# mj-will/aspire

Measured on AMD Instinct MI355X. Metric: particle-steps/sec (N x n_steps), 1M particles d=32; log-evidence err vs ref, higher is better.
Workload: dtype f64

## Files before the change

### aspire_amd/csrc/asmc_ctx.hip

```cpp
#include <dlfcn.h>
#include <stdarg.h>

#include <math.h>

#include "asmc_common.h"

static thread_local char g_err[512] = "";

void asmc_set_error(const char* fmt, ...) {
    va_list ap;
    va_start(ap, fmt);
    vsnprintf(g_err, sizeof(g_err), fmt, ap);
    va_end(ap);
}

__global__ __launch_bounds__(256) void k_poison_lds(int words) {
    extern __shared__ unsigned int s_poison[];
    for (int i = threadIdx.x; i < words; i += 256) s_poison[i] = 0xFFFFFFFFu;
    __syncthreads();
    if (s_poison[(threadIdx.x * 977) % words] != 0xFFFFFFFFu) __builtin_trap();
}
void asmc_poison_lds(asmc_ctx* ctx, hipStream_t st) {
    const int bytes = 160 * 1024 - 1024;
    static bool attr_set_dev[ASMC_MAX_DEVICES] = {false}; bool& attr_set = attr_set_dev[asmc_dev_slot(ctx)];
    if (!attr_set) {
        (void)hipFuncSetAttribute(reinterpret_cast<const void*>(k_poison_lds), hipFuncAttributeMaxDynamicSharedMemorySize, bytes);
        attr_set = true;
    }
    hipLaunchKernelGGL(k_poison_lds, dim3(4 * ctx->num_cu), dim3(256), bytes, st, bytes / 4);
}

void asmc_prof_begin(asmc_ctx* ctx, const char* label, const void* kernel, hipStream_t st) {
    if (!ctx || !ctx->prof_on) return;
    int v = 0;
    while (v < ctx->prof_nv && ctx->prof_vfn[v] != kernel) v++;
    if (v < ASMC_PROF_VARIANTS) {
        if (v == ctx->prof_nv) ctx->prof_vfn[v] = kernel, ctx->prof_vcnt[v] = 0, ctx->prof_nv++;
        ctx->prof_vcnt[v]++;
    }
    if (ctx->prof_n >= ASMC_PROF_MAX) return;
    ctx->prof_label[ctx->prof_n] = label;
    (void)hipEventRecord(ctx->prof_ev[2 * ctx->prof_n], st);
}

void asmc_prof_end(asmc_ctx* ctx, hipStream_t st) {
    if (!ctx || !ctx->prof_on || ctx->prof_n >= ASMC_PROF_MAX) return;
    (void)hipEventRecord(ctx->prof_ev[2 * ctx->prof_n + 1], st);
    ctx->prof_n++;
}

void asmc_bm_table_host(double* tab) {
    const long double two_pi = 6.283185307179586476925286766559005768L;
    for (int k = 0; k < BM_SC_N; k++) {
        const long double ang = two_pi * ((long double)k + 0.5L) / (long double)BM_SC_N;
        tab[2 * k] = (double)sinl(ang);
        tab[2 * k + 1] = (double)cosl(ang);
    }
    for (int i = 0; i < BM_LG_N; i++) {
        const long double c = 0.5L + ((long double)i + 0.5L) / (2.0L * BM_LG_N);
        const double rc = (double)(1.0L / c);
        tab[2 * (BM_SC_N + i)] = rc;
        tab[2 * (BM_SC_N + i) + 1] = (double)(2.0L * logl((long double)rc));
    }
}

extern "C" {

int asmc_profile_enable(asmc_ctx* ctx, int on) {
    ASMC_REQUIRE(ctx != nullptr, "null ctx");
    if (on && !ctx->prof_ev) {
        ctx->prof_ev = new (std::nothrow) hipEvent_t[2 * ASMC_PROF_MAX];
        ctx->prof_label = new (std::nothrow) const char*[ASMC_PROF_MAX];
        if (!ctx->prof_ev || !ctx->prof_label) {
            asmc_set_error("out of host memory");
            return ASMC_ERR_NOMEM;
        }
        for (int i = 0; i < 2 * ASMC_PROF_MAX; i++) ASMC_HIP(hipEventCreate(&ctx->prof_ev[i]));
    }
    ctx->prof_on = on ? 1 : 0;
    if (on) ctx->prof_n = 0, ctx->prof_nv = 0;
    return ASMC_OK;
}

int asmc_profile_variants(asmc_ctx* ctx, char* buf, int64_t buf_len) {
    ASMC_REQUIRE(ctx && buf && buf_len > 0, "bad arguments");
    buf[0] = 0;
    int64_t off = 0;
    for (int v = 0; v < ctx->prof_nv; v++) {
        Dl_info info;
        const char* sym = dladdr(ctx->prof_vfn[v], &info) && info.dli_sname && info.dli_saddr == ctx->prof_vfn[v] ? info.dli_sname : nullptr;
        char unknown[32];
        if (!sym) snprintf(unknown, sizeof(unknown), "%p", ctx->prof_vfn[v]), sym = unknown;
        const int w = snprintf(buf + off, (size_t)(buf_len - off), "%s %lld\n", sym, ctx->prof_vcnt[v]);
        if (w < 0 || off + w >= buf_len) {
            buf[off] = 0;
            asmc_set_error("asmc_profile_variants: buffer of %lld bytes too small", (long long)buf_len);
            return ASMC_ERR_ARG;
        }
        off += w;
    }
    ctx->prof_nv = 0;
    return ASMC_OK;
}

int asmc_profile_report(asmc_ctx* ctx, char* buf, int64_t buf_len) {
    ASMC_REQUIRE(ctx && buf && buf_len > 0, "bad arguments");
    buf[0] = 0;
    if (!ctx->prof_ev || ctx->prof_n == 0) return ASMC_OK;
    ASMC_HIP(hipEventSynchronize(ctx->prof_ev[2 * (ctx->prof_n - 1) + 1]));
    const int n = ctx->prof_n;
    int64_t off = 0;
    char* done = new (std::nothrow) char[n]();
    if (!done) return ASMC_ERR_NOMEM;
    for (int i = 0; i < n; i++) {
        if (done[i]) continue;
        double tot = 0.0;
        int cnt = 0;
        for (int j = i; j < n; j++) {
            if (done[j] || strcmp(ctx->prof_label[j], ctx->prof_label[i]) != 0) continue;
            float ms = 0.f;
            if (hipEventElapsedTime(&ms, ctx->prof_ev[2 * j], ctx->prof_ev[2 * j + 1]) == hipSuccess) {
                tot += ms;
                cnt++;
            }
            done[j] = 1;
        }
        const int w = snprintf(buf + off, (size_t)(buf_len - off), "%s %d %.6f\n", ctx->prof_label[i], cnt, cnt ? tot / cnt : 0.0);
        if (w < 0 || off + w >= buf_len) break;
        off += w;
    }
    delete[] done;
    ctx->prof_n = 0;
    return ASMC_OK;
}

int asmc_abi_version(void) { return ASMC_ABI_VERSION; }

const char* asmc_last_error(void) { return g_err; }

int asmc_device_count(int* n_out) {
    ASMC_REQUIRE(n_out != nullptr, "null output");
    int n = 0;
    hipError_t e = hipGetDeviceCount(&n);
    if (e != hipSuccess) {
        *n_out = 0;
        asmc_set_error("hipGetDeviceCount failed: %s", hipGetErrorString(e));
        return ASMC_ERR_HIP;
    }
    *n_out = n;
    return ASMC_OK;
}

int asmc_ctx_create(asmc_ctx** ctx_out, int device, int64_t n_max, int d_max) {
    ASMC_REQUIRE(ctx_out != nullptr, "null ctx_out");
    ASMC_REQUIRE(n_max > 0, "n_max must be positive");
    ASMC_REQUIRE(d_max > 0 && d_max <= ASMC_MAX_DIMS, "d_max out of range");
    *ctx_out = nullptr;
    ASMC_HIP(hipSetDevice(device));
    hipDeviceProp_t prop;
    ASMC_HIP(hipGetDeviceProperties(&prop, device));
    asmc_ctx* c = new (std::nothrow) asmc_ctx();
    if (!c) {
        asmc_set_error("out of host memory");
        return ASMC_ERR_NOMEM;
    }
    memset(c, 0, sizeof(*c));
    c->device = device;
    c->n_max = n_max;
    c->d_max = d_max;
    c->num_cu = prop.multiProcessorCount > 0 ? prop.multiProcessorCount : 256;
    c->n_tiles_max = scan_tiles(n_max) + 1;
    c->gram_blocks = (d_max <= 128 ? 4 : 2) * c->num_cu;
    if (c->gram_blocks > ASMC_MAX_BLOCKS) c->gram_blocks = ASMC_MAX_BLOCKS;
    hipError_t e = hipSuccess;
    auto dmalloc = [&](void** p, size_t bytes) {
        if (e == hipSuccess) e = hipMalloc(p, bytes);
    };
    dmalloc((void**)&c->d_partials, sizeof(double) * ASMC_MAX_BLOCKS * ASMC_MAX_BETAS * 2);
    dmalloc((void**)&c->d_small, sizeof(double) * DS_LEN);
    dmalloc((void**)&c->d_keys, sizeof(unsigned long long) * (ASMC_MAX_BETAS + 8));
    dmalloc((void**)&c->d_tiles, sizeof(double) * scratch_tiles_len(c->n_tiles_max));
    dmalloc((void**)&c->d_tiles_i, sizeof(long long) * scratch_tiles_i_len(c->n_tiles_max));
    c->gram_cap = (size_t)c->gram_blocks * d_max * d_max;
    if (c->gram_cap < (size_t)2048 * 1024) c->gram_cap = (size_t)2048 * 1024;
    dmalloc((void**)&c->d_gram, sizeof(double) * c->gram_cap);
    c->d_mmtab = nullptr;
    c->poison_lds = getenv("ASMC_POISON_LDS") != nullptr;
    c->d_max_pad = d_max <= 4 ? 4 : d_max <= 8 ? 8 : d_max <= 16 ? 16 : d_max <= 32 ? 32 : d_max <= 64 ? 64 : d_max <= 128 ? 128 : 0;
    dmalloc((void**)&c->d_mmtab, sizeof(double) * 2 * 144 * 64);
    dmalloc((void**)&c->d_guide, sizeof(unsigned int) * ((size_t)n_max + 8));
    dmalloc((void**)&c->d_tilectr, ASMC_TILECTR_BYTES + (size_t)n_max + 64);
    c->d_flags = c->d_tilectr ? reinterpret_cast<unsigned char*>(c->d_tilectr) + ASMC_TILECTR_BYTES : nullptr;
    dmalloc((void**)&c->d_gamma, sizeof(double) * ((size_t)ASMC_GAMMA_BATCH * (size_t)n_max + 64 * ASMC_GAMMA_BATCH));
    dmalloc((void**)&c->d_rec, sizeof(double) * 4 * (size_t)n_max);
    const size_t student = (size_t)d_max * (d_max + 1) + (size_t)(ASMC_STUDENT_MAX_ROWS / 64) * (d_max + 2);
    dmalloc((void**)&c->d_student, sizeof(double) * student);
    if (e == hipSuccess) e = hipHostMalloc((void**)&c->h_student, sizeof(double) * student, hipHostMallocDefault);
    dmalloc((void**)&c->d_counts, sizeof(long long) * (size_t)(ASMC_MAX_PCN_STEPS + ASMC_MAX_BLOCKS + n_max / 64 + 8));
    dmalloc((void**)&c->d_rho, sizeof(double) * (ASMC_MAX_PCN_STEPS + 8));
    dmalloc((void**)&c->d_stretch, sizeof(unsigned long long) * ASMC_MAX_PCN_STEPS);
    dmalloc((void**)&c->d_mh, sizeof(unsigned long long) * ASMC_MAX_PCN_STEPS);
    dmalloc((void**)&c->d_nuts, sizeof(unsigned long long) * (4 * ASMC_MAX_PCN_STEPS + 8));
    if (e == hipSuccess) e = hipMemset(c->d_tilectr, 0, ASMC_TILECTR_BYTES);
    dmalloc((void**)&c->d_bar, sizeof(unsigned int) * 1024 * 17);
    if (e == hipSuccess) e = hipMemset(c->d_bar, 0, sizeof(unsigned int) * 1024 * 17);
    dmalloc((void**)&c->d_pcgtab, sizeof(unsigned long long) * (64 * 4 + 8));
    dmalloc((void**)&c->d_select, sizeof(long long) * (2 * (ASMC_SELECT_THREADS / 64) + 8));
    dmalloc((void**)&c->d_ptab, sizeof(double) * (2 * 32 * 32 + 32 + 3 * ASMC_MAX_COMPONENTS * (1 + 2 * 32) + 64));
    dmalloc((void**)&c->d_bmtab, sizeof(double) * 2 * BM_TAB_N);
    dmalloc((void**)&c->d_fimg, ASMC_FUSED_IMAGE_BYTES);
    dmalloc((void**)&c->d_ref, sizeof(double) * (128 + 128 * 128));
    if (e == hipSuccess) {
        double tab[2 * BM_TAB_N];
        asmc_bm_table_host(tab);
        e = hipMemcpy(c->d_bmtab, tab, sizeof(tab), hipMemcpyHostToDevice);
    }
    if (e == hipSuccess) e = hipHostMalloc((void**)&c->h_pinned, sizeof(double) * HP_LEN, hipHostMallocDefault);
    if (e == hipSuccess) e = hipHostMalloc((void**)&c->h_gram, sizeof(double) * (128 + 128 * 128), hipHostMallocDefault);
    if (e != hipSuccess) {
        asmc_set_error("asmc_ctx_create: allocation failed: %s", hipGetErrorString(e));
        asmc_ctx_destroy(c);
        return ASMC_ERR_NOMEM;
    }
    *ctx_out = c;
    return ASMC_OK;
}

int asmc_ctx_destroy(asmc_ctx* c) {
    if (!c) return ASMC_OK;
    (void)hipSetDevice(c->device);
    (void)hipFree(c->d_partials);
    (void)hipFree(c->d_small);
    (void)hipFree(c->d_keys);
    (void)hipFree(c->d_tiles);
    (void)hipFree(c->d_tiles_i);
    (void)hipFree(c->d_gram);
    if (c->d_mmtab) (void)hipFree(c->d_mmtab);
    if (c->d_f16tab) (void)hipFree(c->d_f16tab);
    (void)hipFree(c->d_guide);
    (void)hipFree(c->d_gamma);
    (void)hipFree(c->d_student);
    if (c->h_student) (void)hipHostFree(c->h_student);
    if (c->d_ysoa) (void)hipFree(c->d_ysoa);
    if (c->d_xpad) (void)hipFree(c->d_xpad);
    if (c->d_chain_lq) (void)hipFree(c->d_chain_lq);
    if (c->d_chain_rows) (void)hipFree(c->d_chain_rows);
    (void)hipFree(c->d_counts);
    (void)hipFree(c->d_rho);
    (void)hipFree(c->d_stretch);
    (void)hipFree(c->d_mh);
    (void)hipFree(c->d_nuts);
    if (c->d_nuts_ws) (void)hipFree(c->d_nuts_ws);
    (void)hipFree(c->d_tilectr);
    (void)hipFree(c->d_rec);
    (void)hipFree(c->d_bar);
    (void)hipFree(c->d_pcgtab);
    (void)hipFree(c->d_select);
    (void)hipFree(c->d_ptab);
    (void)hipFree(c->d_bmtab);
    (void)hipFree(c->d_fimg);
    (void)hipFree(c->d_ref);
    if (c->prof_ev) {
        for (int i = 0; i < 2 * ASMC_PROF_MAX; i++) (void)hipEventDestroy(c->prof_ev[i]);
        delete[] c->prof_ev;
        delete[] c->prof_label;
    }
    if (c->h_pinned) (void)hipHostFree(c->h_pinned);
    if (c->h_gram) (void)hipHostFree(c->h_gram);
    if (c->ev_mutate) (void)hipEventDestroy(c->ev_mutate);
    if (c->ev_is) (void)hipEventDestroy(c->ev_is);
    delete c;
    return ASMC_OK;
}

}
```

### aspire_amd/csrc/asmc_pcn_dev.h

```cpp
#pragma once
#include "asmc_common.h"

bool asmc_flow_math_split();

struct PcnAdaptArgs {
    unsigned int* done;
    unsigned long long* nonfinite;
    long long* cell;
    const long long* prev_cell;
    long long* counts_out;
    double* rho;
    double* rho_hist;
    double target;
    int64_t n;
    int t, adapt;
    int last;
};

__device__ __forceinline__ double pcn_adapt_rho(double rho, long long c, int64_t n, double target, int t) {
    const double acc = (double)c / (double)n;
    double r = exp(log(rho) + (acc - target) / pow((double)(t + 1), 0.75));
    r = r < 1e-4 ? 1e-4 : r;
    r = r > 0.99 ? 0.99 : r;
    return r;
// ... 58 lines not shown
    const double dk = (double)k;
    return fma(dk, 6.93147180369123816490e-01, -((hfsq - fma(s, hfsq + R, dk * 1.90821492927058770002e-10)) - f));
}

__device__ __forceinline__ double bm_sqrt(double a) {
    const double y = __builtin_amdgcn_rsq(a);
    double g = a * y, h = 0.5 * y;
    const double r = fma(-h, g, 0.5);
    g = fma(g, r, g);
    h = fma(h, r, h);
    const double dres = fma(-g, g, a);
    return a > 0.0 ? fma(dres, h, g) : 0.0;
}

__device__ __forceinline__ void bm_sincos_turns(double u, double& sn, double& cs) {
    const double q = __builtin_rint(4.0 * u);
    const double f = fma(q, -0.25, u);
    const double x = f * 6.28318530717958647692;
    const double z = x * x;
    const double v = z * x;
    const double rs = fma(z, fma(z, fma(z, fma(z, 1.58969099521155010221e-10, -2.50507602534068634195e-08), 2.75573137070700676789e-06),
                                 -1.98412698298579493134e-04), 8.33333333332248946124e-03);
    const double sx = fma(v, fma(z, rs, -1.66666666666666324348e-01), x);
    const double rc = z * fma(z, fma(z, fma(z, fma(z, fma(z, -1.13596475577881948265e-11, 2.08757232129817482790e-09),
                                                -2.75573143513906633035e-07), 2.48015872894767294178e-05),
                                 -1.38888888888741095749e-03), 4.16666666666666019037e-02);
    const double hz = 0.5 * z;
    const double wv = 1.0 - hz;
    const double cx = wv + fma(z, rc, (1.0 - wv) - hz);
    const int qi = (int)q;
    const bool swap = qi & 1;
    const double s0 = swap ? cx : sx, c0 = swap ? sx : cx;
    sn = (qi & 2) ? -s0 : s0;
    cs = ((qi + 1) & 2) ? -c0 : c0;
}

__device__ __forceinline__ void box_muller(double u1, double u2, double& z0, double& z1) {
#ifdef ASMC_NOISE_LIBM
    const double r = sqrt(-2.0 * log(u1));
    double s, c;
    sincospi(2.0 * u2, &s, &c);
#else
    const double r = bm_sqrt(-2.0 * bm_log_unit(u1));
    double s, c;
    bm_sincos_turns(u2, s, c);
#endif
    z0 = r * c;
    z1 = r * s;
}

typedef double bm_d2 __attribute__((ext_vector_type(2)));
void asmc_bm_table_host(double* tab);

template <int THREADS>
__device__ __forceinline__ void bm_tab_stage(bm_d2* __restrict__ s, const double* __restrict__ g) {
    for (int e = threadIdx.x; e < BM_TAB_N; e += THREADS) s[e] = reinterpret_cast<const bm_d2*>(g)[e];
}
__device__ __forceinline__ void bm_tab_stage_rt(bm_d2* __restrict__ s, const double* __restrict__ g) {
    for (int e = threadIdx.x; e < BM_TAB_N; e += (int)blockDim.x) s[e] = reinterpret_cast<const bm_d2*>(g)[e];
}
__device__ __forceinline__ bm_d2* bm_lds() {
    __shared__ bm_d2 s_bm[BM_TAB_N];
    return s_bm;
}

struct BmPair {
    double m, sx, cm1;
    int e;
};
__device__ __forceinline__ void bm_pair_idx(uint32_t wr, uint32_t wa, BmPair& t, uint32_t& i_sc, uint32_t& i_lg) {
    i_sc = wa >> 24;
    const double X = (double)wr + 0.5;
    t.m = __builtin_amdgcn_frexp_mant(X);
    t.e = __builtin_amdgcn_frexp_exp(X);
    const uint32_t mh = (uint32_t)((unsigned long long)__double_as_longlong(t.m) >> 32);
    i_lg = BM_SC_N + ((mh >> 13) & (BM_LG_N - 1));
    const double x = fma((double)((int)(wa & 0xFFFFFFu) - (1 << 23)), 1.4629180792671596e-09, 7.314590396335798e-10);
    const double z = x * x;
    const double ps = fma(z, fma(z, -1.9841269841269841e-04, 8.3333333333333332e-03), -1.6666666666666666e-01);
    t.sx = fma(x * z, ps, x);
    t.cm1 = z * fma(z, fma(z, -1.3888888888888889e-03, 4.1666666666666664e-02), -0.5);
}
__device__ __forceinline__ void bm_pair_fin(const BmPair& t, const bm_d2 sc, const bm_d2 lg, double& z0, double& z1) {
    const double sn = sc.x + fma(sc.y, t.sx, sc.x * t.cm1);
    const double cs = sc.y + fma(-sc.x, t.sx, sc.y * t.cm1);
    const double r = fma(t.m, lg.x, -1.0);
    double p = fma(r, 3.3333333333333331e-01, -4.0000000000000002e-01);
    p = fma(r, p, 0.5);
    p = fma(r, p, -6.6666666666666663e-01);
    p = fma(r, p, 1.0);
    p = fma(r, p, -2.0);
    const double a = fma((double)(32 - t.e), 1.3862943611198906, lg.y) + r * p;
    const double y = __builtin_amdgcn_rsq(a);
    double g = a * y, h = 0.5 * y;
    const double rr = fma(-h, g, 0.5);
    g = fma(g, rr, g);
    h = fma(h, rr, h);
    const double rad = fma(fma(-g, g, a), h, g);
    z0 = rad * cs;
    z1 = rad * sn;
}
__device__ __forceinline__ void bm_pair32(uint32_t wr, uint32_t wa, const bm_d2* __restrict__ tab, double& z0, double& z1) {
    BmPair t;
    uint32_t i_sc, i_lg;
    bm_pair_idx(wr, wa, t, i_sc, i_lg);
    bm_pair_fin(t, tab[i_sc], tab[i_lg], z0, z1);
}

__device__ __forceinline__ void normal_quad(unsigned long long seed, unsigned long long gid, uint32_t step, uint32_t q,
                                            const bm_d2* __restrict__ tab, double& z0, double& z1, double& z2, double& z3) {
    uint32_t w[4];
    philox4x32_10((uint32_t)gid, (uint32_t)(gid >> 32), step, q | 0x20000000u, (uint32_t)seed, (uint32_t)(seed >> 32), w);
    BmPair ta, tb;
    uint32_t ia_sc, ia_lg, ib_sc, ib_lg;
    bm_pair_idx(w[0], w[1], ta, ia_sc, ia_lg);
    bm_pair_idx(w[2], w[3], tb, ib_sc, ib_lg);
    const bm_d2 sca = tab[ia_sc], lga = tab[ia_lg], scb = tab[ib_sc], lgb = tab[ib_lg];
    bm_pair_fin(ta, sca, lga, z0, z1);
    bm_pair_fin(tb, scb, lgb, z2, z3);
}
__device__ __forceinline__ void normal_pair(unsigned long long seed, unsigned long long gid, uint32_t step, uint32_t pr,
                                            const bm_d2* __restrict__ tab, double& z0, double& z1) {
    uint32_t w[4];
    philox4x32_10((uint32_t)gid, (uint32_t)(gid >> 32), step, (pr >> 1) | 0x20000000u, (uint32_t)seed, (uint32_t)(seed >> 32), w);
    const bool second = pr & 1u;
    bm_pair32(second ? w[2] : w[0], second ? w[3] : w[1], tab, z0, z1);
}

__device__ __forceinline__ void normal_quad_f32_raw(unsigned long long seed, unsigned long long gid, uint32_t step,
                                                    uint32_t slot, float& f0, float& f1, float& f2, float& f3) {
    uint32_t w[4];
    philox4x32_10((uint32_t)gid, (uint32_t)(gid >> 32), step, slot | 0x40000000u, (uint32_t)seed,
                  (uint32_t)(seed >> 32), w);
    const float k = 2.3283064365386963e-10f;
    const float u0 = fmaf((float)w[0], k, 1.1641532182693481e-10f);
    const float u1 = fmaf((float)w[2], k, 1.1641532182693481e-10f);
    const float t0 = (float)w[1] * k, t1 = (float)w[3] * k;
    const float r0 = __builtin_amdgcn_sqrtf(-1.3862943611198906f * __builtin_amdgcn_logf(u0));
    const float r1 = __builtin_amdgcn_sqrtf(-1.3862943611198906f * __builtin_amdgcn_logf(u1));
    f0 = r0 * __builtin_amdgcn_cosf(t0);
    f1 = r0 * __builtin_amdgcn_sinf(t0);
    f2 = r1 * __builtin_amdgcn_cosf(t1);
    f3 = r1 * __builtin_amdgcn_sinf(t1);
}

__device__ __forceinline__ void normal_quad_f32(unsigned long long seed, unsigned long long gid, uint32_t step,
                                                uint32_t slot, double& z0, double& z1, double& z2, double& z3) {
    float f0, f1, f2, f3;
    normal_quad_f32_raw(seed, gid, step, slot, f0, f1, f2, f3);
    z0 = (double)f0;
    z1 = (double)f1;
    z2 = (double)f2;
    z3 = (double)f3;
}

__device__ __forceinline__ double accept_uniform(unsigned long long seed, unsigned long long gid,
                                                 uint32_t step) {
    uint32_t w[4];
    philox4x32_10((uint32_t)gid, (uint32_t)(gid >> 32), step, 0xFFFFFFFFu, (uint32_t)seed,
                  (uint32_t)(seed >> 32), w);
    return u01_from_words(w[0], w[1]);
}

template <bool F32 = false>
__device__ __forceinline__ double gamma_unit(double shape, unsigned long long seed, unsigned long long gid,
                                             uint32_t step, const bm_d2* __restrict__ tab) {
    const double dd = shape - 1.0 / 3.0, c = 1.0 / sqrt(9.0 * dd);
#pragma unroll
    for (uint32_t a = 0; a < 8; a++) {
        double z0;
        uint32_t w[4];
        philox4x32_10((uint32_t)gid, (uint32_t)(gid >> 32), step, (F32 ? 0xC0000000u : 0x80000000u) | a, (uint32_t)seed, (uint32_t)(seed >> 32), w);
        if (F32) {
            const float k = 2.3283064365386963e-10f;
            const float u0 = fmaf((float)w[0], k, 1.1641532182693481e-10f);
            const float r0 = __builtin_amdgcn_sqrtf(-1.3862943611198906f * __builtin_amdgcn_logf(u0));
            z0 = (double)(r0 * __builtin_amdgcn_cosf((float)w[1] * k));
        } else {
            double z1;
            bm_pair32(w[0], w[1], tab, z0, z1);
        }
        const double u = u01_from_words(w[2], w[3]);
        double v = 1.0 + c * z0;
        if (v <= 0.0) continue;
        v = v * v * v;
        if (log(u) < 0.5 * z0 * z0 + dd - dd * v + dd * log(v)) return dd * v;
    }
    return dd;
}
template <bool TP = true>
__device__ __forceinline__ double tpcn_scale(double rho, double nu, double q0, const double* __restrict__ gam, int64_t i) {
    if (!TP || gam == nullptr) return rho;
    return rho * sqrt((nu + q0) / (2.0 * gam[i]));
}
template <bool TP>
__device__ __forceinline__ double tpcn_scale_ct(double rho, double nu, double q0, const double* __restrict__ gam, int64_t i) {
    if (!TP) return rho;
    return rho * sqrt((nu + q0) / (2.0 * gam[i]));
}
__device__ __forceinline__ double log1p_nonneg(double x) {
    const double u = 1.0 + x;
    const double r = bm_log_unit(u);
    return u < INFINITY ? r : u;
}
template <bool TP>
__device__ __forceinline__ double ref_corr_ct(double q, double nu, int d) {
    if (!TP) return 0.5 * q;
    return 0.5 * ((double)d + nu) * log1p_nonneg(q / nu);
}

template <bool TP = true>
__device__ __forceinline__ double ref_corr(double q, double nu, int d) {
    if (!TP) return 0.5 * q;
    return nu > 0.0 ? 0.5 * ((double)d + nu) * log1p_nonneg(q / nu) : 0.5 * q;
}

struct MixDev {
    int C;
    const double* logw;
    const double* mu;
    const double* prec;
};

static inline MixDev to_dev(const asmc_mixture& m) {
    MixDev r;
    r.C = m.n_components;
    r.logw = m.logw_dev;
    r.mu = m.mu_dev;
    r.prec = m.prec_dev;
    return r;
}


__device__ __forceinline__ double log_p_t_guard(double r) { return (r < INFINITY) ? r : -INFINITY; }
__device__ __forceinline__ double log_p_t(double ll, double lp, double lq, double beta) {
    return log_p_t_guard((1.0 - beta) * lq + beta * (ll + lp));
}


struct PcnDev {
    int d;
    double beta;
    const double* mu;
    const double* L;
    const double* Linv;
    MixDev ll, lp, lq;
    unsigned long long seed, gid0;
    int noise;
    double nu;
    const double* gam;
    void* ys;
    long long n_pad;
    const double* bmtab;
    unsigned char* tile_par;
    int d_noise;
    int dpad;
    int mode;
};


#define PTAB_TRI(D) ((D) * ((D) + 1) / 2)
#define PTAB_MIX(D) (ASMC_MAX_COMPONENTS * (1 + 2 * (D)))
#define PTAB_SIZE(D) (2 * PTAB_TRI(D) + (D) + 3 * PTAB_MIX(D))
#define PTAB_BLK(D) (((D) / 4) * ((D) / 4 + 1) / 2 * 16)
struct PcnScalars {
    double beta;
    double nu;
    const double* gam;
    void* ys;
    long long n_pad;
    int d_real;
    unsigned long long seed, gid0;
    int c_ll, c_lp, c_lq;
    const double* bmtab;
    unsigned char* tile_par;
    int d_noise;
};


template <typename T>
__device__ __forceinline__ double soa_load(__amdgpu_buffer_rsrc_t r, unsigned voff, unsigned soff) {
    if constexpr (sizeof(T) == 8) {
        const auto v = __builtin_amdgcn_raw_buffer_load_b64(r, (int)voff, (int)soff, 0);
        return __builtin_bit_cast(double, v);
    } else {
        const unsigned v = __builtin_amdgcn_raw_buffer_load_b32(r, (int)voff, (int)soff, 0);
        return (double)__uint_as_float(v);
    }
}
template <typename T>
__device__ __forceinline__ void soa_store(__amdgpu_buffer_rsrc_t r, unsigned voff, unsigned soff, double x) {
    if constexpr (sizeof(T) == 8) {
        using u2 = decltype(__builtin_amdgcn_raw_buffer_load_b64(r, 0, 0, 0));
        __builtin_amdgcn_raw_buffer_store_b64(__builtin_bit_cast(u2, x), r, (int)voff, (int)soff, 0);
    } else {
        __builtin_amdgcn_raw_buffer_store_b32(__float_as_uint((float)x), r, (int)voff, (int)soff, 0);
    }
}


bool asmc_pcn_flow_fused_ok(const asmc_pcn_params* prm, const asmc_coupling* f);
int asmc_pcn_flow_fused_launch(asmc_ctx* ctx, int64_t n, int x_dtype, double* ll, double* lp, double* lq, const PcnDev& pd,
                               const asmc_coupling* f, const double* rho_ptr, uint32_t step, unsigned int* tile_counter,
                               long long* block_counts, int* grid_out, const PcnAdaptArgs& adapt, int img_words, hipStream_t st);
int asmc_pcn_flow_fused_stage(asmc_ctx* ctx, const PcnDev& pd, const asmc_coupling* f, int* words_out, hipStream_t st);

#define MM_WHITEN 0
#define MM_STEP 1
#define MM_UNWHITEN 2
#define MM_STEP_T 3
#define MM_XPROPOSE 4
#define MM_XPROPOSE_T 5
#define MM_UNWHITEN_X 6
bool asmc_pcn_mm_supported(int d, const void* x);
int asmc_pcn_mm_pack(asmc_ctx* ctx, const PcnDev& pd, hipStream_t st);
int asmc_pcn_flow16_tables(asmc_ctx* ctx, const PcnDev& pd, const asmc_coupling* f, hipStream_t st);
int asmc_pcn_flow16_launch(asmc_ctx* ctx, int64_t n, int x_dtype, void* x, double* ll, double* lp, double* lq, const PcnDev& pd,
                           const asmc_coupling* f, const double* rho_ptr, uint32_t step, long long* block_counts, int* grid_out,
                           unsigned long long* nonfinite, hipStream_t st);
int asmc_pcn_mm_launch(asmc_ctx* ctx, int64_t n, int x_dtype, void* x, double* ll, double* lp, double* lq, const PcnDev& pd,
                       int mode, const double* rho_ptr, uint32_t step, long long* block_counts, int* grid_out,
                       hipStream_t st);
bool asmc_gram_mm_supported(int d, const void* x);
int asmc_gram_mm_launch(asmc_ctx* ctx, int64_t n, int d, int x_dtype, const void* x, const double* d_center, int* grid_out,
                        hipStream_t st, double* out2, double n_div);
```

### aspire_amd/csrc/asmc_pcn_drive.hip

```cpp
#include <stdlib.h>

#include <chrono>

#include "asmc_pcn_shared.h"

static PcnDev pcn_dev_from_params(const asmc_ctx* ctx, const asmc_pcn_params* prm, int d_noise) {
    PcnDev pd;
    memset(&pd, 0, sizeof(pd));
    pd.bmtab = ctx->d_bmtab;
    pd.d = prm->d;
    pd.d_noise = d_noise;
    pd.beta = prm->beta;
    pd.mu = prm->mu_dev;
    pd.L = prm->L_dev;
    pd.Linv = prm->Linv_dev;
    pd.seed = prm->seed;
    pd.gid0 = prm->gid0;
    pd.nu = prm->nu;
    return pd;
}

struct PcnNeeds {
    int n_mix;
    bool noise;
// ... 245 lines not shown
        rc = pack_pcn_tables(ctx, pd, st);
        if (rc) return rc;
        return pcn_step_launch(ctx, n, x_dtype, const_cast<void*>(x), qf_old, qf_new, nullptr, pd, rho_ptr, step, nullptr, &grid, st);
    }
    if (asmc_pcn_mm_supported(d, x) && ((uintptr_t)x_prop % 16) == 0 && ctx->d_mmtab && !pcn_env_generic()) {
        pd.noise = ASMC_NOISE_F64;
        rc = asmc_pcn_mm_pack(ctx, pd, st);
        if (rc) return rc;
        return asmc_pcn_mm_launch(ctx, n, x_dtype, const_cast<void*>(x), qf_old, qf_new, reinterpret_cast<double*>(x_prop), pd,
                                  pd.nu > 0.0 ? MM_XPROPOSE_T : MM_XPROPOSE, rho_ptr, step, nullptr, &grid, st);
    }
    const int D = pcn_pad_dim(d);
    if (D != d && D > 0 && D <= ctx->d_max_pad && !(D == 32 && d > 16) && !pcn_env_generic() && !pcn_env_nopad()) {
        PcnDev src = pd;
        src.ll.C = src.lp.C = src.lq.C = 0;
        PcnPadded pad;
        rc = pcn_pad_problem(ctx, n, d, D, x_dtype, x, src, 0, st, &pad);
        if (rc) return rc;
        PcnDev p2 = pd;
        p2.d = D;
        p2.d_noise = d;
        p2.mu = pad.mu;
        p2.L = pad.L;
        p2.Linv = pad.Linv;
        rc = pcn_propose_launch(ctx, n, D, x_dtype, pad.xp, pad.xq, qf_old, qf_new, p2, rho_ptr, step, st);
        if (rc) return rc;
        return launch_unpad_rows(ctx, n, d, D, x_dtype, pad.xq, x_prop, st);
    }
    return pcn_generic_propose_launch(ctx, n, x_dtype, x, x_prop, qf_old, qf_new, pd, rho_ptr, step, &grid, st);
}

static int ysplit_pd(asmc_ctx* ctx, int64_t n, const asmc_pcn_params* prm, PcnDev& pd) {
    ASMC_REQUIRE(ctx && prm, "null pointer");
    ASMC_REQUIRE(n > 0 && n <= ctx->n_max, "n out of range for this ctx");
    ASMC_REQUIRE(prm->x_dtype == ASMC_F64 || prm->x_dtype == ASMC_F32, "bad x_dtype");
    ASMC_REQUIRE(prm->mu_dev && prm->L_dev && prm->Linv_dev, "null reference pointer");
    ASMC_REQUIRE(!(prm->nu > 0.0) || prm->nu >= 1.0, "nu must be >= 1 (or <= 0 for the Gaussian reference)");
    pd = pcn_dev_from_params(ctx, prm, 0);
    ASMC_REQUIRE(prm->noise == ASMC_NOISE_F64 || prm->noise == ASMC_NOISE_F32, "bad noise mode");
    pd.noise = prm->noise;
    return ASMC_OK;
}

static int ysplit_propose_prepare(asmc_ctx* ctx, int64_t n, PcnDev& pd, uint32_t step, hipStream_t st) {
    pd.ys = ctx->d_ysoa;
    pd.n_pad = ((n + 63) / 64) * 64;
    if (ctx->ptab_tag == 0 || ctx->ptab_tag != ctx->ysplit_seq) {
        const int rc = pack_pcn_tables(ctx, pd, st);
        if (rc) return rc;
        ctx->ptab_tag = ctx->ysplit_seq;
    }
    return pcn_prepare_gamma(ctx, n, pd, step, st);
}

extern "C" {

int asmc_pcn_propose(asmc_ctx* ctx, int64_t n, int d, int x_dtype, const void* x, void* x_prop, double* qf_old,
                     double* qf_new, const double* mu, const double* L, const double* Linv, double rho, double nu,
                     uint64_t seed, uint64_t gid0, uint32_t step, asmc_stream stream) {
    ASMC_REQUIRE(ctx && x && x_prop && qf_old && qf_new && mu && L && Linv, "null pointer");
    ASMC_REQUIRE(!(nu > 0.0) || nu >= 1.0, "nu must be >= 1 (or <= 0 for the Gaussian reference)");
    ASMC_REQUIRE(n > 0 && n <= ctx->n_max && d > 0 && d <= ASMC_MAX_DIMS, "bad sizes");
    ASMC_REQUIRE(x_dtype == ASMC_F64 || x_dtype == ASMC_F32, "bad x_dtype");
    ASMC_REQUIRE(rho >= 0.0 && rho <= 1.0, "rho must be in (0, 1], or 0 for the device-resident step size");
    const int fits = pcn_generic_check(d, x_dtype);
    if (fits) return fits;
    hipStream_t st = as_stream(stream);
    PcnDev pd;
    memset(&pd, 0, sizeof(pd));
    pd.bmtab = ctx->d_bmtab;
    pd.d = d;
    pd.mu = mu;
    pd.L = L;
    pd.Linv = Linv;
    pd.seed = seed;
    pd.gid0 = gid0;
    pd.nu = nu;
    if (rho > 0.0) {
        const int rc = pcn_set_scalar_launch(ctx, ctx->d_rho, rho, st);
        if (rc) return rc;
    }
    return pcn_propose_launch(ctx, n, d, x_dtype, x, x_prop, qf_old, qf_new, pd, ctx->d_rho, step, st);
}

int asmc_pcn_split_begin(asmc_ctx* ctx, double rho0, asmc_stream stream) {
    ASMC_REQUIRE(ctx != nullptr, "null ctx");
    ASMC_REQUIRE(rho0 > 0.0 && rho0 <= 1.0, "rho must be in (0, 1]");
    return pcn_set_scalar_launch(ctx, ctx->d_rho, rho0, as_stream(stream));
}

int asmc_pcn_split_adapt(asmc_ctx* ctx, int64_t n_global, double target_accept, int t, int adapt, asmc_stream stream) {
    ASMC_REQUIRE(ctx != nullptr, "null ctx");
    ASMC_REQUIRE(n_global > 0 && t >= 0 && t < ASMC_MAX_PCN_STEPS, "bad n_global / step index");
    hipStream_t st = as_stream(stream);
    return pcn_close_step(ctx, st, 1, reinterpret_cast<const long long*>(ctx->d_keys), n_global, t, ctx->d_counts, ctx->d_rho,
                          ctx->d_rho + 8, target_accept, adapt);
}

int asmc_pcn_split_end(asmc_ctx* ctx, int n_steps, int64_t* n_accept_host, double* rho_hist_host, double* rho_host,
                       asmc_stream stream) {
    ASMC_REQUIRE(ctx && n_accept_host && rho_host, "null pointer");
    ASMC_REQUIRE(n_steps >= 1 && n_steps <= ASMC_MAX_PCN_STEPS, "n_steps out of range");
    hipStream_t st = as_stream(stream);
    ASMC_HIP(hipStreamSynchronize(st));
    return pcn_finish_call(ctx, 0, nullptr, n_steps, nullptr, false, rho_host, n_accept_host, rho_hist_host, st);
}

int asmc_pcn_ysplit_begin(asmc_ctx* ctx, int64_t n, const void* x, const asmc_pcn_params* prm, double rho0,
                          asmc_stream stream) {
    PcnDev pd;
    int rc = ysplit_pd(ctx, n, prm, pd);
    if (rc) return rc;
    ASMC_REQUIRE(x != nullptr, "null pointer");
    ASMC_REQUIRE(rho0 > 0.0 && rho0 <= 1.0, "rho must be in (0, 1]");
    hipStream_t st = as_stream(stream);
    if (!pcn_reg_supported(pd.d, prm->x_dtype == ASMC_F64 ? 8 : 4, x) || !pcn_ensure_ysoa(ctx, n, pd.d, prm->x_dtype, pd, st)) {
        asmc_set_error("whitened-state split session: d=%d is not a register-kernel dimension or no scratch", pd.d);
        return ASMC_ERR_UNSUPPORTED;
    }
    rc = pcn_set_scalar_launch(ctx, ctx->d_rho, rho0, st);
    if (rc) return rc;
    rc = pack_pcn_tables(ctx, pd, st);
    if (rc) return rc;
    ctx->ptab_tag = ++ctx->ysplit_seq;
    pd.mode = PCN_WHITEN_S;
    pd.noise = ASMC_NOISE_F64;
    int grid = 0;
    return pcn_step_launch(ctx, n, prm->x_dtype, const_cast<void*>(x), nullptr, nullptr, nullptr, pd, ctx->d_rho, 0, pcn_block_counts(ctx),
                           &grid, st);
}

int asmc_pcn_ysplit_propose(asmc_ctx* ctx, int64_t n, const asmc_pcn_params* prm, uint32_t step, void* x_prop,
                            asmc_stream stream) {
    PcnDev pd;
    int rc = ysplit_pd(ctx, n, prm, pd);
    if (rc) return rc;
    ASMC_REQUIRE(x_prop != nullptr && ((uintptr_t)x_prop % 16) == 0, "x_prop must be a 16-byte aligned device buffer");
    ASMC_REQUIRE(ctx->d_ysoa != nullptr, "no session (asmc_pcn_ysplit_begin)");
    hipStream_t st = as_stream(stream);
    rc = ysplit_propose_prepare(ctx, n, pd, step, st);
    if (rc) return rc;
    int grid = 0;
    return pcn_reg_flow_launch(ctx, n, prm->x_dtype, PCN_FLOW_PROPOSE_SX, nullptr, x_prop, nullptr, nullptr, nullptr, nullptr, nullptr,
                               nullptr, pd, ctx->d_rho, step, pcn_block_counts(ctx), &grid, st);
}

int asmc_pcn_ysplit_propose_tr(asmc_ctx* ctx, int64_t n, const asmc_pcn_params* prm, uint32_t step, const asmc_transform* t,
                               const double* premap_dev, const asmc_mixture* qmix, int minus_logj, void* x_prop,
                               double* logj_out, double* lq_out, asmc_stream stream) {
    PcnDev pd;
    int rc = ysplit_pd(ctx, n, prm, pd);
    if (rc) return rc;
    ASMC_REQUIRE(t && x_prop && logj_out && ((uintptr_t)x_prop % 16) == 0, "null / misaligned pointer");
    ASMC_REQUIRE(ctx->d_ysoa != nullptr, "no session (asmc_pcn_ysplit_begin)");
    ASMC_REQUIRE(t->d == pd.d && t->kind_dev && t->lower_dev && t->upper_dev, "transform tables missing or of another dimension");
    ASMC_REQUIRE((t->mean_dev == nullptr) == (t->std_dev == nullptr), "affine stage needs both mean and std");
    ASMC_REQUIRE((premap_dev == nullptr) == (qmix == nullptr) && (premap_dev == nullptr) == (lq_out == nullptr),
                 "premap, mixture and lq_out come together");
    ASMC_REQUIRE(!qmix || qmix->n_components == 1, "the proposal density must be a single Gaussian");
    const int logit = (t->hints & 7) == (ASMC_TR_NO_PERIODIC | ASMC_TR_NO_PROBIT);
    const int probit = (t->hints & 7) == (ASMC_TR_NO_PERIODIC | ASMC_TR_NO_LOGIT);
    if (!logit && !probit) {
        asmc_set_error("asmc_pcn_ysplit_propose_tr: the transform must be non-periodic with ONE bounded stage (hints %d)", t->hints);
        return ASMC_ERR_UNSUPPORTED;
    }
    hipStream_t st = as_stream(stream);
    rc = ysplit_propose_prepare(ctx, n, pd, step, st);
    if (rc) return rc;
    double* d_tab = ctx->d_small + DS_TRTAB;
    rc = pcn_trtab_pack_launch(ctx, pd.d, t, premap_dev, qmix, minus_logj, d_tab, st);
    if (rc) return rc;
    int grid = 0;
    return pcn_reg_flow_launch(ctx, n, prm->x_dtype, logit ? PCN_FLOW_PROPOSE_SXT_LOGIT : PCN_FLOW_PROPOSE_SXT_PROBIT, nullptr, x_prop,
                               nullptr, nullptr, nullptr, logj_out, lq_out, d_tab, pd, ctx->d_rho, step, pcn_block_counts(ctx), &grid, st);
}

int asmc_pcn_ysplit_accept(asmc_ctx* ctx, int64_t n, const asmc_pcn_params* prm, uint32_t step, double* ll, double* lp,
                           double* lq, const double* ll_new, const double* lp_new, const double* lq_new, double* lj,
                           const double* lj_new, int64_t n_global, int t, asmc_stream stream) {
    PcnDev pd;
    int rc = ysplit_pd(ctx, n, prm, pd);
    if (rc) return rc;
    ASMC_REQUIRE(ll && lp && lq && ll_new && lp_new && lq_new, "null pointer");
    ASMC_REQUIRE((lj == nullptr) == (lj_new == nullptr), "log-Jacobian arrays: both or neither");
    ASMC_REQUIRE(ctx->d_ysoa != nullptr, "no session (asmc_pcn_ysplit_begin)");
    ASMC_REQUIRE(n_global > 0 && t >= 0 && t < ASMC_MAX_PCN_STEPS, "bad n_global / step index");
    hipStream_t st = as_stream(stream);
    pd.ys = ctx->d_ysoa;
    pd.n_pad = ((n + 63) / 64) * 64;
    rc = pcn_prepare_gamma(ctx, n, pd, step, st);
    if (rc) return rc;
    int grid = 0;
    long long* d_block = pcn_block_counts(ctx);
    rc = pcn_reg_flow_launch(ctx, n, prm->x_dtype, lj ? PCN_FLOW_ACCEPT_SJ : PCN_FLOW_ACCEPT_S, lj, const_cast<double*>(lj_new), ll, lp, lq,
                             const_cast<double*>(ll_new), const_cast<double*>(lp_new), lq_new, pd, ctx->d_rho, step, d_block, &grid, st);
    if (rc) return rc;
    return pcn_close_step(ctx, st, grid, d_block, n_global, t, ctx->d_counts, ctx->d_rho, ctx->d_rho + 8, prm->target_accept,
                          prm->adapt);
}

}

int asmc_pcn_ysplit_unwhiten(asmc_ctx* ctx, int64_t n, void* x, const asmc_pcn_params* prm, bool repack, hipStream_t st) {
    PcnDev pd;
    int rc = ysplit_pd(ctx, n, prm, pd);
    if (rc) return rc;
    ASMC_REQUIRE(x != nullptr && ctx->d_ysoa != nullptr, "null pointer / no session");
    ASMC_REQUIRE(repack || pcn_reg_supported(pd.d, prm->x_dtype == ASMC_F64 ? 8 : 4, x), "x_out: a 16-byte aligned buffer of a session's d");
    pd.ys = ctx->d_ysoa;
    pd.n_pad = ((n + 63) / 64) * 64;
    pd.mode = PCN_UNWHITEN_XS;
    pd.noise = ASMC_NOISE_F64;
    if (repack || ctx->ptab_tag == 0 || ctx->ptab_tag != ctx->ysplit_seq) {
        rc = pack_pcn_tables(ctx, pd, st);
        if (rc) return rc;
        if (!repack) ctx->ptab_tag = ctx->ysplit_seq;
    }
    int grid = 0;
    return pcn_step_launch(ctx, n, prm->x_dtype, x, nullptr, nullptr, nullptr, pd, ctx->d_rho, 0, pcn_block_counts(ctx), &grid, st);
}

extern "C" {

int asmc_pcn_ysplit_end(asmc_ctx* ctx, int64_t n, void* x, const asmc_pcn_params* prm, asmc_stream stream) {
    return asmc_pcn_ysplit_unwhiten(ctx, n, x, prm, true, as_stream(stream));
}

int asmc_pcn_accept(asmc_ctx* ctx, int64_t n, int d, int x_dtype, void* x, const void* x_prop, double* ll, double* lp,
                    double* lq, const double* ll_new, const double* lp_new, const double* lq_new,
                    double* lj_old, const double* lj_new, const double* qf_old, const double* qf_new,
                    double beta, uint64_t seed, uint64_t gid0, uint32_t step, int64_t* n_accept_host,
                    asmc_stream stream) {
    ASMC_REQUIRE(ctx && x && x_prop && ll && lp && lq && ll_new && lp_new && lq_new && qf_old && qf_new, "null pointer");
    ASMC_REQUIRE(n > 0 && n <= ctx->n_max && d > 0, "bad sizes");
    ASMC_REQUIRE(x_dtype == ASMC_F64 || x_dtype == ASMC_F32, "bad x_dtype");
    hipStream_t st = as_stream(stream);
    int rc = pcn_accept_flags_launch(ctx, n, ll, lp, lq, ll_new, lp_new, lq_new, lj_old, lj_new, qf_old, qf_new, beta, seed, gid0, step, st);
    if (rc) return rc;
    rc = launch_copy_flagged(ctx, n, d, x_dtype, x, x_prop, ctx->d_flags, st);
    if (rc) return rc;
    if (n_accept_host) {
        unsigned long long* h = reinterpret_cast<unsigned long long*>(ctx->h_pinned);
        ASMC_HIP(hipMemcpyAsync(h, ctx->d_keys, sizeof(unsigned long long), hipMemcpyDeviceToHost, st));
        ASMC_HIP(hipStreamSynchronize(st));
        *n_accept_host = (int64_t)h[0];
    }
    return ASMC_OK;
}

int64_t asmc_pcn_flow_work_bytes(int64_t n, int d, int x_dtype) {
    const int64_t xb = ((n * d * (x_dtype == ASMC_F64 ? 8 : 4) + 255) / 256) * 256;
    return xb + 5 * (((n * 8 + 255) / 256) * 256);
}

}

static unsigned long long* pcn_flow_bad_cell(asmc_ctx* ctx) {
    return reinterpret_cast<unsigned long long*>(ctx->d_tilectr + 2 * ASMC_MAX_PCN_STEPS);
}

static int pcn_mutate_flow_impl(asmc_ctx* ctx, int64_t n, void* x, double* ll, double* lp, double* lq,
                                const asmc_pcn_params* prm, const asmc_coupling* flow, void* work_dev, int n_steps, uint32_t step0,
                                double* rho_inout_host, int64_t* n_accept_host, double* rho_hist_host, asmc_stream stream, int d_noise) {
    hipStream_t st = as_stream(stream);
    const int d = prm->d;
    const int64_t xb = ((n * d * (prm->x_dtype == ASMC_F64 ? 8 : 4) + 255) / 256) * 256;
    const int64_t vb = ((n * 8 + 255) / 256) * 256;
    char* w = reinterpret_cast<char*>(work_dev);
    void* x_prop = w;
    double* q0 = reinterpret_cast<double*>(w + xb);
    double* q1 = reinterpret_cast<double*>(w + xb + vb);
    double* ll_new = reinterpret_cast<double*>(w + xb + 2 * vb);
    double* lp_new = reinterpret_cast<double*>(w + xb + 3 * vb);
    double* lq_new = reinterpret_cast<double*>(w + xb + 4 * vb);
    PcnDev pd = pcn_dev_from_params(ctx, prm, d_noise);
    double* d_rho = ctx->d_rho;
    long long* d_block = pcn_block_counts(ctx);
    const PcnLoop loop = {ctx, n, prm, n_steps, step0, st};
    int rc;
    const bool reg_ok = pcn_reg_supported(d, prm->x_dtype == ASMC_F64 ? 8 : 4, x) && !pcn_env_xstate();
    if (reg_ok) {
        pd.ll = to_dev(prm->log_likelihood);
        pd.lp = to_dev(prm->log_prior);
        pd.lq = pd.lp;
        pd.noise = prm->noise;
        rc = pack_pcn_tables(ctx, pd, st, d_rho, *rho_inout_host);
        if (rc) return rc;
        int grid = 0;
        const bool soa = pcn_ensure_ysoa(ctx, n, d, prm->x_dtype, pd, st, asmc_pcn_flow_fused_ok(prm, flow));
        auto convert = [&](int mode) -> int {
            PcnDev pc = pd;
            pc.mode = !soa ? mode : mode == PCN_WHITEN ? PCN_WHITEN_S : PCN_UNWHITEN_XS;
            pc.noise = ASMC_NOISE_F64;
            return pcn_step_launch(ctx, n, prm->x_dtype, x, ll, lp, lq, pc, d_rho, 0, d_block, &grid, st);
        };
        rc = convert(PCN_WHITEN);
        if (rc) return rc;
        const bool fused = soa && asmc_pcn_flow_fused_ok(prm, flow);
        if (d_noise > 0 && !fused) {
            asmc_set_error("asmc_pcn_mutate_flow: the zero-padded form needs the one-kernel step");
            return ASMC_ERR_UNSUPPORTED;
        }
        if (fused) {
            ASMC_HIP(hipMemsetAsync(ctx->d_tilectr, 0, ASMC_TILECTR_BYTES + ((size_t)((n + 63) / 64) + 15) / 16 * 16, st));
            pd.tile_par = ctx->d_flags;
            int img_words = 0;
            rc = asmc_pcn_flow_fused_stage(ctx, pd, flow, &img_words, st);
            if (rc) return rc;
            const int lag = prm->adapt >= 2 ? prm->adapt : 1;
            rc = pcn_steps(
                loop, pd,
                [&](int t, uint32_t step, int* g) -> int {
                    PcnAdaptArgs ad = {ctx->d_tilectr + ASMC_MAX_PCN_STEPS + t,
                                       reinterpret_cast<unsigned long long*>(ctx->d_tilectr + 2 * ASMC_MAX_PCN_STEPS),
                                       ctx->count_hook ? ctx->count_cell : nullptr,
                                       ctx->count_hook && t > 0 ? ctx->count_cell : nullptr, ctx->d_counts, d_rho, d_rho + 8,
                                       prm->target_accept, ctx->count_hook ? ctx->count_n_global : n, t, prm->adapt, t == n_steps - 1};
                    if (ctx->count_hook && lag > ctx->count_cells) {
                        asmc_set_error("adapt_lag %d needs %d exchange cells, the installed hook has %d (asmc_pcn_set_count_cells)", lag, lag, ctx->count_cells);
                        return ASMC_ERR_ARG;
                    }
                    return asmc_pcn_flow_fused_launch(ctx, n, prm->x_dtype == ASMC_F64 ? ASMC_F64 : ASMC_F32, ll, lp, lq, pd, flow, d_rho, step,
                                                      ctx->d_tilectr + t, d_block, g, ad, img_words, st);
                },
                [&](int t, int) -> int {
                    if (!(ctx->count_hook && ((t + 1) % lag == 0 || t == n_steps - 1))) return ASMC_OK;
                    const int hrc = ctx->count_hook(ctx->count_hook_user, reinterpret_cast<asmc_stream>(st));
                    if (hrc != 0) {
                        asmc_set_error("accept-count exchange hook failed (%d)", hrc);
                        return ASMC_ERR_ARG;
                    }
                    return t == n_steps - 1 ? pcn_adapt_exchanged_launch(ctx, t, prm->target_accept, prm->adapt, lag, st) : ASMC_OK;
                });
        } else {
            rc = pcn_steps(
                loop, pd,
                [&](int, uint32_t step, int* g) -> int {
                    int r = pcn_reg_flow_launch(ctx, n, prm->x_dtype, soa ? PCN_FLOW_PROPOSE_S : PCN_FLOW_PROPOSE, x, x_prop, ll, lp, lq, ll_new,
                                                lp_new, lq_new, pd, d_rho, step, d_block, g, st);
                    if (r) return r;
                    r = asmc_coupling_logprob(ctx, n, prm->x_dtype, x_prop, flow, lq_new, stream);
                    if (r) return r;
                    return pcn_reg_flow_launch(ctx, n, prm->x_dtype, soa ? PCN_FLOW_ACCEPT_S : PCN_FLOW_ACCEPT, x, x_prop, ll, lp, lq, ll_new,
                                               lp_new, lq_new, pd, d_rho, step, d_block, g, st);
                },
                pcn_close(loop, d_block));
        }
        if (rc) return rc;
        rc = convert(PCN_UNWHITEN_X);
        if (rc) return rc;
    } else {
        rc = pcn_set_scalar_launch(ctx, d_rho, *rho_inout_host, st);
        if (rc) return rc;
        if (d_noise > 0) {
            asmc_set_error("asmc_pcn_mutate_flow: the zero-padded form needs the one-kernel step");
            return ASMC_ERR_UNSUPPORTED;
        }
        rc = pcn_steps(
            loop, pd,
            [&](int, uint32_t step, int* g) -> int {
                int r = pcn_propose_launch(ctx, n, d, prm->x_dtype, x, x_prop, q0, q1, pd, d_rho, step, st);
                if (r) return r;
                r = asmc_coupling_logprob(ctx, n, prm->x_dtype, x_prop, flow, lq_new, stream);
                if (r) return r;
                r = asmc_mixture_logpdf(ctx, n, d, prm->x_dtype, x_prop, &prm->log_prior, lp_new, stream);
                if (r) return r;
                r = asmc_mixture_logpdf(ctx, n, d, prm->x_dtype, x_prop, &prm->log_likelihood, ll_new, stream);
                if (r) return r;
                r = pcn_accept_flags_launch(ctx, n, ll, lp, lq, ll_new, lp_new, lq_new, nullptr, nullptr, q0, q1, prm->beta, prm->seed, prm->gid0,
                                            step, st);
                if (r) return r;
                *g = 1;
                return launch_copy_flagged(ctx, n, d, prm->x_dtype, x, x_prop, ctx->d_flags, st);
            },
            pcn_close(loop, reinterpret_cast<const long long*>(ctx->d_keys)));
        if (rc) return rc;
    }
    return pcn_finish_call(ctx, n, lq, n_steps, pcn_flow_bad_cell(ctx), ctx->mutate_defer, rho_inout_host, n_accept_host, rho_hist_host, st);
}

static int pcn_mutate_flow16_impl(asmc_ctx* ctx, int64_t n, void* x, double* ll, double* lp, double* lq, const asmc_pcn_params* prm,
                                  const asmc_coupling* flow, int n_steps, uint32_t step0, double* rho_inout_host,
                                  int64_t* n_accept_host, double* rho_hist_host, asmc_stream stream, int d_noise) {
    ASMC_REQUIRE(ctx->d_mmtab != nullptr && ((uintptr_t)x % 16) == 0, "flow16: ctx was created with d_max <= 32, or a misaligned state");
    hipStream_t st = as_stream(stream);
    PcnDev pd = pcn_dev_from_params(ctx, prm, d_noise);
    pd.ll = to_dev(prm->log_likelihood);
    pd.lp = to_dev(prm->log_prior);
    pd.lq = pd.lp;
    pd.noise = prm->noise;
    double* d_rho = ctx->d_rho;
    long long* d_block = pcn_block_counts(ctx);
    unsigned long long* d_bad = pcn_flow_bad_cell(ctx);
    const PcnLoop loop = {ctx, n, prm, n_steps, step0, st};
    int rc = pcn_set_scalar_launch(ctx, d_rho, *rho_inout_host, st);
    if (rc) return rc;
    ASMC_HIP(hipMemsetAsync(d_bad, 0, sizeof(unsigned long long), st));
    rc = asmc_pcn_mm_pack(ctx, pd, st);
    if (rc) return rc;
    rc = asmc_pcn_flow16_tables(ctx, pd, flow, st);
    if (rc) return rc;
    int grid = 0;
    rc = asmc_pcn_mm_launch(ctx, n, prm->x_dtype, x, ll, lp, lq, pd, MM_WHITEN, d_rho, 0, d_block, &grid, st);
    if (rc) return rc;
    rc = pcn_steps(
        loop, pd,
        [&](int, uint32_t step, int* g) { return asmc_pcn_flow16_launch(ctx, n, prm->x_dtype, x, ll, lp, lq, pd, flow, d_rho, step, d_block, g, d_bad, st); },
        pcn_close(loop, d_block));
    if (rc) return rc;
    rc = asmc_pcn_mm_launch(ctx, n, prm->x_dtype, x, ll, lp, lq, pd, MM_UNWHITEN_X, d_rho, 0, d_block, &grid, st);
    if (rc) return rc;
    return pcn_finish_call(ctx, n, lq, n_steps, d_bad, ctx->mutate_defer, rho_inout_host, n_accept_host, rho_hist_host, st);
}

template <typename Impl>
static int pcn_flow_padded_tail(asmc_ctx* ctx, int64_t n, int d, int D, int x_dtype, const void* xp, void* x, int n_steps,
                                double* rho_inout_host, int64_t* n_accept_host, double* rho_hist_host, hipStream_t st, Impl impl) {
    const int caller_defers = ctx->mutate_defer;
    ctx->mutate_defer = 1;
    int rc = impl();
    ctx->mutate_defer = caller_defers;
    if (rc) return rc;
    rc = launch_unpad_rows(ctx, n, d, D, x_dtype, xp, x, st);
    if (rc) return rc;
    if (caller_defers) return ASMC_OK;
    ctx->mutate_pending_steps = 0;
    return pcn_collect(ctx, n_steps, true, true, rho_inout_host, n_accept_host, rho_hist_host, st);
}

extern "C" {

int asmc_pcn_mutate_flow(asmc_ctx* ctx, int64_t n, void* x, double* ll, double* lp, double* lq,
                         const asmc_pcn_params* prm, const asmc_coupling* flow, void* work_dev, int64_t work_bytes,
                         int n_steps, uint32_t step0, double* rho_inout_host, int64_t* n_accept_host,
                         double* rho_hist_host, asmc_stream stream) {
    ASMC_REQUIRE(ctx && x && prm && flow, "null pointer");
    if (ctx->chain_on) {
        asmc_set_error("asmc_pcn_mutate_flow: the chain recorder is honoured by asmc_pcn_mutate only (asmc_chain_clear first)");
        return ASMC_ERR_UNSUPPORTED;
    }
    ASMC_REQUIRE(flow->affine == ASMC_AFFINE_TANH || (flow->affine == ASMC_AFFINE_SOFTCLIP && flow->kind == ASMC_FLOW_MAF),
                 "bad affine form (the soft-clipped form is for autoregressive flows)");
    const int d = prm->d;
    const bool lay16 = asmc_flow_layout(flow->kind, flow->dims, flow->hidden) == 1;
    int D16 = 0;
    asmc_pcn_params p16 = *prm;
    if ((d > 32 || lay16) && d <= 128 && d == flow->dims && ctx->d_mmtab && !pcn_env_generic() && !pcn_env_nopad() && !pcn_env_xstate()) {
        const int D = d <= 64 ? 64 : 128;
        p16.d = D;
        if ((D <= ctx->d_max_pad || d <= 32) && asmc_pcn_flow16_ok(&p16, flow)) D16 = D;
    }
    asmc_pcn_params p2 = *prm;
    p2.d = 32;
    const bool pad32 = !D16 && d >= 2 && d < 32 && d == flow->dims && 32 <= ctx->d_max_pad && !pcn_env_generic() && !pcn_env_nopad() &&
                       asmc_pcn_flow_fused_ok(&p2, flow) && !pcn_env_aos() && !pcn_env_xstate();
    const bool reads_noise = D16 || pad32 || (pcn_reg_supported(d, prm->x_dtype == ASMC_F64 ? 8 : 4, x) && !pcn_env_xstate());
    int rc = pcn_check_call(__func__, ctx, n, x, ll, lp, lq, prm, n_steps, rho_inout_host, n_accept_host,
                            {2, reads_noise, flow, !D16, work_dev, work_bytes});
    if (rc) return rc;
    hipStream_t st = as_stream(stream);
    if (D16) {
        if (d == D16 && ((uintptr_t)x % 16) == 0)
            return pcn_mutate_flow16_impl(ctx, n, x, ll, lp, lq, prm, flow, n_steps, step0, rho_inout_host, n_accept_host, rho_hist_host,
                                          stream, 0);
        void* xp = nullptr;
        rc = pcn_pad_params(ctx, n, x, prm, D16, 2, st, &p16, &xp);
        if (rc) return rc;
        return pcn_flow_padded_tail(ctx, n, d, D16, prm->x_dtype, xp, x, n_steps, rho_inout_host, n_accept_host, rho_hist_host, st, [&]() {
            return pcn_mutate_flow16_impl(ctx, n, xp, ll, lp, lq, &p16, flow, n_steps, step0, rho_inout_host, n_accept_host,
                                          rho_hist_host, stream, d);
        });
    }
    if (pad32) {
        void* xp = nullptr;
        rc = pcn_pad_params(ctx, n, x, prm, 32, 2, st, &p2, &xp);
        if (rc) return rc;
        rc = pcn_flow_padded_tail(ctx, n, d, 32, prm->x_dtype, xp, x, n_steps, rho_inout_host, n_accept_host, rho_hist_host, st, [&]() {
            return pcn_mutate_flow_impl(ctx, n, xp, ll, lp, lq, &p2, flow, work_dev, n_steps, step0, rho_inout_host, n_accept_host,
                                        rho_hist_host, stream, d);
        });
        if (rc != ASMC_ERR_UNSUPPORTED) return rc;
        ctx->mutate_pending_steps = 0;
    }
    return pcn_mutate_flow_impl(ctx, n, x, ll, lp, lq, prm, flow, work_dev, n_steps, step0, rho_inout_host, n_accept_host, rho_hist_host,
                                stream, 0);
}

int asmc_pcn_mutate_flow_enqueue(asmc_ctx* ctx, int64_t n, void* x, double* ll, double* lp, double* lq,
                                 const asmc_pcn_params* prm, const asmc_coupling* flow, void* work_dev, int64_t work_bytes,
                                 int n_steps, uint32_t step0, double rho, asmc_stream stream) {
    ASMC_REQUIRE(ctx != nullptr, "null ctx");
    ASMC_REQUIRE(ctx->mutate_pending_steps == 0, "a deferred mutation is still pending (asmc_pcn_mutate_flow_result)");
    int64_t dummy_acc = 0;
    ctx->mutate_defer = 1;
    const int rc = asmc_pcn_mutate_flow(ctx, n, x, ll, lp, lq, prm, flow, work_dev, work_bytes, n_steps, step0, &rho, &dummy_acc,
                                        nullptr, stream);
    ctx->mutate_defer = 0;
    return rc;
}

int asmc_pcn_mutate_flow_result(asmc_ctx* ctx, int n_steps, double* rho_out_host, int64_t* n_accept_host, double* rho_hist_host,
                                asmc_stream stream) {
    ASMC_REQUIRE(ctx && rho_out_host && n_accept_host, "null pointer");
    ASMC_REQUIRE(ctx->mutate_pending_steps == n_steps && n_steps > 0, "no deferred mutation of this length is pending");
    ctx->mutate_pending_steps = 0;
    return pcn_collect(ctx, n_steps, true, true, rho_out_host, n_accept_host, rho_hist_host, as_stream(stream), ctx->ev_mutate);
}

int64_t asmc_pcn_flow_nonfinite(asmc_ctx* ctx) { return ctx ? (int64_t)ctx->flow_nonfinite : -1; }

int64_t asmc_pcn_lq_nan(asmc_ctx* ctx) { return ctx ? (int64_t)ctx->lq_nan : -1; }

int asmc_pcn_set_count_hook(asmc_ctx* ctx, asmc_count_hook hook, void* user, int64_t* cell_dev, int64_t n_global) {
    ASMC_REQUIRE(ctx != nullptr, "null ctx");
    ASMC_REQUIRE(hook == nullptr || (cell_dev != nullptr && n_global > 0), "hook needs a device cell and n_global > 0");
    ctx->count_hook = hook;
    ctx->count_hook_user = user;
    ctx->count_cell = reinterpret_cast<long long*>(cell_dev);
    ctx->count_n_global = n_global;
    ctx->count_cells = 1;
    return ASMC_OK;
}

int asmc_pcn_set_count_cells(asmc_ctx* ctx, int n_cells) {
    ASMC_REQUIRE(ctx != nullptr && n_cells >= 1 && n_cells <= ASMC_MAX_COUNT_CELLS, "n_cells out of range");
    ctx->count_cells = n_cells;
    return ASMC_OK;
}

typedef int (*rccl_allreduce_fn)(const void*, void*, size_t, int, int, void*, hipStream_t);
static int rccl_count_hook(void* user, asmc_stream stream) {
    asmc_ctx* ctx = static_cast<asmc_ctx*>(user);
    const int nccl_int64 = 4, nccl_sum = 0;
    return reinterpret_cast<rccl_allreduce_fn>(ctx->rccl_allreduce)(ctx->count_cell, ctx->count_cell, (size_t)ctx->count_cells, nccl_int64, nccl_sum,
                                                                    ctx->rccl_comm, reinterpret_cast<hipStream_t>(stream));
}

int asmc_set_rccl(asmc_ctx* ctx, void* allreduce_fn, void* nccl_comm) {
    ASMC_REQUIRE(ctx != nullptr, "null ctx");
    ASMC_REQUIRE((allreduce_fn == nullptr) == (nccl_comm == nullptr), "function and communicator come together");
    ctx->rccl_allreduce = allreduce_fn;
    ctx->rccl_comm = nccl_comm;
    return ASMC_OK;
}

int asmc_set_rccl_allgather(asmc_ctx* ctx, void* allgather_fn) {
    ASMC_REQUIRE(ctx != nullptr, "null ctx");
    ctx->rccl_allgather = allgather_fn;
    return ASMC_OK;
}

int asmc_rccl_all_gather(asmc_ctx* ctx, const void* send_dev, void* recv_dev, int64_t count, int is_int64, asmc_stream stream) {
    ASMC_REQUIRE(ctx && send_dev && recv_dev && count > 0, "bad arguments");
    ASMC_REQUIRE(ctx->rccl_allgather && ctx->rccl_comm, "asmc_set_rccl / asmc_set_rccl_allgather first");
    typedef int (*allgather_fn)(const void*, void*, size_t, int, void*, hipStream_t);
    const int dt = is_int64 ? 4 : 8;
    if (reinterpret_cast<allgather_fn>(ctx->rccl_allgather)(send_dev, recv_dev, (size_t)count, dt, ctx->rccl_comm,
                                                            reinterpret_cast<hipStream_t>(stream)) != 0) {
        asmc_set_error("asmc_rccl_all_gather: ncclAllGather failed");
        return ASMC_ERR_ARG;
    }
    return ASMC_OK;
}

int asmc_pcn_set_count_rccl(asmc_ctx* ctx, int64_t* cell_dev, int64_t n_global) {
    ASMC_REQUIRE(ctx != nullptr, "null ctx");
    if (cell_dev == nullptr) return asmc_pcn_set_count_hook(ctx, nullptr, nullptr, nullptr, 0);
    ASMC_REQUIRE(ctx->rccl_allreduce && ctx->rccl_comm, "asmc_set_rccl first");
    return asmc_pcn_set_count_hook(ctx, rccl_count_hook, ctx, cell_dev, n_global);
}

}
```

### aspire_amd/csrc/asmc_pcn_fused.hip

```cpp
#include <stdlib.h>

#include "asmc_common.h"
#include <type_traits>
#include "asmc_pcn_dev.h"
#include "asmc_flow_dev.h"

#ifndef FUSED_THREADS
#define FUSED_THREADS 512
#endif

#define FUSED_TL_DOUBLES 1368
#define FUSED_MAX_COMPONENTS 4
#ifndef MV_DEPTH
#define MV_DEPTH 4
#endif
typedef double double2v __attribute__((ext_vector_type(2)));
__host__ __device__ constexpr int mv_group(int bi) {
    int g = 0;
    while ((g + 1) * (g + 2) <= bi) g++;
    return g;
}
template <int I, int N, typename F>
__device__ __forceinline__ void mv_for_each(F& f) {
    if constexpr (I < N) {
        f(std::integral_constant<int, I>{});
        mv_for_each<I + 1, N>(f);
    }
}
#ifndef FUSED_INPLACE
#define FUSED_INPLACE 1
#endif
#ifndef FUSED_MVMFMA
#define FUSED_MVMFMA FUSED_INPLACE
#endif
typedef double fused_d4 __attribute__((ext_vector_type(4)));
typedef unsigned fused_u4 __attribute__((ext_vector_type(4)));
__device__ __forceinline__ void fused_swap32(double& x, double& y) {
    const unsigned long long xb = __builtin_bit_cast(unsigned long long, x), yb = __builtin_bit_cast(unsigned long long, y);
    const auto lo = __builtin_amdgcn_permlane32_swap((unsigned)xb, (unsigned)yb, false, false);
    const auto hi = __builtin_amdgcn_permlane32_swap((unsigned)(xb >> 32), (unsigned)(yb >> 32), false, false);
    x = __builtin_bit_cast(double, ((unsigned long long)hi[0] << 32) | lo[0]);
    y = __builtin_bit_cast(double, ((unsigned long long)hi[1] << 32) | lo[1]);
}
__device__ __forceinline__ void fused_swap16(double& x, double& y) {
    const unsigned long long xb = __builtin_bit_cast(unsigned long long, x), yb = __builtin_bit_cast(unsigned long long, y);
    const auto lo = __builtin_amdgcn_permlane16_swap((unsigned)xb, (unsigned)yb, false, false);
    const auto hi = __builtin_amdgcn_permlane16_swap((unsigned)(xb >> 32), (unsigned)(yb >> 32), false, false);
    x = __builtin_bit_cast(double, ((unsigned long long)hi[0] << 32) | lo[0]);
    y = __builtin_bit_cast(double, ((unsigned long long)hi[1] << 32) | lo[1]);
}
__device__ __forceinline__ void fused_transpose4(double& q0, double& q1, double& q2, double& q3) {
    fused_swap32(q0, q2);
    fused_swap32(q1, q3);
    fused_swap16(q0, q1);
    fused_swap16(q2, q3);
}
#ifndef HS1P_PREFETCH
#define HS1P_PREFETCH false
#endif
#ifndef FUSED_PRIO_A
#define FUSED_PRIO_A 2
#define FUSED_PRIO_B 1
#endif
#ifndef MV_CHUNK
#define MV_CHUNK 8
#endif
constexpr int FUSED_D = 32;
constexpr int T_MU = FUSED_D * FUSED_D, T_LLMU = T_MU + FUSED_D, T_LLPR = T_LLMU + FUSED_D, T_LPMU = T_LLPR + FUSED_D, T_LPPR = T_LPMU + FUSED_D,
              T_LOGW = T_LPPR + FUSED_D, T_LOC = T_LOGW + 2;
static_assert(T_LOC + 3 * FUSED_D / 2 <= FUSED_TL_DOUBLES, "pCN tables");
constexpr int M_MU = 12 * 64, M_MIX = M_MU + FUSED_D, M_LOGW = M_MIX + 2 * FUSED_MAX_COMPONENTS * 2 * FUSED_D, M_LOC = M_LOGW + 2 * FUSED_MAX_COMPONENTS;
static_assert(M_LOC + 3 * FUSED_D / 2 <= FUSED_TL_DOUBLES, "pCN tables (matrix-core variant)");
constexpr bool MVM = FUSED_MVMFMA && FUSED_INPLACE;

template <int W, int NOISE, bool HS, int KIND>
__device__ __forceinline__ void fused_stage_tables(float* __restrict__ sp, const double* __restrict__ ptab, const PcnScalars& p,
                                                   const float* __restrict__ packed, int n_layers, const float* __restrict__ loc,
                                                   const float* __restrict__ scale) {
    constexpr int D = FUSED_D, THREADS = FUSED_THREADS, HF = KIND == ASMC_FLOW_MAF ? 32 : 16;
    using FD = FlowDims<HF, W>;
    if (HS) {
        flow_stage_hs<HF, W, THREADS>(sp, packed, n_layers);
    } else {
        const int total4 = n_layers * FD::LAYER / 4;
        for (int base = 0; base < total4; base += THREADS * 8) {
            float4 tmp[8];
#pragma unroll
            for (int q = 0; q < 8; q++) {
                const int i4 = base + q * THREADS + threadIdx.x;
                tmp[q] = i4 < total4 ? reinterpret_cast<const float4*>(packed)[i4] : make_float4(0.f, 0.f, 0.f, 0.f);
            }
#pragma unroll
            for (int q = 0; q < 8; q++) {
                const int i4 = base + q * THREADS + threadIdx.x;
                if (i4 < total4) reinterpret_cast<float4*>(sp)[i4] = tmp[q];
            }
        }
    }
    double* tl = reinterpret_cast<double*>(sp + (size_t)n_layers * FD::LAYER);
    {
        const double* m0g = ptab + 2 * PTAB_TRI(D) + D;
        const int dr = (p.d_noise > 0 && p.d_noise < D) ? p.d_noise : D;
        const int dhalf = KIND == ASMC_FLOW_MAF ? 16 : dr / 2;
        auto nat = [&](int r) -> int {
            const int c = r < 16 ? (r < dhalf ? r : -1) : (r - 16 + dhalf);
            return (c >= 0 && c < dr) ? c : -1;
        };
        if (MVM) {
            for (int e = threadIdx.x; e < 12 * 64; e += THREADS) {
                const int slot = e >> 6, l = e & 63, mb = slot < 4 ? 0 : 1, sidx = slot < 4 ? slot : slot - 4;
                const int i = l & 15, j = nat(16 * mb + 4 * (i & 3) + (i >> 2)), k = 4 * sidx + (l >> 4);
                tl[e] = (j >= 0 && k <= j) ? ptab[j * (j + 1) / 2 + k] : 0.0;
            }
            for (int e = threadIdx.x; e < D; e += THREADS) {
                const int j = nat(16 * ((e >> 2) & 1) + 4 * (e >> 3) + (e & 3));
                tl[M_MU + e] = j >= 0 ? ptab[2 * PTAB_TRI(D) + j] : 0.0;
                reinterpret_cast<float*>(tl + M_LOC)[e] = j >= 0 ? loc[j] : 0.0f;
                reinterpret_cast<float*>(tl + M_LOC)[D + e] = j >= 0 ? scale[j] : 1.0f;
                reinterpret_cast<float*>(tl + M_LOC)[2 * D + e] = j >= 0 ? 1.0f / scale[j] : 1.0f;
            }
            for (int e = threadIdx.x; e < 2 * FUSED_MAX_COMPONENTS * D; e += THREADS) {
                const int tc = e / D, er = e % D, tt = tc / FUSED_MAX_COMPONENTS, c = tc % FUSED_MAX_COMPONENTS;
                const int j = nat(16 * ((er >> 2) & 1) + 4 * (er >> 3) + (er & 3));
                const bool live = j >= 0 && c < (tt == 0 ? p.c_ll : p.c_lp);
                const double* mg = m0g + (size_t)tt * PTAB_MIX(D);
                tl[M_MIX + tc * 2 * D + er] = live ? mg[ASMC_MAX_COMPONENTS + c * D + j] : 0.0;
                tl[M_MIX + tc * 2 * D + D + er] = live ? mg[ASMC_MAX_COMPONENTS * (1 + D) + c * D + j] : 0.0;
            }
            if (threadIdx.x < 2 * FUSED_MAX_COMPONENTS) {
                const int tt = threadIdx.x / FUSED_MAX_COMPONENTS, c = threadIdx.x % FUSED_MAX_COMPONENTS;
                tl[M_LOGW + threadIdx.x] = c < (tt == 0 ? p.c_ll : p.c_lp) ? m0g[(size_t)tt * PTAB_MIX(D) + c] : -INFINITY;
            }
        } else {
            for (int e = threadIdx.x; e < D * D; e += THREADS) {
                const int j = e / D, k = e - j * D;
                tl[e] = k <= j ? ptab[j * (j + 1) / 2 + k] : 0.0;
            }
            for (int e = threadIdx.x; e < D; e += THREADS) {
                tl[T_MU + e] = ptab[2 * PTAB_TRI(D) + e];
                tl[T_LLMU + e] = m0g[ASMC_MAX_COMPONENTS + e];
                tl[T_LLPR + e] = m0g[ASMC_MAX_COMPONENTS * (1 + D) + e];
                tl[T_LPMU + e] = m0g[PTAB_MIX(D) + ASMC_MAX_COMPONENTS + e];
                tl[T_LPPR + e] = m0g[PTAB_MIX(D) + ASMC_MAX_COMPONENTS * (1 + D) + e];
                reinterpret_cast<float*>(tl + T_LOC)[e] = loc[e];
                reinterpret_cast<float*>(tl + T_LOC)[D + e] = scale[e];
                reinterpret_cast<float*>(tl + T_LOC)[2 * D + e] = 1.0f / scale[e];
            }
        }
        if (!MVM && threadIdx.x == 0) tl[T_LOGW] = m0g[0], tl[T_LOGW + 1] = m0g[PTAB_MIX(D)];
    }
    if (NOISE == ASMC_NOISE_F64) bm_tab_stage<THREADS>(reinterpret_cast<bm_d2*>(tl + FUSED_TL_DOUBLES), p.bmtab);
}
template <int W, int NOISE, int KIND>
__host__ __device__ constexpr int fused_image_words(int n_layers) {
    return (int)(((size_t)n_layers * FlowDims<(KIND == ASMC_FLOW_MAF ? 32 : 16), W>::LAYER * sizeof(float) + FUSED_TL_DOUBLES * sizeof(double) +
                  (NOISE == ASMC_NOISE_F64 ? BM_TAB_N * sizeof(bm_d2) : 0)) / 16);
}
template <int W, int NOISE, bool HS, int KIND>
__global__ __launch_bounds__(FUSED_THREADS) void k_fused_stage_image(const double* __restrict__ ptab, PcnScalars p, const float* __restrict__ packed,
                                                                     int n_layers, const float* __restrict__ loc, const float* __restrict__ scale,
                                                                     fused_u4* __restrict__ img, int img_words) {
    extern __shared__ __align__(16) float sp[];
    fused_stage_tables<W, NOISE, HS, KIND>(sp, ptab, p, packed, n_layers, loc, scale);
    __syncthreads();
    for (int i = threadIdx.x; i < img_words; i += FUSED_THREADS) img[i] = reinterpret_cast<const fused_u4*>(sp)[i];
}

template <typename T, int W, int NOISE, bool HS, int KIND = ASMC_FLOW_COUPLING, bool MIX = false>
__global__ __launch_bounds__(FUSED_THREADS) void k_pcn_flow_fused(
    int64_t n, double* __restrict__ ll, double* __restrict__ lp, double* __restrict__ lq, const double* __restrict__ ptab,
    PcnScalars p, const double* rho_ptr, uint32_t step, const float* __restrict__ packed, int n_layers,
    const float* __restrict__ loc, const float* __restrict__ scale, float ladj0, float base_const,
    unsigned int* __restrict__ tile_counter, long long* __restrict__ block_counts, PcnAdaptArgs ad, int par_words, int affine,
    const fused_u4* __restrict__ img, int img_words) {
    constexpr int D = FUSED_D, H = 16, THREADS = FUSED_THREADS;
    constexpr int HF = KIND == ASMC_FLOW_MAF ? 32 : H;
    static_assert(KIND == ASMC_FLOW_COUPLING || HS, "the autoregressive variant runs the split-fp16 layers only");
    using FD = FlowDims<HF, W>;
    extern __shared__ __align__(16) float sp[];
    constexpr int IMG_Q = ASMC_FUSED_IMAGE_BYTES / 16 / THREADS;
    fused_u4 iw[IMG_Q];
    if (img != nullptr) {
#pragma unroll
        for (int q = 0; q < IMG_Q; q++) {
            const int i4 = q * THREADS + (int)threadIdx.x;
            iw[q] = img[i4 < img_words ? i4 : img_words - 1];
        }
    } else {
        fused_stage_tables<W, NOISE, HS, KIND>(sp, ptab, p, packed, n_layers, loc, scale);
    }
    double* tl = reinterpret_cast<double*>(sp + (size_t)n_layers * FD::LAYER);
    bm_d2* bmt = reinterpret_cast<bm_d2*>(tl + FUSED_TL_DOUBLES);
    unsigned* const par_bits = reinterpret_cast<unsigned*>(bmt + BM_TAB_N);
    for (int wd = threadIdx.x; wd < par_words; wd += THREADS) {
        const uint4 b0 = reinterpret_cast<const uint4*>(p.tile_par)[2 * wd], b1 = reinterpret_cast<const uint4*>(p.tile_par)[2 * wd + 1];
        const unsigned q[8] = {b0.x, b0.y, b0.z, b0.w, b1.x, b1.y, b1.z, b1.w};
        unsigned bits = 0;
#pragma unroll
        for (int k = 0; k < 8; k++) {
            const unsigned nib = (((q[k] & 0x01010101u) * 0x01020408u) >> 24) & 0xFu;
            bits |= nib << (4 * k);
        }
        par_bits[wd] = bits;
    }
    if (img != nullptr) {
        __builtin_amdgcn_sched_barrier(0);
#pragma unroll
        for (int q = 0; q < IMG_Q; q++) {
            const int i4 = q * THREADS + (int)threadIdx.x;
            if (i4 < img_words) reinterpret_cast<fused_u4*>(sp)[i4] = iw[q];
        }
    }
    __syncthreads();
    const int lane = threadIdx.x & 63, wave = threadIdx.x >> 6, hh = lane >> 5;
    const bool first_on_simd = __builtin_amdgcn_readfirstlane(wave) < 4;
#ifdef FUSED_STAGGER
    if (!first_on_simd) {
#pragma unroll 1
        for (int i = 0; i < FUSED_STAGGER; i++) __builtin_amdgcn_s_sleep(127);
    }
#endif
    double rho;
    if (ad.prev_cell) {
        const double rp = ad.rho_hist[ad.t - 1];
        if (ad.adapt <= 1) {
            const long long cp = *ad.prev_cell;
            rho = ad.adapt ? pcn_adapt_rho(rp, cp, ad.n, ad.target, ad.t - 1) : rp;
            if (blockIdx.x == 0 && threadIdx.x == 0) ad.counts_out[ad.t - 1] = cp;
        } else if (ad.t % ad.adapt == 0) {
            double r = rp;
            for (int tp = ad.t - ad.adapt; tp < ad.t; tp++) {
                const long long ct = ad.prev_cell[tp % ad.adapt];
                r = pcn_adapt_rho(r, ct, ad.n, ad.target, tp);
                if (blockIdx.x == 0 && threadIdx.x == 0) ad.counts_out[tp] = ct;
            }
            rho = r;
        } else {
            rho = rp;
        }
    } else {
        rho = *rho_ptr;
    }
    if (ad.cell && blockIdx.x == 0 && threadIdx.x == 0) ad.rho_hist[ad.t] = rho;
    const double a = sqrt(1.0 - rho * rho);
    const int dn = __builtin_amdgcn_readfirstlane((p.d_noise > 0 && p.d_noise < 32) ? p.d_noise : 32);
    const int64_t n_tiles = (n + 63) / 64;
    long long n_acc = 0, n_bad = 0;
#ifdef FUSED_STAMP
    unsigned long long tsum[8] = {0, 0, 0, 0, 0, 0, 0, 0}, tprev = 0;
    int ntile = 0;
#define STAMP(k)                                                  \
    do {                                                          \
        __builtin_amdgcn_sched_barrier(0);                        \
        unsigned long long tn_;                                   \
        asm volatile("s_memtime %0\n\ts_waitcnt lgkmcnt(0)" : "=s"(tn_)::"memory"); \
        tsum[k] += tn_ - tprev;                                   \
        tprev = tn_;                                              \
        __builtin_amdgcn_sched_barrier(0);                        \
    } while (0)
#else
#define STAMP(k)
#endif
    const unsigned long long ysa = (unsigned long long)(uintptr_t)p.ys;
    T* ysu = reinterpret_cast<T*>(((unsigned long long)(unsigned)__builtin_amdgcn_readfirstlane((int)(ysa >> 32)) << 32) |
                                  (unsigned)__builtin_amdgcn_readfirstlane((int)(unsigned)ysa));
    const int half_records = (int)__builtin_amdgcn_readfirstlane((int)(unsigned)((unsigned long long)p.n_pad * D * sizeof(T)));
    T* const ysu1 = ysu + (size_t)__builtin_amdgcn_readfirstlane((int)(unsigned)p.n_pad) * D;
    const unsigned ys_row = (unsigned)__builtin_amdgcn_readfirstlane((int)(unsigned)p.n_pad) * (unsigned)sizeof(T);
    const unsigned ys_lane = (unsigned)lane * (unsigned)sizeof(T);
    unsigned char* __restrict__ const tile_par = p.tile_par;
#ifdef FUSED_STAMP
    asm volatile("s_memtime %0\n\ts_waitcnt lgkmcnt(0)" : "=s"(tprev)::"memory");
#endif
#ifdef FUSED_HALF
    const bool idle_wave = wave >= 4;
#else
    const bool idle_wave = false;
#endif
#ifdef FUSED_STATIC_TILES
    unsigned static_next = blockIdx.x * (THREADS / 64) + (threadIdx.x >> 6);
    auto tile_fetch = [&]() -> unsigned {
        const unsigned t_l = static_next;
        static_next += gridDim.x * (THREADS / 64);
        return t_l;
    };
#else
    const unsigned deal_stride = gridDim.x * (unsigned)(THREADS / 64);
    const unsigned n_dealt = (unsigned)(((n + 63) / 64) / deal_stride) * deal_stride;
    unsigned deal_next = blockIdx.x * (unsigned)(THREADS / 64) + (threadIdx.x >> 6);
    auto tile_fetch = [&]() -> unsigned {
        if (deal_next < n_dealt) {
            const unsigned t_d = deal_next;
            deal_next += deal_stride;
            return t_d;
        }
        unsigned t_l = 0;
        if (lane == 0) t_l = n_dealt + atomicAdd(tile_counter, 1u);
        return t_l;
    };
#endif
    auto tile_parity = [&](unsigned t) -> unsigned {
        if (FUSED_INPLACE) return 0u;
        if (par_words > 0) return (unsigned)__builtin_amdgcn_readfirstlane((int)((par_bits[t >> 5] >> (t & 31u)) & 1u));
        return (unsigned)__builtin_amdgcn_readfirstlane((int)tile_par[t]);
    };
    auto tile_load = [&](unsigned t, unsigned par, double(&v)[D], double& oll, double& olp, double& olq) __attribute__((always_inline)) {
        const int64_t i = (int64_t)t * 64 + lane;
        const bool valid = i < n;
        const unsigned ys_tile = t * 64u * (unsigned)sizeof(T);
        const __amdgpu_buffer_rsrc_t ysr = __builtin_amdgcn_make_buffer_rsrc(par ? ysu1 : ysu, 0, half_records, 0x00020000);
        (void)valid;
#pragma unroll
        for (int j = 0; j < D; j++) v[j] = soa_load<T>(ysr, ys_lane, ys_tile + (unsigned)j * ys_row);
        oll = olp = olq = 0.0;
        if (valid) oll = ll[i], olp = lp[i], olq = lq[i];
    };
    double v[D];
    double oll = 0.0, olp = 0.0, olq = 0.0;
    unsigned t = idle_wave ? 0xFFFFFFFFu : (unsigned)__builtin_amdgcn_readfirstlane((int)tile_fetch());
    unsigned par = 0;
    bool have = (int64_t)t < n_tiles;
    if (have) {
        par = tile_parity(t);
        tile_load(t, par, v, oll, olp, olq);
    }
    while (have) {
        STAMP(0);
        int zoff;
        asm volatile("v_mov_b32 %0, 0" : "=v"(zoff));
        const double* __restrict__ Lt = tl + zoff;
        const float* __restrict__ locs = reinterpret_cast<const float*>(tl + (MVM ? M_LOC : T_LOC)) + zoff;
        const int64_t i = (int64_t)t * 64 + lane;
        const bool valid = i < n;
        const unsigned ys_tile = t * 64u * (unsigned)sizeof(T);
#if !FUSED_INPLACE
        const __amdgpu_buffer_rsrc_t ypr = __builtin_amdgcn_make_buffer_rsrc(par ? ysu : ysu1, 0, half_records, 0x00020000);
#endif
        const unsigned long long gid = p.gid0 + (unsigned long long)i;
        double q0 = 0.0, q1 = 0.0, q0t = 0.0;
        if (p.gam != nullptr) {
#pragma unroll
            for (int j = 0; j < D; j++) q0t = fma(v[j], v[j], q0t);
        }
        STAMP(1);
        const double rs = tpcn_scale(rho, p.nu, q0t, p.gam, valid ? i : 0);
        auto noise_phase = [&](auto full_c) {
            constexpr bool FULL = decltype(full_c)::value;
#pragma unroll
            for (int qd = 0; qd < D / 4; qd++) {
                if (!FULL && 4 * qd >= dn) continue;
                double z[4];
                if constexpr (NOISE == ASMC_NOISE_F64) normal_quad(p.seed, gid, step, (uint32_t)qd, bmt, z[0], z[1], z[2], z[3]);
                else normal_quad_f32(p.seed, gid, step, (uint32_t)qd, z[0], z[1], z[2], z[3]);
                if (FULL || 4 * qd + 4 <= dn) {
#pragma unroll
                    for (int e = 0; e < 4; e++) {
                        q0 = fma(v[4 * qd + e], v[4 * qd + e], q0);
                        v[4 * qd + e] = (double)(T)fma(rs, z[e], a * v[4 * qd + e]);
                        q1 = fma(v[4 * qd + e], v[4 * qd + e], q1);
                    }
                } else {
#pragma unroll
                    for (int e = 0; e < 4; e++) {
                        if (4 * qd + e >= dn) continue;
                        q0 = fma(v[4 * qd + e], v[4 * qd + e], q0);
                        v[4 * qd + e] = (double)(T)fma(rs, z[e], a * v[4 * qd + e]);
                        q1 = fma(v[4 * qd + e], v[4 * qd + e], q1);
                    }
                }
#ifndef FUSED_NOISE_SB
#define FUSED_NOISE_SB 1
#endif
                if constexpr (NOISE == ASMC_NOISE_F64) {
                    if (qd % FUSED_NOISE_SB == FUSED_NOISE_SB - 1) __builtin_amdgcn_sched_barrier(0);
                } else {
                    if (qd & 1) __builtin_amdgcn_sched_barrier(0);
                }
            }
        };
        if (dn == D) noise_phase(std::true_type{});
        else noise_phase(std::false_type{});
        STAMP(2);
        float xf[D];
        double qa = 0.0, qb = 0.0, mix_ll = 0.0, mix_lp = 0.0;
        if constexpr (MVM) {
#pragma unroll
            for (int sI = 0; sI < D / 4; sI++) fused_transpose4(v[4 * sI], v[4 * sI + 1], v[4 * sI + 2], v[4 * sI + 3]);
            const double* __restrict__ rowt = Lt + (lane >> 4) * 8;
            const double* __restrict__ Aimg = Lt + lane;
            fused_d4 acc[2][4];
            typedef double row_d2 __attribute__((ext_vector_type(2)));
            typedef float row_f2 __attribute__((ext_vector_type(2)));
            static_assert(M_MU % 2 == 0 && M_MIX % 2 == 0 && D % 4 == 0, "16-byte aligned row tables");
            const row_d2* __restrict__ row2 = reinterpret_cast<const row_d2*>(rowt);
            auto row4 = [&](int off, int mb, double (&out)[4]) {
                const row_d2 lo = row2[(off + 4 * mb) / 2], hi = row2[(off + 4 * mb) / 2 + 1];
                out[0] = lo.x, out[1] = lo.y, out[2] = hi.x, out[3] = hi.y;
            };
#pragma unroll
            for (int mb = 0; mb < 2; mb++) {
                double mu4[4];
                row4(M_MU, mb, mu4);
                const fused_d4 m = {mu4[0], mu4[1], mu4[2], mu4[3]};
#pragma unroll
                for (int nb = 0; nb < 4; nb++) acc[mb][nb] = m;
            }
#pragma unroll
            for (int sI = 0; sI < D / 4; sI++) {
                const double a1 = Aimg[(4 + sI) * 64];
                const double a0 = sI < 4 ? Aimg[sI * 64] : 0.0;
#pragma unroll
                for (int nb = 0; nb < 4; nb++) {
                    if (sI < 4) acc[0][nb] = __builtin_amdgcn_mfma_f64_16x16x4f64(a0, v[4 * sI + nb], acc[0][nb], 0, 0, 0);
                    acc[1][nb] = __builtin_amdgcn_mfma_f64_16x16x4f64(a1, v[4 * sI + nb], acc[1][nb], 0, 0, 0);
                }
                if (sI & 1) __builtin_amdgcn_sched_barrier(0);
            }
            double qpa[4] = {0.0, 0.0, 0.0, 0.0}, qpb[4] = {0.0, 0.0, 0.0, 0.0};
            const float* __restrict__ locr = locs + (lane >> 4) * 8;
#pragma unroll
            for (int mb = 0; mb < 2; mb++)
#pragma unroll
                for (int rp = 0; rp < 2; rp++) {
                    const int e2 = (4 * mb + 2 * rp) / 2;
                    const row_d2 ma2 = row2[M_MIX / 2 + e2], pa2 = row2[(M_MIX + D) / 2 + e2];
                    const row_d2 mb2 = row2[(M_MIX + FUSED_MAX_COMPONENTS * 2 * D) / 2 + e2], pb2 = row2[(M_MIX + FUSED_MAX_COMPONENTS * 2 * D + D) / 2 + e2];
                    const row_f2 lc2 = reinterpret_cast<const row_f2*>(locr)[e2], sc2 = reinterpret_cast<const row_f2*>(locr + D)[e2],
                                 rc2 = reinterpret_cast<const row_f2*>(locr + 2 * D)[e2];
#pragma unroll
                    for (int nb = 0; nb < 4; nb++) {
                        double xj[2];
#pragma unroll
                        for (int rr = 0; rr < 2; rr++) {
                            const int r = 2 * rp + rr;
                            xj[rr] = (double)(T)acc[mb][nb][r];
                            const double ta = xj[rr] - ma2[rr], tb = xj[rr] - mb2[rr];
                            qpa[nb] = fma(ta * ta, pa2[rr], qpa[nb]);
                            qpb[nb] = fma(tb * tb, pb2[rr], qpb[nb]);
                        }
                        const flow_std2 z2 = flow_standardise2(flow_std2{(float)xj[0], (float)xj[1]}, lc2, sc2, rc2);
                        xf[(4 * mb + nb) * 4 + 2 * rp] = z2.x;
                        xf[(4 * mb + nb) * 4 + 2 * rp + 1] = z2.y;
                    }
                }
            fused_transpose4(qpa[0], qpa[1], qpa[2], qpa[3]);
            fused_transpose4(qpb[0], qpb[1], qpb[2], qpb[3]);
            qa = (qpa[0] + qpa[1]) + (qpa[2] + qpa[3]);
            qb = (qpb[0] + qpb[1]) + (qpb[2] + qpb[3]);
            auto more_components = [&](int tt, int C, double q0c) -> double {
                double best = Lt[M_LOGW + tt * FUSED_MAX_COMPONENTS] - 0.5 * q0c;
                if (!MIX || C == 1) return best;
                double ssum = 1.0;
#pragma unroll 1
                for (int c = 1; c < C; c++) {
                    const double* __restrict__ tb = rowt + M_MIX + (tt * FUSED_MAX_COMPONENTS + c) * 2 * D;
                    double qp[4] = {0.0, 0.0, 0.0, 0.0};
#pragma unroll
                    for (int mb = 0; mb < 2; mb++)
#pragma unroll
                        for (int r = 0; r < 4; r++) {
                            const double mc = tb[4 * mb + r], pc = tb[D + 4 * mb + r];
#pragma unroll
                            for (int nb = 0; nb < 4; nb++) {
                                const double tv = (double)(T)acc[mb][nb][r] - mc;
                                qp[nb] = fma(tv * tv, pc, qp[nb]);
                            }
                        }
                    fused_transpose4(qp[0], qp[1], qp[2], qp[3]);
                    const double tc = Lt[M_LOGW + tt * FUSED_MAX_COMPONENTS + c] - 0.5 * ((qp[0] + qp[1]) + (qp[2] + qp[3]));
                    if (tc > best) {
                        ssum = fma(ssum, exp(best - tc), 1.0);
                        best = tc;
                    } else if (tc > -INFINITY) {
                        ssum += exp(tc - best);
                    }
                }
                return best == -INFINITY ? -INFINITY : best + log(ssum);
            };
            mix_ll = more_components(0, p.c_ll, qa);
            mix_lp = more_components(1, p.c_lp, qb);
        } else {
#ifdef MV_COMPILER
#pragma unroll
        for (int g = 0; g < D / 4; g++) {
            const int j0 = 4 * g;
            double sr[4] = {0.0, 0.0, 0.0, 0.0};
#pragma unroll
            for (int k = 0; k < j0 + 4; k++) {
#pragma unroll
                for (int r = 0; r < 4; r++)
                    if (k <= j0 + r) sr[r] = fma(Lt[(j0 + r) * D + k], v[k], sr[r]);
                if ((k & (MV_CHUNK - 1)) == MV_CHUNK - 1 || k == j0 + 3) asm volatile("" : "+v"(sr[0]), "+v"(sr[1]), "+v"(sr[2]), "+v"(sr[3])::"memory");
            }
#pragma unroll
            for (int r = 0; r < 4; r++) {
                const int j = j0 + r;
                const double xj = (double)(T)(Lt[T_MU + j] + sr[r]);
                const double ta = xj - Lt[T_LLMU + j], tb = xj - Lt[T_LPMU + j];
                qa = fma(ta * ta, Lt[T_LLPR + j], qa);
                qb = fma(tb * tb, Lt[T_LPPR + j], qb);
                xf[j] = flow_standardise((float)xj, locs[j], locs[D + j], locs[2 * D + j]);
            }
            asm volatile("" : "+v"(qa), "+v"(qb), "+v"(xf[j0]), "+v"(xf[j0 + 1]), "+v"(xf[j0 + 2]), "+v"(xf[j0 + 3])::"memory");
        }
#else
        {
            constexpr int NB = (D / 4) * (D / 4 + 1), P = MV_DEPTH;
            const unsigned lbase = (unsigned)(size_t)tl + (unsigned)zoff;
            double2v ring[P][4];
            double sr[4] = {0.0, 0.0, 0.0, 0.0};
            auto issue = [&](auto bc) {
                constexpr int bi = decltype(bc)::value, g = mv_group(bi), b = bi - g * (g + 1), slot = bi % P;
                constexpr int o0 = ((4 * g + 0) * D + 2 * b) * 8, o1 = o0 + D * 8, o2 = o1 + D * 8, o3 = o2 + D * 8;
                auto& rg = ring[slot];
                const unsigned lb = lbase;
                asm volatile("ds_read_b128 %0, %4 offset:%5\n\tds_read_b128 %1, %4 offset:%6\n\t"
                             "ds_read_b128 %2, %4 offset:%7\n\tds_read_b128 %3, %4 offset:%8"
                             : "=&v"(rg[0]), "=&v"(rg[1]), "=&v"(rg[2]), "=&v"(rg[3])
                             : "v"(lb), "n"(o0), "n"(o1), "n"(o2), "n"(o3));
            };
            auto consume = [&](auto bc) {
                constexpr int bi = decltype(bc)::value, g = mv_group(bi), b = bi - g * (g + 1), slot = bi % P, j0 = 4 * g;
                constexpr int ahead = (NB - 1 - bi) < (P - 1) ? (NB - 1 - bi) : (P - 1);
                if constexpr (bi + P - 1 < NB) issue(std::integral_constant<int, (bi + P - 1 < NB ? bi + P - 1 : 0)>{});
                auto& rg = ring[slot];
                static_assert(ahead <= 3, "lgkmcnt holds 15");
                if constexpr (ahead == 0)
                    asm volatile("s_waitcnt lgkmcnt(0)" : "+v"(rg[0]), "+v"(rg[1]), "+v"(rg[2]), "+v"(rg[3]));
                else if constexpr (ahead == 1)
                    asm volatile("s_waitcnt lgkmcnt(4)" : "+v"(rg[0]), "+v"(rg[1]), "+v"(rg[2]), "+v"(rg[3]));
                else if constexpr (ahead == 2)
                    asm volatile("s_waitcnt lgkmcnt(8)" : "+v"(rg[0]), "+v"(rg[1]), "+v"(rg[2]), "+v"(rg[3]));
                else
                    asm volatile("s_waitcnt lgkmcnt(12)" : "+v"(rg[0]), "+v"(rg[1]), "+v"(rg[2]), "+v"(rg[3]));
#pragma unroll
                for (int e = 0; e < 2; e++)
#pragma unroll
                    for (int r = 0; r < 4; r++)
                        if (2 * b + e <= j0 + r) sr[r] = fma(rg[r][e], v[2 * b + e], sr[r]);
                if constexpr (b == 2 * g + 1) {
#pragma unroll
                    for (int r = 0; r < 4; r++) {
                        const int j = j0 + r;
                        const double xj = (double)(T)(Lt[T_MU + j] + sr[r]);
                        const double ta = xj - Lt[T_LLMU + j], tb = xj - Lt[T_LPMU + j];
                        qa = fma(ta * ta, Lt[T_LLPR + j], qa);
                        qb = fma(tb * tb, Lt[T_LPPR + j], qb);
                        xf[j] = flow_standardise((float)xj, locs[j], locs[D + j], locs[2 * D + j]);
                        sr[r] = 0.0;
                    }
                    auto &a0 = qa, &a1 = qb;
                    auto &f0 = xf[j0], &f1 = xf[j0 + 1], &f2 = xf[j0 + 2], &f3 = xf[j0 + 3];
                    asm volatile("" : "+v"(a0), "+v"(a1), "+v"(f0), "+v"(f1), "+v"(f2), "+v"(f3)::"memory");
                }
            };
            mv_for_each<0, (P - 1 < NB ? P - 1 : NB)>(issue);
            mv_for_each<0, NB>(consume);
        }
#endif
        }
        const double nll = MVM ? mix_ll : Lt[T_LOGW] - 0.5 * qa;
        const double nlp = MVM ? mix_lp : Lt[T_LOGW + 1] - 0.5 * qb;
        STAMP(3);
#if !FUSED_INPLACE
        if (valid) {
#pragma unroll
            for (int j = 0; j < D; j++) soa_store<T>(ypr, ys_lane, ys_tile + (unsigned)j * ys_row, v[j]);
        }
#endif
        double t2 = p.beta * (nll + nlp);
        t2 = (t2 < INFINITY) ? t2 : __builtin_nan("");
        double c1 = ref_corr(q1, p.nu, dn);
        double rhs = log_p_t(oll, olp, olq, p.beta) + ref_corr(q0, p.nu, dn);
        double logu = bm_log_unit(accept_uniform(p.seed, gid, step));
        double kll = nll, klp = nlp;
        double kacc = ((t2 + c1) - rhs) - logu;
        asm volatile("" : "+v"(kacc), "+v"(kll), "+v"(klp));
#ifndef FUSED_NOSB
        __builtin_amdgcn_sched_barrier(0);
#endif
        float lqt[2];
        unsigned tn_l = 0;
        float xaA[1][H / 2], xbA[1][H / 2], xaB[1][H / 2], xbB[1][H / 2];
        if constexpr (MVM) {
#pragma unroll
            for (int mb = 0; mb < 2; mb++)
#pragma unroll
                for (int r = 0; r < 4; r++) {
                    const auto sA = __builtin_amdgcn_permlane16_swap(__float_as_uint(xf[(4 * mb + 0) * 4 + r]), __float_as_uint(xf[(4 * mb + 1) * 4 + r]), false, false);
                    const auto sB = __builtin_amdgcn_permlane16_swap(__float_as_uint(xf[(4 * mb + 2) * 4 + r]), __float_as_uint(xf[(4 * mb + 3) * 4 + r]), false, false);
                    if (mb == 0) {
                        xaA[0][r] = __uint_as_float(sA[0]), xaA[0][4 + r] = __uint_as_float(sA[1]);
                        xaB[0][r] = __uint_as_float(sB[0]), xaB[0][4 + r] = __uint_as_float(sB[1]);
                    } else {
                        xbA[0][r] = __uint_as_float(sA[0]), xbA[0][4 + r] = __uint_as_float(sA[1]);
                        xbB[0][r] = __uint_as_float(sB[0]), xbB[0][4 + r] = __uint_as_float(sB[1]);
                    }
                }
        } else {
#pragma unroll
        for (int r = 0; r < H / 2; r++) {
            const auto s1 = __builtin_amdgcn_permlane32_swap(__float_as_uint(xf[r]), __float_as_uint(xf[H / 2 + r]), false, false);
            xaA[0][r] = __uint_as_float(s1[0]);
            xaB[0][r] = __uint_as_float(s1[1]);
            const auto s2 = __builtin_amdgcn_permlane32_swap(__float_as_uint(xf[H + r]), __float_as_uint(xf[H + H / 2 + r]), false, false);
            xbA[0][r] = __uint_as_float(s2[0]);
            xbB[0][r] = __uint_as_float(s2[1]);
        }
        }
        if constexpr (KIND == ASMC_FLOW_MAF) {
            float xA[16], xB[16];
#pragma unroll
            for (int r = 0; r < 8; r++) xA[r] = xaA[0][r], xA[8 + r] = xbA[0][r], xB[r] = xaB[0][r], xB[8 + r] = xbB[0][r];
#ifndef FUSED_NOPRIO
            if (first_on_simd)
                __builtin_amdgcn_s_setprio(FUSED_PRIO_A);
            else
                __builtin_amdgcn_s_setprio(FUSED_PRIO_B);
#endif
            STAMP(4);
            tn_l = tile_fetch();
            auto maf_tile = [&](float(&xv)[16], auto form_c) __attribute__((always_inline)) -> float {
                constexpr int FORM = decltype(form_c)::value;
                float ladj = 0.0f;
                unsigned amax_pk = 0u;
                for (int c = 0; c < n_layers; c++) {
                    float cond[16];
#pragma unroll
                    for (int r = 0; r < 16; r++) cond[r] = xv[r];
                    coupling_layer_hs1p<HF, W, false, FORM, true>(cond, xv, sp + (size_t)c * FD::LAYER, lane, hh, ladj, amax_pk, FORM);
                    __builtin_amdgcn_sched_barrier(0);
                }
                float amax = range_pk_max(amax_pk);
                float q = 0.0f;
#pragma unroll
                for (int r = 0; r < 16; r++) q += xv[r] * xv[r];
                q += __shfl_xor(q, 32);
                const float lj = ladj + __shfl_xor(ladj, 32);
                amax = fmaxf(amax, __shfl_xor(amax, 32));
                return !(amax < FLOW_HS_MAX) ? __builtin_nanf("") : (-0.5f * q + base_const) + (ladj0 + lj);
            };
            if (affine == 0) {
                lqt[0] = maf_tile(xA, std::integral_constant<int, 0>{});
                __builtin_amdgcn_sched_barrier(0);
                STAMP(5);
                lqt[1] = maf_tile(xB, std::integral_constant<int, 0>{});
            } else {
                lqt[0] = maf_tile(xA, std::integral_constant<int, 1>{});
                __builtin_amdgcn_sched_barrier(0);
                STAMP(5);
                lqt[1] = maf_tile(xB, std::integral_constant<int, 1>{});
            }
        } else {
        auto flow_tile = [&](float(&xa)[1][H / 2], float(&xb)[1][H / 2]) __attribute__((always_inline)) -> float {
            float ladj[1] = {0.0f};
            float amax = 0.0f;
#ifndef FUSED_NOFLOW
            for (int c = 0; c < n_layers; c++) {
                const float* lpk = sp + (size_t)c * FD::LAYER;
                if (HS) {
                    if ((c & 1) == 0)
                        coupling_layer_hs<H, W, false, -1, false>(xa[0], xb[0], lpk, lane, hh, ladj[0], amax);
                    else
                        coupling_layer_hs<H, W, false, -1, false>(xb[0], xa[0], lpk, lane, hh, ladj[0], amax);
                } else if ((c & 1) == 0)
                    coupling_layer<H, W, 1>(xa, xb, lpk, lane, hh, ladj);
                else
                    coupling_layer<H, W, 1>(xb, xa, lpk, lane, hh, ladj);
            }
#endif
            float q = 0.0f;
#pragma unroll
            for (int r = 0; r < H / 2; r++) q += xa[0][r] * xa[0][r] + xb[0][r] * xb[0][r];
            q += __shfl_xor(q, 32);
            const float lj = ladj[0] + __shfl_xor(ladj[0], 32);
            amax = fmaxf(amax, __shfl_xor(amax, 32));
            return !(amax < FLOW_HS_MAX) ? __builtin_nanf("") : (-0.5f * q + base_const) + (ladj0 + lj);
        };
#ifndef FUSED_NOPRIO
        if (first_on_simd)
            __builtin_amdgcn_s_setprio(FUSED_PRIO_A);
        else
            __builtin_amdgcn_s_setprio(FUSED_PRIO_B);
#endif
        STAMP(4);
        tn_l = tile_fetch();
#ifndef FUSED_FLOW2
#define FUSED_FLOW2 1
#endif
        if (HS && FUSED_INPLACE) {
            auto one_tile = [&](float(&xa)[1][H / 2], float(&xb)[1][H / 2]) __attribute__((always_inline)) -> float {
                float ladj = 0.0f;
                unsigned amax_pk = 0u;
                for (int c = 0; c < n_layers; c++) {
                    const float* lpk = sp + (size_t)c * FD::LAYER;
                    if ((c & 1) == 0)
                        coupling_layer_hs1p<H, W, HS1P_PREFETCH, 0, true>(xa[0], xb[0], lpk, lane, hh, ladj, amax_pk);
                    else
                        coupling_layer_hs1p<H, W, HS1P_PREFETCH, 0, true>(xb[0], xa[0], lpk, lane, hh, ladj, amax_pk);
                    __builtin_amdgcn_sched_barrier(0);
                }
                float amax = range_pk_max(amax_pk);
                float q = 0.0f;
#pragma unroll
                for (int r = 0; r < H / 2; r++) q += xa[0][r] * xa[0][r] + xb[0][r] * xb[0][r];
                q += __shfl_xor(q, 32);
                const float lj = ladj + __shfl_xor(ladj, 32);
                amax = fmaxf(amax, __shfl_xor(amax, 32));
                return !(amax < FLOW_HS_MAX) ? __builtin_nanf("") : (-0.5f * q + base_const) + (ladj0 + lj);
            };
            lqt[0] = one_tile(xaA, xbA);
            __builtin_amdgcn_sched_barrier(0);
            STAMP(5);
            lqt[1] = one_tile(xaB, xbB);
        } else if (HS && FUSED_FLOW2 && W < 128) {
            float ladjA = 0.0f, ladjB = 0.0f;
            unsigned amaxA = 0u, amaxB = 0u;
            for (int c = 0; c < n_layers; c++) {
                const float* lpk = sp + (size_t)c * FD::LAYER;
                if ((c & 1) == 0)
                    coupling_layer_hs2<H, W>(xaA[0], xbA[0], xaB[0], xbB[0], lpk, lane, hh, ladjA, ladjB, amaxA, amaxB);
                else
                    coupling_layer_hs2<H, W>(xbA[0], xaA[0], xbB[0], xaB[0], lpk, lane, hh, ladjA, ladjB, amaxA, amaxB);
                __builtin_amdgcn_sched_barrier(0);
            }
            auto finish = [&](const float(&xa)[1][H / 2], const float(&xb)[1][H / 2], float ladj, unsigned amax_pk) -> float {
                float amax = range_pk_max(amax_pk);
                float q = 0.0f;
#pragma unroll
                for (int r = 0; r < H / 2; r++) q += xa[0][r] * xa[0][r] + xb[0][r] * xb[0][r];
                q += __shfl_xor(q, 32);
                const float lj = ladj + __shfl_xor(ladj, 32);
                amax = fmaxf(amax, __shfl_xor(amax, 32));
                return !(amax < FLOW_HS_MAX) ? __builtin_nanf("") : (-0.5f * q + base_const) + (ladj0 + lj);
            };
            lqt[0] = finish(xaA, xbA, ladjA, amaxA);
            lqt[1] = finish(xaB, xbB, ladjB, amaxB);
        } else {
            lqt[0] = flow_tile(xaA, xbA);
            __builtin_amdgcn_sched_barrier(0);
            STAMP(5);
            lqt[1] = flow_tile(xaB, xbB);
        }
        }
        __builtin_amdgcn_sched_barrier(0);
        __builtin_amdgcn_s_setprio(0);
        STAMP(6);
        const double nlq = (double)(hh == 0 ? lqt[0] : lqt[1]);
        const bool lq_finite = fabs(nlq) < INFINITY;
        if (valid && !lq_finite) n_bad++;
        const bool accepted = valid && lq_finite && fma(1.0 - p.beta, nlq, kacc) > 0.0;
#if FUSED_INPLACE
        if (accepted) {
            ll[i] = kll;
            lp[i] = klp;
            lq[i] = nlq;
            n_acc++;
        }
        if constexpr (MVM) {
            const unsigned long long accmask = __ballot(accepted);
            const unsigned ys_lane_t = (unsigned)(lane >> 4) * ys_row + (unsigned)(lane & 15) * (unsigned)sizeof(T);
            const __amdgpu_buffer_rsrc_t ysw = __builtin_amdgcn_make_buffer_rsrc(ysu, 0, half_records, 0x00020000);
#pragma unroll
            for (int r = 0; r < 4; r++) {
                if ((accmask >> (16 * r + (lane & 15))) & 1ull) {
#pragma unroll
                    for (int sI = 0; sI < D / 4; sI++)
                        soa_store<T>(ysw, ys_lane_t, ys_tile + (unsigned)(4 * sI) * ys_row + (unsigned)(16 * r) * (unsigned)sizeof(T), v[4 * sI + r]);
                }
            }
        } else if (accepted) {
            const __amdgpu_buffer_rsrc_t ysw = __builtin_amdgcn_make_buffer_rsrc(ysu, 0, half_records, 0x00020000);
#pragma unroll
            for (int j = 0; j < D; j++) soa_store<T>(ysw, ys_lane, ys_tile + (unsigned)j * ys_row, v[j]);
        }
        const unsigned tn = (unsigned)__builtin_amdgcn_readfirstlane((int)tn_l);
        const bool have_n = (int64_t)tn < n_tiles;
        unsigned par_n = 0;
        double vn[D];
#pragma unroll
        for (int j = 0; j < D; j++) vn[j] = 0.0;
        double olln = 0.0, olpn = 0.0, olqn = 0.0;
        if (have_n) {
            par_n = tile_parity(tn);
            tile_load(tn, par_n, vn, olln, olpn, olqn);
        }
#else
        const unsigned tn = (unsigned)__builtin_amdgcn_readfirstlane((int)tn_l);
        const bool have_n = (int64_t)tn < n_tiles;
        unsigned par_n = 0;
        double vn[D];
#pragma unroll
        for (int j = 0; j < D; j++) vn[j] = 0.0;
        double olln = 0.0, olpn = 0.0, olqn = 0.0;
        if (have_n) {
            par_n = tile_parity(tn);
            tile_load(tn, par_n, vn, olln, olpn, olqn);
        }
        if (accepted) {
            ll[i] = kll;
            lp[i] = klp;
            lq[i] = nlq;
            n_acc++;
        }
        {
            const int n_a = __builtin_popcountll(__ballot(accepted)), n_r = __builtin_popcountll(__ballot(valid && !accepted));
            const bool flip = n_a > 0 && n_r <= n_a;
            if (flip ? n_r > 0 : n_a > 0) {
                const __amdgpu_buffer_rsrc_t src = __builtin_amdgcn_make_buffer_rsrc(flip == (par != 0) ? ysu1 : ysu, 0, half_records, 0x00020000);
                const __amdgpu_buffer_rsrc_t dst = __builtin_amdgcn_make_buffer_rsrc(flip == (par != 0) ? ysu : ysu1, 0, half_records, 0x00020000);
                if (valid && accepted != flip) {
                    double w[D];
#pragma unroll
                    for (int j = 0; j < D; j++) w[j] = soa_load<T>(src, ys_lane, ys_tile + (unsigned)j * ys_row);
#pragma unroll
                    for (int j = 0; j < D; j++) soa_store<T>(dst, ys_lane, ys_tile + (unsigned)j * ys_row, w[j]);
                }
            }
            if (flip && lane == 0) tile_par[t] = (unsigned char)(par ^ 1u);
        }
#endif
        STAMP(7);
#ifdef FUSED_STAMP
        ntile++;
#endif
#ifndef FUSED_NOSB
        __builtin_amdgcn_sched_barrier(0);
#endif
        t = tn, par = par_n, have = have_n;
        oll = olln, olp = olpn, olq = olqn;
#pragma unroll
        for (int j = 0; j < D; j++) v[j] = vn[j];
    }
#ifdef FUSED_STAMP
    if (lane == 0 && blockIdx.x == 7 && (wave == 0 || wave == 4) && ntile > 0)
        printf("wave %d tiles %d | fetch %llu yload %llu noise %llu matvec %llu park+swap %llu flowA %llu flowB %llu accept %llu (cycles per tile)\n", wave, ntile,
               tsum[0] / ntile, tsum[1] / ntile, tsum[2] / ntile, tsum[3] / ntile, tsum[4] / ntile, tsum[5] / ntile, tsum[6] / ntile, tsum[7] / ntile);
#endif
    __shared__ long long s_cnt[THREADS / 64];
    n_acc = wave_sum_ll(n_acc);
    n_bad = wave_sum_ll(n_bad);
    if (lane == 0 && n_bad != 0 && ad.nonfinite) atomicAdd(ad.nonfinite, (unsigned long long)n_bad);
    if (lane == 0) s_cnt[wave] = n_acc;
    __syncthreads();
    if (threadIdx.x == 0) {
        long long tsum = 0;
        for (int w = 0; w < THREADS / 64; w++) tsum += s_cnt[w];
        block_counts[blockIdx.x] = tsum;
    }
    if (ad.done == nullptr) return;
    __shared__ int s_last;
    if (threadIdx.x == 0) {
        __builtin_amdgcn_fence(__ATOMIC_RELEASE, "agent");
        const unsigned int tk = __hip_atomic_fetch_add(ad.done, 1u, __ATOMIC_RELAXED, __HIP_MEMORY_SCOPE_AGENT);
        s_last = (tk == gridDim.x - 1u);
        if (s_last) __builtin_amdgcn_fence(__ATOMIC_ACQUIRE, "agent");
    }
    __syncthreads();
    if (!s_last) return;
    long long c = 0;
    for (int b = threadIdx.x; b < (int)gridDim.x; b += THREADS)
        c += __hip_atomic_load(&block_counts[b], __ATOMIC_RELAXED, __HIP_MEMORY_SCOPE_AGENT);
    c = wave_sum_ll(c);
    __syncthreads();
    if (lane == 0) s_cnt[wave] = c;
    __syncthreads();
    if (threadIdx.x == 0) {
        c = 0;
        for (int w = 0; w < THREADS / 64; w++) c += s_cnt[w];
        if (ad.cell) {
            ad.cell[ad.adapt >= 2 ? ad.t % ad.adapt : 0] = c;
            return;
        }
        ad.counts_out[ad.t] = c;
        ad.rho_hist[ad.t] = rho;
        if (ad.adapt == 1) {
            *ad.rho = pcn_adapt_rho(rho, c, ad.n, ad.target, ad.t);
        } else if (ad.adapt >= 2 && ((ad.t + 1) % ad.adapt == 0 || ad.last)) {
            double r = rho;
            for (int tp = ad.t - (ad.t % ad.adapt); tp <= ad.t; tp++)
                r = pcn_adapt_rho(r, tp == ad.t ? c : ad.counts_out[tp], ad.n, ad.target, tp);
            *ad.rho = r;
        }
    }
}

static PcnScalars fused_scalars(const PcnDev& pd) {
    PcnScalars ps;
    ps.beta = pd.beta;
    ps.nu = pd.nu;
    ps.gam = pd.gam;
    ps.ys = pd.ys;
    ps.n_pad = pd.n_pad;
    ps.d_real = pd.d;
    ps.d_noise = pd.d_noise;
    ps.seed = pd.seed;
    ps.gid0 = pd.gid0;
    ps.c_ll = pd.ll.C;
    ps.c_lp = pd.lp.C;
    ps.c_lq = 0;
    ps.bmtab = pd.bmtab;
    ps.tile_par = pd.tile_par;
    return ps;
}

template <typename T>
static int launch_pcn_flow_fused(asmc_ctx* ctx, int64_t n, double* ll, double* lp, double* lq, const PcnDev& pd,
                                 const asmc_coupling* f, const double* rho_ptr, uint32_t step, unsigned int* tile_counter,
                                 long long* block_counts, int* grid_out, const PcnAdaptArgs& adapt, int img_words, hipStream_t st) {
    const PcnScalars ps = fused_scalars(pd);
    const fused_u4* img = img_words > 0 ? reinterpret_cast<const fused_u4*>(ctx->d_fimg) : nullptr;
    const float ladj0 = (float)(-f->log_scale_sum);
    const float base_const = (float)(-0.5 * f->dims * 1.8378770664093453);
    const int64_t n_tiles = (n + 63) / 64;
    const int grid = (int)(n_tiles < (int64_t)ctx->num_cu * (FUSED_THREADS / 64) ? (n_tiles + FUSED_THREADS / 64 - 1) / (FUSED_THREADS / 64) : ctx->num_cu);
    *grid_out = grid;
    const bool hs = asmc_flow_math_split();
    const bool mix = pd.ll.C > 1 || pd.lp.C > 1;
#define ASMC_FUSED_CASE_K(WW, NZ, HSV, KD) ASMC_FUSED_CASE_KM(WW, NZ, HSV, KD, false)
#define ASMC_FUSED_CASE_KM(WW, NZ, HSV, KD, MX)                                                                           \
    if (f->hidden == WW && pd.noise == NZ && hs == HSV && f->kind == KD && mix == MX) {                                   \
        auto kern = k_pcn_flow_fused<T, WW, NZ, HSV, KD, MX>;                                                                 \
        const size_t lds0 = (size_t)f->n_layers * FlowDims<(KD == ASMC_FLOW_MAF ? 32 : 16), WW>::LAYER * sizeof(float) + FUSED_TL_DOUBLES * sizeof(double) + BM_TAB_N * sizeof(bm_d2); \
        const size_t par_bytes = (size_t)((n_tiles + 31) / 32) * 4;    \
        const int par_words = (!FUSED_INPLACE && lds0 + par_bytes <= 160 * 1024) ? (int)(par_bytes / 4) : 0;                     \
        const size_t lds = lds0 + (size_t)par_words * 4;                                                                     \
        static size_t attr_lds_dev[ASMC_MAX_DEVICES] = {0}; size_t& attr_lds = attr_lds_dev[asmc_dev_slot(ctx)];                                                                                      \
        if (lds > 64 * 1024 && lds > attr_lds) {                                                                         \
            ASMC_HIP(hipFuncSetAttribute(reinterpret_cast<const void*>(kern), hipFuncAttributeMaxDynamicSharedMemorySize, (int)lds)); \
            attr_lds = lds;                                                                                              \
        }                                                                                                                \
        ASMC_LAUNCH(ctx, st, "k_pcn_flow_fused", kern, dim3(grid), dim3(FUSED_THREADS), lds, st, n, ll, lp, lq,                     \
                    (const double*)ctx->d_ptab, ps, rho_ptr, step, f->packed_dev, (int)f->n_layers, f->loc_dev, f->scale_dev, \
                    ladj0, base_const, tile_counter, block_counts, adapt, par_words, KD == ASMC_FLOW_MAF ? (int)f->affine : 0, img, img_words);  \
        ASMC_LAUNCH_CHECK();                                                                                             \
        return ASMC_OK;                                                                                                  \
    }
#define ASMC_FUSED_CASE(WW, NZ, HSV) ASMC_FUSED_CASE_K(WW, NZ, HSV, ASMC_FLOW_COUPLING)
    ASMC_FUSED_CASE(64, ASMC_NOISE_F64, true)
#ifndef FUSED_ONLY_HEADLINE
    ASMC_FUSED_CASE_KM(64, ASMC_NOISE_F64, true, ASMC_FLOW_COUPLING, true)
    ASMC_FUSED_CASE_KM(64, ASMC_NOISE_F32, true, ASMC_FLOW_COUPLING, true)
    ASMC_FUSED_CASE(64, ASMC_NOISE_F64, false)
    ASMC_FUSED_CASE(64, ASMC_NOISE_F32, true)
    ASMC_FUSED_CASE(64, ASMC_NOISE_F32, false)
    ASMC_FUSED_CASE(32, ASMC_NOISE_F64, true)
    ASMC_FUSED_CASE(32, ASMC_NOISE_F64, false)
    ASMC_FUSED_CASE(32, ASMC_NOISE_F32, true)
    ASMC_FUSED_CASE(32, ASMC_NOISE_F32, false)
    ASMC_FUSED_CASE(128, ASMC_NOISE_F64, true)
    ASMC_FUSED_CASE(128, ASMC_NOISE_F64, false)
    ASMC_FUSED_CASE(128, ASMC_NOISE_F32, true)
    ASMC_FUSED_CASE(128, ASMC_NOISE_F32, false)
    ASMC_FUSED_CASE_K(64, ASMC_NOISE_F64, true, ASMC_FLOW_MAF)
    ASMC_FUSED_CASE_K(64, ASMC_NOISE_F32, true, ASMC_FLOW_MAF)
    ASMC_FUSED_CASE_K(32, ASMC_NOISE_F64, true, ASMC_FLOW_MAF)
    ASMC_FUSED_CASE_K(32, ASMC_NOISE_F32, true, ASMC_FLOW_MAF)
#endif
#undef ASMC_FUSED_CASE
#undef ASMC_FUSED_CASE_K
#undef ASMC_FUSED_CASE_KM
    asmc_set_error("fused flow step: unsupported flow (kind %d, hidden width %d)", (int)f->kind, (int)f->hidden);
    return ASMC_ERR_UNSUPPORTED;
}

bool asmc_pcn_flow_fused_ok(const asmc_pcn_params* prm, const asmc_coupling* f) {
    if (getenv("ASMC_FLOW_SPLIT")) return false;
    if (prm->d != 32 || f->dims > 32 || f->dims < 2) return false;
    if (f->dims != 32 && !(FUSED_MVMFMA && FUSED_INPLACE)) return false;
    if (f->kind == ASMC_FLOW_COUPLING && (f->dims % 2)) return false;
    const bool mvm = FUSED_MVMFMA && FUSED_INPLACE && f->kind == ASMC_FLOW_COUPLING && f->hidden == 64 && asmc_flow_math_split();
    const int cmax = mvm ? FUSED_MAX_COMPONENTS : 1;
    if (prm->log_likelihood.n_components < 1 || prm->log_likelihood.n_components > cmax) return false;
    if (prm->log_prior.n_components < 1 || prm->log_prior.n_components > cmax) return false;
    if (!(f->hidden == 32 || f->hidden == 64 || f->hidden == 128)) return false;
    if (f->kind == ASMC_FLOW_MAF) {
        if (!asmc_flow_math_split() || f->hidden == 128) return false;
        const size_t per_tr = (size_t)((2 * (f->hidden / 32) + 2) * 32 + f->hidden * 32 + f->hidden * f->hidden + 2 * 32 * f->hidden) * sizeof(float);
        return per_tr * (size_t)f->n_layers + FUSED_TL_DOUBLES * sizeof(double) + BM_TAB_N * sizeof(bm_d2) <= 160 * 1024;
    }
    const size_t per_layer = (size_t)((2 * (f->hidden / 32) + 1) * 32 + f->hidden * 16 + f->hidden * f->hidden + 2 * 16 * f->hidden) * sizeof(float);
    return per_layer * (size_t)f->n_layers + FUSED_TL_DOUBLES * sizeof(double) + BM_TAB_N * sizeof(bm_d2) <= 160 * 1024;
}


int asmc_pcn_flow_fused_stage(asmc_ctx* ctx, const PcnDev& pd, const asmc_coupling* f, int* words_out, hipStream_t st) {
    *words_out = 0;
    const char* mode = getenv("ASMC_FUSED_STAGE");
    if (mode && !strcmp(mode, "inline")) return ASMC_OK;
    const PcnScalars ps = fused_scalars(pd);
    const bool hs = asmc_flow_math_split();
#define ASMC_STAGE_CASE(WW, NZ, HSV, KD)                                                                                 \
    if (f->hidden == WW && pd.noise == NZ && hs == HSV && f->kind == KD) {                                               \
        auto kern = k_fused_stage_image<WW, NZ, HSV, KD>;                                                                \
        const int words = fused_image_words<WW, NZ, KD>((int)f->n_layers);                                               \
        const size_t lds = (size_t)words * 16;                                                                           \
        if (lds > ASMC_FUSED_IMAGE_BYTES) {                                                                              \
            asmc_set_error("fused flow step: LDS image of %zu bytes", lds);                                              \
            return ASMC_ERR_UNSUPPORTED;                                                                                 \
        }                                                                                                                \
        static size_t attr_lds_dev[ASMC_MAX_DEVICES] = {0}; size_t& attr_lds = attr_lds_dev[asmc_dev_slot(ctx)];         \
        if (lds > 64 * 1024 && lds > attr_lds) {                                                                         \
            ASMC_HIP(hipFuncSetAttribute(reinterpret_cast<const void*>(kern), hipFuncAttributeMaxDynamicSharedMemorySize, (int)lds)); \
            attr_lds = lds;                                                                                              \
        }                                                                                                                \
        ASMC_LAUNCH(ctx, st, "k_fused_stage_image", kern, dim3(1), dim3(FUSED_THREADS), lds, st, (const double*)ctx->d_ptab, ps, \
                    f->packed_dev, (int)f->n_layers, f->loc_dev, f->scale_dev, reinterpret_cast<fused_u4*>(ctx->d_fimg), words); \
        ASMC_LAUNCH_CHECK();                                                                                             \
        *words_out = words;                                                                                              \
        return ASMC_OK;                                                                                                  \
    }
#define ASMC_STAGE_CASES(WW)                                   \
    ASMC_STAGE_CASE(WW, ASMC_NOISE_F64, true, ASMC_FLOW_COUPLING)  \
    ASMC_STAGE_CASE(WW, ASMC_NOISE_F32, true, ASMC_FLOW_COUPLING)  \
    ASMC_STAGE_CASE(WW, ASMC_NOISE_F64, false, ASMC_FLOW_COUPLING) \
    ASMC_STAGE_CASE(WW, ASMC_NOISE_F32, false, ASMC_FLOW_COUPLING)
    ASMC_STAGE_CASES(64)
#ifndef FUSED_ONLY_HEADLINE
    ASMC_STAGE_CASES(32)
    ASMC_STAGE_CASES(128)
    ASMC_STAGE_CASE(64, ASMC_NOISE_F64, true, ASMC_FLOW_MAF)
    ASMC_STAGE_CASE(64, ASMC_NOISE_F32, true, ASMC_FLOW_MAF)
    ASMC_STAGE_CASE(32, ASMC_NOISE_F64, true, ASMC_FLOW_MAF)
    ASMC_STAGE_CASE(32, ASMC_NOISE_F32, true, ASMC_FLOW_MAF)
#endif
#undef ASMC_STAGE_CASES
#undef ASMC_STAGE_CASE
    asmc_set_error("fused flow step: unsupported flow (kind %d, hidden width %d)", (int)f->kind, (int)f->hidden);
    return ASMC_ERR_UNSUPPORTED;
}

int asmc_pcn_flow_fused_launch(asmc_ctx* ctx, int64_t n, int x_dtype, double* ll, double* lp, double* lq, const PcnDev& pd,
                               const asmc_coupling* f, const double* rho_ptr, uint32_t step, unsigned int* tile_counter,
                               long long* block_counts, int* grid_out, const PcnAdaptArgs& adapt, int img_words, hipStream_t st) {
    if (x_dtype == ASMC_F64)
        return launch_pcn_flow_fused<double>(ctx, n, ll, lp, lq, pd, f, rho_ptr, step, tile_counter, block_counts, grid_out, adapt, img_words, st);
    return launch_pcn_flow_fused<float>(ctx, n, ll, lp, lq, pd, f, rho_ptr, step, tile_counter, block_counts, grid_out, adapt, img_words, st);
}
```

### aspire_amd/csrc/asmc_scratch.h

```cpp
#pragma once

constexpr int DS_LEN = 4096;
constexpr int DS_REDUCE = 0;
constexpr int DS_REDUCE_LEN = 1024;
constexpr int DS_CDF_TOTAL = 1024;
constexpr int DS_CDF_APPROX_TOTAL = 1025;
constexpr int DS_GRAM_CENTER = 2048;
constexpr int DS_GRAM_CENTER_LEN = 128;
constexpr int DS_REF_STATUS = 2300;
constexpr int DS_STUDENT_EM = 2320;
constexpr int DS_STUDENT_EM_LEN = 8;
constexpr int DS_BISECT = 2560;
constexpr int DS_BISECT_REC = 64;
constexpr int DS_BISECT_LEN = 2 * DS_BISECT_REC;
constexpr int DS_TRTAB = 3072;
#define TRTAB_ROWS 14
#define TRTAB_SCALARS 8
constexpr int DS_TRTAB_LEN = TRTAB_ROWS * 32 + TRTAB_SCALARS;

constexpr int HP_LEN = 8192;
constexpr int HP_FRONT = 0;
constexpr int HP_FRONT_LEN = 128;
constexpr int HP_PCN_COUNTS = 0;
constexpr int HP_PCN_COUNTS_LEN = ASMC_MAX_PCN_STEPS;
constexpr int HP_PCN_RHO_HEAD = ASMC_MAX_PCN_STEPS;
constexpr int HP_PCN_RHO_HEAD_LEN = 8;
constexpr int HP_PCN_RHO_HIST = HP_PCN_RHO_HEAD + HP_PCN_RHO_HEAD_LEN;
constexpr int HP_PCN_RHO_HIST_LEN = ASMC_MAX_PCN_STEPS;
constexpr int HP_PCN_RHO = 8000;
constexpr int HP_PCN_NONFINITE = 8001;
constexpr int HP_PCN_LQ_COUNTS = 8002;
constexpr int HP_PCN_LQ_COUNTS_LEN = 2;
constexpr int HP_GRAM_CENTER = 2048;
constexpr int HP_GRAM_CENTER_LEN = 128;
constexpr int HP_PCG_TAB = 4096;
constexpr int HP_PCG_TAB_LEN = 256;
constexpr int HP_STEP_RESULT = 4096 + 512;
constexpr int HP_STEP_RESULT_LEN = 40 + 4 * 64;
constexpr int REF_STATUS_CELL0 = 8010;
constexpr int REF_STATUS_CELLS = 16;

constexpr size_t scratch_tiles_len(int64_t n_tiles_max) { return (size_t)(n_tiles_max * 4 + 64); }
constexpr size_t scratch_tiles_i_len(int64_t n_tiles_max) { return (size_t)(n_tiles_max * 8 + 64); }
static inline double* scratch_tile_s(const asmc_ctx* ctx) { return ctx->d_tiles + ctx->n_tiles_max * 2; }
static inline double* scratch_tile_s2(const asmc_ctx* ctx) { return ctx->d_tiles + ctx->n_tiles_max * 3; }
static inline long long* scratch_tile_split(const asmc_ctx* ctx) { return ctx->d_tiles_i + ctx->n_tiles_max * 4; }
static inline long long* scratch_count_total(const asmc_ctx* ctx) { return ctx->d_tiles_i + ctx->n_tiles_max * 8; }
constexpr bool scratch_tiles_fit(int64_t t) { return 4 * t <= (int64_t)scratch_tiles_len(t) && 8 * t + 1 <= (int64_t)scratch_tiles_i_len(t); }
static_assert(scratch_tiles_fit(1) && scratch_tiles_fit(1 << 20), "four / eight entries per tile and the total lie inside the tile arrays");

struct ScratchRegion {
    int buf, off, len, held;
};
enum {
    R_DS_REDUCE, R_DS_CDF_TOTAL, R_DS_CDF_APPROX_TOTAL, R_DS_GRAM_CENTER, R_DS_REF_STATUS, R_DS_STUDENT_EM, R_DS_BISECT, R_DS_TRTAB,
    R_HP_FRONT, R_HP_PCN_COUNTS, R_HP_PCN_RHO_HEAD, R_HP_PCN_RHO_HIST, R_HP_PCN_RHO, R_HP_PCN_NONFINITE, R_HP_PCN_LQ_COUNTS,
    R_HP_GRAM_CENTER, R_HP_PCG_TAB, R_HP_STEP_RESULT, R_HP_REF_STATUS, R_COUNT
};
constexpr ScratchRegion SCRATCH_MAP[R_COUNT] = {
    {0, DS_REDUCE, DS_REDUCE_LEN, 0},
    {0, DS_CDF_TOTAL, 1, 1},
    {0, DS_CDF_APPROX_TOTAL, 1, 0},
    {0, DS_GRAM_CENTER, DS_GRAM_CENTER_LEN, 0},
    {0, DS_REF_STATUS, 1, 0},
    {0, DS_STUDENT_EM, DS_STUDENT_EM_LEN, 0},
    {0, DS_BISECT, DS_BISECT_LEN, 1},
    {0, DS_TRTAB, DS_TRTAB_LEN, 0},
    {1, HP_FRONT, HP_FRONT_LEN, 0},
    {1, HP_PCN_COUNTS, HP_PCN_COUNTS_LEN, 1},
    {1, HP_PCN_RHO_HEAD, HP_PCN_RHO_HEAD_LEN, 1},
    {1, HP_PCN_RHO_HIST, HP_PCN_RHO_HIST_LEN, 1},
    {1, HP_PCN_RHO, 1, 1},
    {1, HP_PCN_NONFINITE, 1, 1},
    {1, HP_PCN_LQ_COUNTS, HP_PCN_LQ_COUNTS_LEN, 1},
    {1, HP_GRAM_CENTER, HP_GRAM_CENTER_LEN, 0},
    {1, HP_PCG_TAB, HP_PCG_TAB_LEN, 0},
    {1, HP_STEP_RESULT, HP_STEP_RESULT_LEN, 1},
    {1, REF_STATUS_CELL0, REF_STATUS_CELLS, 1},
};
constexpr int SCRATCH_KNOWN_OVERLAPS[][2] = {
    {R_HP_PCN_COUNTS, R_HP_FRONT},
    {R_HP_PCN_RHO_HEAD, R_HP_GRAM_CENTER},
    {R_HP_PCN_RHO_HIST, R_HP_GRAM_CENTER},
    {R_HP_PCN_RHO_HIST, R_HP_PCG_TAB},
};
constexpr int SCRATCH_HIST_SAFE_STEPS = HP_PCG_TAB - HP_PCN_RHO_HIST;

constexpr bool scratch_overlap(const ScratchRegion& a, const ScratchRegion& b) {
    return a.buf == b.buf && a.off < b.off + b.len && b.off < a.off + a.len;
}
constexpr bool scratch_known_overlap(int i, int j) {
    for (const auto& k : SCRATCH_KNOWN_OVERLAPS)
        if ((k[0] == i && k[1] == j) || (k[0] == j && k[1] == i)) return true;
    return false;
}
constexpr int scratch_first_outside() {
    for (int i = 0; i < R_COUNT; i++)
        if (SCRATCH_MAP[i].off < 0 || SCRATCH_MAP[i].len < 1 || SCRATCH_MAP[i].off + SCRATCH_MAP[i].len > (SCRATCH_MAP[i].buf ? HP_LEN : DS_LEN))
            return i;
    return -1;
}
constexpr int scratch_first_clash() {
    for (int i = 0; i < R_COUNT; i++)
        for (int j = 0; j < R_COUNT; j++)
            if (i != j && SCRATCH_MAP[i].held && scratch_overlap(SCRATCH_MAP[i], SCRATCH_MAP[j]) && !scratch_known_overlap(i, j)) return i;
    return -1;
}
constexpr bool scratch_known_overlaps_real() {
    for (const auto& k : SCRATCH_KNOWN_OVERLAPS)
        if (!scratch_overlap(SCRATCH_MAP[k[0]], SCRATCH_MAP[k[1]]) || !SCRATCH_MAP[k[0]].held || SCRATCH_MAP[k[1]].held) return false;
    return true;
}
static_assert(scratch_first_outside() == -1, "a scratch region leaves its buffer");
static_assert(scratch_first_clash() == -1, "a held scratch region overlaps another region");
static_assert(scratch_known_overlaps_real(), "SCRATCH_KNOWN_OVERLAPS lists held x transient overlaps that exist, nothing else");
static_assert(SCRATCH_HIST_SAFE_STEPS == 2040 && HP_PCN_RHO_HIST + SCRATCH_HIST_SAFE_STEPS <= HP_PCG_TAB, "history x jump-table staging");
static_assert(HP_PCN_RHO_HIST + HP_PCN_RHO_HIST_LEN <= HP_STEP_RESULT, "the longest history stays in front of the result record");
```

### aspire_amd/samplers/smc.py

```python
from __future__ import annotations

import copy
import logging
import math
import os
from typing import Any, Callable

import numpy as np
import torch

from .. import smc_math
from .._xp import is_torch, to_numpy
from ..history import SMCHistory
from ..samples import SMCSamples, Samples
from ..targets import DiagGaussianMixture
from .base import IdentityTransform, MCMCSampler, track_calls

logger = logging.getLogger(__name__)

DEFAULT_BETA_TOLERANCE = 1e-8


class SMCSampler(MCMCSampler):

# ... 471 lines not shown
        rows = torch.as_tensor((np.arange(k, dtype=np.int64) * n_local) // k, device=x.device)
        sub = x[rows].to(torch.float64).contiguous()
        if comm.sharded:
            sub = comm.all_gather_tensor(sub)
        st = self._pcn_state
        iters = int(self.sampler_kwargs.get("tpcn_fit_iters", 12 if st.get("nu") is None else 4))
        fit = None
        if (hasattr(e, "student_fit") and self.dims <= int(os.environ.get("ASMC_DEVICE_EM_MAX_D", 128))
                and not os.environ.get("ASMC_HOST_REFERENCE_FIT")):
            fit = e.student_fit(sub, iters, 1e-3, st.get("nu") or 20.0)
        if fit is not None:
            (mu_d, L_d, Linv_d), nu, _, status, _, _ = fit
            if status < 0:
                raise RuntimeError("could not factor the scale matrix of the Student-t fit")
            st["nu"] = nu
            self.history.mcmc_nu.append(float(nu) if nu <= NU_GAUSSIAN else float("inf"))
            return mu_d, L_d, Linv_d, (nu if nu <= NU_GAUSSIAN else 0.0)
        with _single_threaded_blas():
            mean, cov, nu = fit_student_t_device(e, sub, max_iter=iters, nu0=st.get("nu") or 20.0)
            L = _chol(cov)
            Linv = np.linalg.inv(L)
        st["nu"] = nu
        self.history.mcmc_nu.append(float(nu) if nu <= NU_GAUSSIAN else float("inf"))
        return (*self._upload_reference(mean, L, Linv), (nu if nu <= NU_GAUSSIAN else 0.0))

    def _mutate_preconditioned(self, particles: SMCSamples, x: torch.Tensor, beta: float, n_steps: int, target: float):
        e, comm, T = self.engine, self.comm, self.preconditioning_transform
        if getattr(T, "engine", None) is None and hasattr(T, "engine"):
            T.engine = e
        ll, lp, lq = particles.log_likelihood, particles.log_prior, particles.log_q
        n_local = x.shape[0]
        n_global = self._n_global(particles)
        gid0 = self._gid0(particles)
        try:
            z = T.fit(x, comm=comm)
        except TypeError:
            z = T.fit(x)
        z = e.asarray(z, dtype=x.dtype)
        logj = e.asarray(T.inverse(z)[1])
        mu, L, Linv, nu = self._fit_reference(z, n_global, self.sampler_kwargs.get("step_fn", "tpcn"))
        st = self._pcn_state
        if st["rho"] is None:
            st["rho"] = min(2.38 / math.sqrt(self.dims), 0.99)
        seed = int(self.rng.integers(0, 2**63 - 1, dtype=np.int64))
        step0 = st["step"]
        acc_rates = []

        logq_z = None
        if self.sampler_kwargs.get("flow_from_preconditioned", True) and hasattr(self.prior_flow, "log_prob_from_preconditioned"):
            logq_z = self.prior_flow.log_prob_from_preconditioned(T)

        def flow_lq(z_prop, x_prop, logj_new):
            nonlocal logq_z
            if logq_z is not None and z_prop.dtype in (torch.float64, torch.float32) and z_prop.is_contiguous():
                try:
                    return logq_z(z_prop, logj_new)
                except Exception as exc:
                    logger.info("log q from the preconditioned coordinate is not available: %s", exc)
                    logq_z = None
            return self._flow_log_prob(x_prop)

        def step(t, rho):
            z_prop, q0, q1 = e.pcn_propose(z, mu, L, Linv, rho, seed, gid0, step0 + t, nu=nu)
            x_prop, logj_new = T.inverse(z_prop)
            x_prop, logj_new = e.asarray(x_prop, dtype=x.dtype), e.asarray(logj_new)
            lq_new = flow_lq(z_prop, x_prop, logj_new)
            lp_new, ll_new = self._eval_prior_likelihood(x_prop, lq_new)
            return z_prop, q0, q1, ll_new, lp_new, lq_new, logj_new

        if hasattr(e, "pcn_split_begin"):
            if comm.sharded:
                e.set_count_hook(comm, n_global)
            try:
                done = 0
                while done < n_steps and hasattr(e, "pcn_ysplit_begin"):
                    chunk = min(n_steps - done, 2048)
                    sess = e.pcn_ysplit_begin(z, beta, mu, L, Linv, seed, gid0, st["rho"], target, True, nu,
                                              self.sampler_kwargs.get("noise", "f64"))
                    if sess is None:
                        break
                    t_dev = None
                    if (self.sampler_kwargs.get("fuse_transform", True) and hasattr(e, "pcn_ysplit_propose_tr")
                            and hasattr(T, "_tables") and not np.any(getattr(T, "_periodic", [1]))):
                        td = T._tables()[1]
                        if td.hints & 7 in (5, 3):
                            t_dev = td
                    for t in range(done, done + chunk):
                        if t_dev is not None:
                            x_prop, logj_new, lq_new = e.pcn_ysplit_propose_tr(sess, step0 + t, t_dev,
                                                                               getattr(logq_z, "fused_args", None))
                            if lq_new is None:
                                lq_new = self._flow_log_prob(x_prop)
                        else:
                            z_prop = e.pcn_ysplit_propose(sess, step0 + t)
                            x_prop, logj_new = T.inverse(z_prop)
                            x_prop, logj_new = e.asarray(x_prop, dtype=x.dtype), e.asarray(logj_new)
                            lq_new = flow_lq(z_prop, x_prop, logj_new)
                        lp_new, ll_new = self._eval_prior_likelihood(x_prop, lq_new)
                        e.pcn_ysplit_accept(sess, step0 + t, ll, lp, lq, ll_new, lp_new, lq_new, n_global, t - done,
                                            logj=logj, logj_new=logj_new)
                    n_acc, _, st["rho"] = e.pcn_ysplit_end(sess, chunk)
                    acc_rates.extend((n_acc / n_global).tolist())
                    done += chunk
                while done < n_steps:
                    chunk = min(n_steps - done, 2048)
                    e.pcn_split_begin(st["rho"])
                    for t in range(done, done + chunk):
                        z_prop, q0, q1, ll_new, lp_new, lq_new, logj_new = step(t, 0.0)
                        e.pcn_accept(z, z_prop, ll, lp, lq, ll_new, lp_new, lq_new, q0, q1, beta, seed, gid0, step0 + t,
                                     logj_old=logj, logj_new=logj_new, want_count=False)
                        e.pcn_split_adapt(n_global, target, t - done, True)
                    n_acc, _, st["rho"] = e.pcn_split_end(chunk)
                    acc_rates.extend((n_acc / n_global).tolist())
                    done += chunk
            finally:
                if comm.sharded:
                    e.set_count_hook(None, None)
        else:
            for t in range(n_steps):
                z_prop, q0, q1, ll_new, lp_new, lq_new, logj_new = step(t, st["rho"])
                n_acc = e.pcn_accept(z, z_prop, ll, lp, lq, ll_new, lp_new, lq_new, q0, q1, beta, seed, gid0, step0 + t,
                                     logj_old=logj, logj_new=logj_new)
                tot = float(comm.all_gather_f64(np.array([float(n_acc)])).sum())
                acc_rates.append(tot / n_global)
                st["rho"] = pcn_adapt(st["rho"], acc_rates[-1], target, t)
        st["step"] = step0 + n_steps
        self.history.mcmc_acceptance.append(float(np.mean(acc_rates)))
        self.history.mcmc_step_size.append(float(st["rho"]))
        x_new = e.asarray(T.inverse(z)[0], dtype=x.dtype)
        if self._global_counts([e.count_nonfinite(lq)[0]])[0]:
            raise ValueError("Log proposal contains NaN values")
        return self._wrap(x_new, ll, lp, lq, beta, like=particles)

    def _adapt_mode(self) -> int:
        k = int(self.sampler_kwargs.get("adapt_lag", 1) or 1)
        if not 1 <= k <= 64:
            raise ValueError(f"adapt_lag must be in 1 .. 64, got {k}")
        return k

    def _device_flow(self):
        if not hasattr(self.prior_flow, "device_coupling"):
            return self._adapted_zuko_flow()
        if not hasattr(self.engine, "coupling_logprob"):
            return None
        try:
            return self.prior_flow.device_coupling(self.engine)
        except (ValueError, RuntimeError) as exc:
            logger.info("flow stays on its torch modules: %s", exc)
            return None

    def _adapted_zuko_flow(self):
        if not self.sampler_kwargs.get("zuko_adapter", True) or not hasattr(self.engine, "coupling_logprob"):
            return None
        pf = self.prior_flow
        inner = getattr(pf, "_flow", None)
        if inner is None or not hasattr(inner, "state_dict"):
            return None
        dt = getattr(pf, "data_transform", None)
        if dt is not None and type(dt).__name__ != "IdentityTransform":
            logger.info("zuko adapter: the flow lives behind a data transform; it stays on its own modules")
            return None
        cache = self.__dict__.get("_zuko_cache")
        try:
            key = (id(inner), tuple((p.data_ptr(), int(p._version)) for p in inner.parameters()),
                   tuple((b.data_ptr(), int(b._version)) for b in inner.buffers()))
        except Exception:
            key = object()
        if cache is None or cache[0] != key:
            from ..flows import MAFFlow

            try:
                adapted = MAFFlow.from_zuko_state_dict(inner.state_dict(), device=self.engine.device)
                dev = adapted.device_coupling(self.engine)
                probe = torch.randn((256, self.dims), device=self.engine.device, dtype=torch.float64)
                try:
                    own = pf.sample_and_log_prob(256)[0]
                    own = self._to_dev(own).reshape(256, self.dims).to(torch.float64)
                    probe = torch.cat([probe, own[torch.isfinite(own).all(dim=1)]])
                except Exception as exc:
                    logger.info("zuko adapter: no draws from the flow for the cross-check (%s); standard-normal probes only", exc)
                mine = self.engine.coupling_logprob(probe, dev)
                theirs = self._to_dev(pf.log_prob(probe.to(getattr(pf, "dtype", torch.float32))))
                err = float(((mine - theirs).abs() / theirs.abs().clamp_min(1.0)).max())
                if not err <= 1e-4:
                    raise ValueError(f"adapted flow disagrees with the flow's own log_prob (max relative difference {err:.3g})")
                logger.info("zuko adapter in use (unverified against zuko itself; agrees with this flow's log_prob to %.1e on %d points)", err, len(probe))
            except Exception as exc:
                logger.warning("zuko adapter declined: %s", exc)
                dev = None
            cache = self._zuko_cache = (key, dev)
        return cache[1]

    def _flow_fused_ok(self, dev_flow) -> bool:
        return (dev_flow is not None and isinstance(self._log_likelihood, DiagGaussianMixture)
                and isinstance(self._log_prior, DiagGaussianMixture)
                and isinstance(self.preconditioning_transform, IdentityTransform))

    def _fused_ok(self) -> bool:
        return (isinstance(self._log_likelihood, DiagGaussianMixture)
                and isinstance(self._log_prior, DiagGaussianMixture)
                and hasattr(self.prior_flow, "device_mixture")
                and not getattr(self.prior_flow, "_has_transform", lambda: False)()
                and isinstance(self.preconditioning_transform, IdentityTransform))

    def mutate(self, particles: SMCSamples, beta: float, n_steps: int | None = None) -> SMCSamples:
        e, comm = self.engine, self.comm
        kwargs = self.sampler_kwargs.copy()
        n_steps = n_steps or kwargs.pop("n_steps")
        target = float(kwargs.get("target_acceptance_rate", 0.234))
        noise = kwargs.get("noise", "f64")
        x = particles.x if particles.x.is_contiguous() else particles.x.contiguous()
        T = self.preconditioning_transform
        transformed = not (isinstance(T, IdentityTransform) or getattr(T, "is_identity", False))
        if transformed:
            self.last_mutation_path = "preconditioned chain (z = T(x)): split propose / accept around the transform"
            out = self._mutate_preconditioned(particles, x, beta, n_steps, target)
            self._check_reference_fit()
            return out
        self.fit_preconditioning_transform(particles.x)
        ll, lp, lq = particles.log_likelihood, particles.log_prior, particles.log_q
        n_local = x.shape[0]
        n_global = self._n_global(particles)
        gid0 = self._gid0(particles)
        mu, L, Linv, nu = self._fit_reference(x, n_global, kwargs.get("step_fn", "tpcn"), particles.__dict__.get("_moments"))
        st = self._pcn_state
        if st["rho"] is None:
            st["rho"] = min(2.38 / math.sqrt(self.dims), 0.99)
        seed = int(self.rng.integers(0, 2**63 - 1, dtype=np.int64))
        step0 = st["step"]
        acc_rates = []
        dev_flow = self._device_flow()
        on_device = not comm.sharded or hasattr(e, "set_count_hook")
        if comm.sharded and on_device:
            e.set_count_hook(comm, n_global)
        try:
            out = self._mutate_steps(particles, x, ll, lp, lq, beta, n_steps, target, noise, mu, L, Linv, st, seed, step0,
                                     acc_rates, dev_flow, on_device, n_local, n_global, gid0, nu)
        finally:
            if comm.sharded and on_device:
                e.set_count_hook(None, None)
        self._check_reference_fit()
        return out

    def _check_reference_fit(self):
        if not self.__dict__.pop("_ref_fit_pending", False):
            return
        gen = self.__dict__.pop("_ref_fit_generation", None)
        status = self.engine.reference_factor_status(gen) if gen else self.engine.reference_factor_status()
        if status == -2:
            torch.cuda.synchronize(self.engine.device)
            status = self.engine.reference_factor_status(gen) if gen else self.engine.reference_factor_status()
        if status < 0:
            raise RuntimeError("could not factor the particle covariance")
        if status > 0:
            logger.info("reference covariance factored with jitter (try %d)", status)

    def _mutate_steps(self, particles, x, ll, lp, lq, beta, n_steps, target, noise, mu, L, Linv, st, seed, step0, acc_rates,
                      dev_flow, on_device, n_local, n_global, gid0, nu=0.0):
        e = self.engine
        m = (particles, x, ll, lp, lq, beta, n_steps, target, noise, mu, L, Linv, st, seed, step0, acc_rates, dev_flow, on_device,
             n_local, n_global, gid0, nu)
        if self._flow_fused_ok(dev_flow):
            self._steps_flow_on_device(m)
        elif self._fused_ok():
            self._steps_builtin_on_device(m)
        elif hasattr(e, "pcn_split_begin") and on_device:
            self._steps_callables_split(m)
        else:
            self._steps_callables_round_trip(m)
        return self._finish_mutation(m)

    def _steps_flow_on_device(self, m):
        e, comm = self.engine, self.comm
        (particles, x, ll, lp, lq, beta, n_steps, target, noise, mu, L, Linv, st, seed, step0, acc_rates, dev_flow, on_device,
         n_local, n_global, gid0, nu) = m
        self.last_mutation_path = "flow: device-side step loop (asmc_pcn_mutate_flow; one fused kernel per step where its shape is covered)"
        t_ll = self._log_likelihood.device_mixture(e)
        t_lp = self._log_prior.device_mixture(e)
        if on_device:
            done = 0
            while done < n_steps:
                chunk = min(n_steps - done, 2048)
                ahead = chunk == n_steps and n_steps <= 1024 and self._importance_step_follows(beta)
                if ahead:
                    handle = e.pcn_mutate_flow_enqueue(x, ll, lp, lq, beta, mu, L, Linv, t_ll, t_lp, dev_flow, seed, gid0,
                                                       st["rho"], chunk, step0, target, self._adapt_mode(), noise, nu)
                    out = self._wrap(x, ll, lp, lq, beta, like=particles)
                    ok = out.speculate_importance_step(self.current_target_efficiency(beta), self._beta_tolerance, self.rng,
                                                       resample_mode=self.resample_mode, resample_method=self.resample_method,
                                                       moments_n=self._speculated_moments_n(out), defer=True,
                                                       shard_layout=self.shard_layout, factor_ahead=self._factor_ahead())
                    n_acc, rho_hist, rho = e.pcn_mutate_flow_result(handle)
                    if ok:
                        st["prewrapped"] = out
                else:
                    n_acc, rho_hist, rho = e.pcn_mutate_flow(x, ll, lp, lq, beta, mu, L, Linv, t_ll, t_lp, dev_flow, seed,
                                                             gid0, st["rho"], chunk, step0 + done, target, self._adapt_mode(), noise, nu)
                st["rho"] = rho
                st["lq_checked"] = hasattr(e, "pcn_lq_nan")
                acc_rates.extend((n_acc / n_global).tolist())
                done += chunk
                n_bad = e.pcn_flow_nonfinite() if hasattr(e, "pcn_flow_nonfinite") else 0
                if n_bad > 0:
                    logger.warning(f"{n_bad} proposals had a non-finite flow density and were rejected (a badly scaled flow "
                                   "overflows the fp16 operand pairs of the flow kernel; ASMC_FLOW_MATH=f32 uses fp32 MFMAs)")
        else:
            for t in range(n_steps):
                n_acc, _, _ = e.pcn_mutate_flow(x, ll, lp, lq, beta, mu, L, Linv, t_ll, t_lp, dev_flow, seed, gid0,
                                                st["rho"], 1, step0 + t, target, False, noise, nu)
                tot = float(comm.all_gather_f64(np.array([float(n_acc[0])])).sum())
                acc_rates.append(tot / n_global)
                st["rho"] = pcn_adapt(st["rho"], acc_rates[-1], target, t)
        self.n_likelihood_evaluations += n_steps * n_local

    def _steps_builtin_on_device(self, m):
        e, comm = self.engine, self.comm
        (particles, x, ll, lp, lq, beta, n_steps, target, noise, mu, L, Linv, st, seed, step0, acc_rates, dev_flow, on_device,
         n_local, n_global, gid0, nu) = m
        self.last_mutation_path = "built-in densities: device-side step loop (asmc_pcn_mutate)"
        t_ll = self._log_likelihood.device_mixture(e)
        t_lp = self._log_prior.device_mixture(e)
        t_lq = self.prior_flow.device_mixture(e)
        if on_device:
            done = 0
            while done < n_steps:
                chunk = min(n_steps - done, 2048)
                n_acc, rho_hist, rho = e.pcn_mutate(x, ll, lp, lq, beta, mu, L, Linv, t_ll, t_lp, t_lq, seed,
                                                    gid0, st["rho"], chunk, step0 + done, target, self._adapt_mode(), noise, nu)
                st["rho"] = rho
                st["lq_checked"] = hasattr(e, "pcn_lq_nan")
                acc_rates.extend((n_acc / n_global).tolist())
                done += chunk
        else:
            for t in range(n_steps):
                n_acc, _, _ = e.pcn_mutate(x, ll, lp, lq, beta, mu, L, Linv, t_ll, t_lp, t_lq, seed, gid0,
                                           st["rho"], 1, step0 + t, target, False, noise, nu)
                tot = float(comm.all_gather_f64(np.array([float(n_acc[0])])).sum())
                acc_rates.append(tot / n_global)
                st["rho"] = pcn_adapt(st["rho"], acc_rates[-1], target, t)
        self.n_likelihood_evaluations += n_steps * n_local

    def _steps_callables_split(self, m):
        e, comm = self.engine, self.comm
        (particles, x, ll, lp, lq, beta, n_steps, target, noise, mu, L, Linv, st, seed, step0, acc_rates, dev_flow, on_device,
         n_local, n_global, gid0, nu) = m
        done = 0
        self.last_mutation_path = "callables: split propose / accept with the step closed on the stream (asmc_pcn_split_*)"
        while done < n_steps and hasattr(e, "pcn_ysplit_begin"):
            chunk = min(n_steps - done, 2048)
            sess = e.pcn_ysplit_begin(x, beta, mu, L, Linv, seed, gid0, st["rho"], target, True, nu, noise)
            if sess is None:
                break
            self.last_mutation_path = "callables: whitened-state session (asmc_pcn_ysplit_*)"
            for t in range(done, done + chunk):
                x_prop = e.pcn_ysplit_propose(sess, step0 + t)
                lq_new = self._flow_log_prob(x_prop)
                lp_new, ll_new = self._eval_prior_likelihood(x_prop, lq_new)
                e.pcn_ysplit_accept(sess, step0 + t, ll, lp, lq, ll_new, lp_new, lq_new, n_global, t - done)
            n_acc, _, st["rho"] = e.pcn_ysplit_end(sess, chunk)
            acc_rates.extend((n_acc / n_global).tolist())
            done += chunk
        while done < n_steps:
            chunk = min(n_steps - done, 2048)
            e.pcn_split_begin(st["rho"])
            for t in range(done, done + chunk):
                x_prop, q0, q1 = e.pcn_propose(x, mu, L, Linv, 0.0, seed, gid0, step0 + t, nu=nu)
                lq_new = self._flow_log_prob(x_prop)
                lp_new, ll_new = self._eval_prior_likelihood(x_prop, lq_new)
                e.pcn_accept(x, x_prop, ll, lp, lq, ll_new, lp_new, lq_new, q0, q1, beta, seed, gid0, step0 + t,
                             want_count=False)
                e.pcn_split_adapt(n_global, target, t - done, True)
            n_acc, _, st["rho"] = e.pcn_split_end(chunk)
            acc_rates.extend((n_acc / n_global).tolist())
            done += chunk

    def _steps_callables_round_trip(self, m):
        e, comm = self.engine, self.comm
        (particles, x, ll, lp, lq, beta, n_steps, target, noise, mu, L, Linv, st, seed, step0, acc_rates, dev_flow, on_device,
         n_local, n_global, gid0, nu) = m
        self.last_mutation_path = "callables: split propose / accept, one host round trip per step"
        for t in range(n_steps):
            x_prop, q0, q1 = e.pcn_propose(x, mu, L, Linv, st["rho"], seed, gid0, step0 + t, nu=nu)
            lq_new = self._flow_log_prob(x_prop)
            lp_new, ll_new = self._eval_prior_likelihood(x_prop, lq_new)
            n_acc = e.pcn_accept(x, x_prop, ll, lp, lq, ll_new, lp_new, lq_new, q0, q1, beta, seed, gid0,
                                 step0 + t)
            tot = float(comm.all_gather_f64(np.array([float(n_acc)])).sum())
            acc_rates.append(tot / n_global)
            st["rho"] = pcn_adapt(st["rho"], acc_rates[-1], target, t)

    def _finish_mutation(self, m):
        e, comm = self.engine, self.comm
        (particles, x, ll, lp, lq, beta, n_steps, target, noise, mu, L, Linv, st, seed, step0, acc_rates, dev_flow, on_device,
         n_local, n_global, gid0, nu) = m
        st["step"] = step0 + n_steps
        self.history.mcmc_acceptance.append(float(np.mean(acc_rates)))
        self.history.mcmc_step_size.append(float(st["rho"]))
        n_nan = e.pcn_lq_nan() if st.pop("lq_checked", False) else e.count_nonfinite(lq)[0]
        deferred = comm.sharded and beta < 1.0 and self.adaptive and self.device_bisection
        pre = st.pop("prewrapped", None)
        if not deferred and self._global_counts([n_nan])[0]:
            raise ValueError("Log proposal contains NaN values")
        return pre if pre is not None else self._wrap(x, ll, lp, lq, beta, like=particles)


_BLAS_CONTROLLER = []


def _single_threaded_blas():
    try:
        if not _BLAS_CONTROLLER:
            from threadpoolctl import ThreadpoolController

            _BLAS_CONTROLLER.append(ThreadpoolController())
        return _BLAS_CONTROLLER[0].limit(limits=1)
    except Exception:
        import contextlib

        return contextlib.nullcontext()


def pcn_adapt(rho: float, acc: float, target: float, t: int) -> float:
    r = math.exp(math.log(rho) + (acc - target) / (t + 1) ** 0.75)
    return min(max(r, 1e-4), 0.99)
```

Before: 3.578 billion.

## Skip flow density during beta=1 steps and refresh lq once for moved particles

When beta equals one, the fused pCN step kernel runs in a mode that omits the normalizing-flow log q evaluation, because the acceptance ratio does not depend on it. Accepted particles are marked in a per-particle moved-flag array. After the step loop, a separate refresh kernel recomputes lq only for tiles containing moved particles. This removes the flow network cost from every step at the final temperature, at the price of an extra pass, extra flag memory, and lq values that stay stale until the refresh.

```diff
diff --git a/aspire_amd/csrc/asmc_ctx.hip b/aspire_amd/csrc/asmc_ctx.hip
--- a/aspire_amd/csrc/asmc_ctx.hip
+++ b/aspire_amd/csrc/asmc_ctx.hip
@@ -189,7 +189,7 @@
     c->d_max_pad = d_max <= 4 ? 4 : d_max <= 8 ? 8 : d_max <= 16 ? 16 : d_max <= 32 ? 32 : d_max <= 64 ? 64 : d_max <= 128 ? 128 : 0;
     dmalloc((void**)&c->d_mmtab, sizeof(double) * 2 * 144 * 64);
     dmalloc((void**)&c->d_guide, sizeof(unsigned int) * ((size_t)n_max + 8));
-    dmalloc((void**)&c->d_tilectr, ASMC_TILECTR_BYTES + (size_t)n_max + 64);
+    dmalloc((void**)&c->d_tilectr, ASMC_TILECTR_BYTES + scratch_flags_len(n_max));
     c->d_flags = c->d_tilectr ? reinterpret_cast<unsigned char*>(c->d_tilectr) + ASMC_TILECTR_BYTES : nullptr;
     dmalloc((void**)&c->d_gamma, sizeof(double) * ((size_t)ASMC_GAMMA_BATCH * (size_t)n_max + 64 * ASMC_GAMMA_BATCH));
     dmalloc((void**)&c->d_rec, sizeof(double) * 4 * (size_t)n_max);
diff --git a/aspire_amd/csrc/asmc_pcn_dev.h b/aspire_amd/csrc/asmc_pcn_dev.h
--- a/aspire_amd/csrc/asmc_pcn_dev.h
+++ b/aspire_amd/csrc/asmc_pcn_dev.h
@@ -384,8 +384,12 @@
 bool asmc_pcn_flow_fused_ok(const asmc_pcn_params* prm, const asmc_coupling* f);
 int asmc_pcn_flow_fused_launch(asmc_ctx* ctx, int64_t n, int x_dtype, double* ll, double* lp, double* lq, const PcnDev& pd,
                                const asmc_coupling* f, const double* rho_ptr, uint32_t step, unsigned int* tile_counter,
-                               long long* block_counts, int* grid_out, const PcnAdaptArgs& adapt, int img_words, hipStream_t st);
+                               long long* block_counts, int* grid_out, const PcnAdaptArgs& adapt, int img_words, bool no_density,
+                               hipStream_t st);
 int asmc_pcn_flow_fused_stage(asmc_ctx* ctx, const PcnDev& pd, const asmc_coupling* f, int* words_out, hipStream_t st);
+bool asmc_pcn_flow_fused_beta1_ok(const asmc_coupling* f, int img_words);
+int asmc_pcn_flow_fused_refresh(asmc_ctx* ctx, int64_t n, int x_dtype, double* lq, const PcnDev& pd, const asmc_coupling* f,
+                                const double* rho_ptr, unsigned long long* nonfinite, hipStream_t st);
 
 #define MM_WHITEN 0
 #define MM_STEP 1
diff --git a/aspire_amd/csrc/asmc_pcn_drive.hip b/aspire_amd/csrc/asmc_pcn_drive.hip
--- a/aspire_amd/csrc/asmc_pcn_drive.hip
+++ b/aspire_amd/csrc/asmc_pcn_drive.hip
@@ -571,11 +571,13 @@
             return ASMC_ERR_UNSUPPORTED;
         }
         if (fused) {
-            ASMC_HIP(hipMemsetAsync(ctx->d_tilectr, 0, ASMC_TILECTR_BYTES + ((size_t)((n + 63) / 64) + 15) / 16 * 16, st));
+            const bool at_one = prm->beta == 1.0;
+            ASMC_HIP(hipMemsetAsync(ctx->d_tilectr, 0, ASMC_TILECTR_BYTES + scratch_flags_moved_off(n) + (at_one ? scratch_flags_fill(n) : 0), st));
             pd.tile_par = ctx->d_flags;
             int img_words = 0;
             rc = asmc_pcn_flow_fused_stage(ctx, pd, flow, &img_words, st);
             if (rc) return rc;
+            const bool no_density = at_one && asmc_pcn_flow_fused_beta1_ok(flow, img_words);
             const int lag = prm->adapt >= 2 ? prm->adapt : 1;
             rc = pcn_steps(
                 loop, pd,
@@ -590,7 +592,7 @@
                         return ASMC_ERR_ARG;
                     }
                     return asmc_pcn_flow_fused_launch(ctx, n, prm->x_dtype == ASMC_F64 ? ASMC_F64 : ASMC_F32, ll, lp, lq, pd, flow, d_rho, step,
-                                                      ctx->d_tilectr + t, d_block, g, ad, img_words, st);
+                                                      ctx->d_tilectr + t, d_block, g, ad, img_words, no_density, st);
                 },
                 [&](int t, int) -> int {
                     if (!(ctx->count_hook && ((t + 1) % lag == 0 || t == n_steps - 1))) return ASMC_OK;
@@ -601,6 +603,8 @@
                     }
                     return t == n_steps - 1 ? pcn_adapt_exchanged_launch(ctx, t, prm->target_accept, prm->adapt, lag, st) : ASMC_OK;
                 });
+            if (!rc && no_density)
+                rc = asmc_pcn_flow_fused_refresh(ctx, n, prm->x_dtype == ASMC_F64 ? ASMC_F64 : ASMC_F32, lq, pd, flow, d_rho, pcn_flow_bad_cell(ctx), st);
         } else {
             rc = pcn_steps(
                 loop, pd,
diff --git a/aspire_amd/csrc/asmc_pcn_fused.hip b/aspire_amd/csrc/asmc_pcn_fused.hip
--- a/aspire_amd/csrc/asmc_pcn_fused.hip
+++ b/aspire_amd/csrc/asmc_pcn_fused.hip
@@ -166,30 +166,36 @@
     for (int i = threadIdx.x; i < img_words; i += FUSED_THREADS) img[i] = reinterpret_cast<const fused_u4*>(sp)[i];
 }
 
-template <typename T, int W, int NOISE, bool HS, int KIND = ASMC_FLOW_COUPLING, bool MIX = false>
-__global__ __launch_bounds__(FUSED_THREADS) void k_pcn_flow_fused(
+#define FUSED_MODE_STEP 0
+#define FUSED_MODE_NQ 1
+#define FUSED_MODE_LQ 2
+template <typename T, int W, int NOISE, bool HS, int KIND, bool MIX, int MODE>
+__device__ __forceinline__ void fused_step_body(
     int64_t n, double* __restrict__ ll, double* __restrict__ lp, double* __restrict__ lq, const double* __restrict__ ptab,
     PcnScalars p, const double* rho_ptr, uint32_t step, const float* __restrict__ packed, int n_layers,
     const float* __restrict__ loc, const float* __restrict__ scale, float ladj0, float base_const,
     unsigned int* __restrict__ tile_counter, long long* __restrict__ block_counts, PcnAdaptArgs ad, int par_words, int affine,
-    const fused_u4* __restrict__ img, int img_words) {
+    const fused_u4* __restrict__ img, int img_words, unsigned char* __restrict__ moved) {
     constexpr int D = FUSED_D, H = 16, THREADS = FUSED_THREADS;
     constexpr int HF = KIND == ASMC_FLOW_MAF ? 32 : H;
     static_assert(KIND == ASMC_FLOW_COUPLING || HS, "the autoregressive variant runs the split-fp16 layers only");
+    static_assert(MODE == FUSED_MODE_STEP || (FUSED_MVMFMA && FUSED_INPLACE), "the beta = 1 modes live in the matrix-core, in-place build");
+    static_assert(MODE != FUSED_MODE_LQ || HS, "the refresh runs the split-fp16 layers");
     using FD = FlowDims<HF, W>;
     extern __shared__ __align__(16) float sp[];
-    constexpr int IMG_Q = ASMC_FUSED_IMAGE_BYTES / 16 / THREADS;
+    constexpr int IMG_BYTES = MODE == FUSED_MODE_NQ ? (int)(FUSED_TL_DOUBLES * sizeof(double) + BM_TAB_N * sizeof(bm_d2)) : ASMC_FUSED_IMAGE_BYTES;
+    constexpr int IMG_Q = (IMG_BYTES / 16 + THREADS - 1) / THREADS;
     fused_u4 iw[IMG_Q];
-    if (img != nullptr) {
+    if (MODE != FUSED_MODE_STEP || img != nullptr) {
 #pragma unroll
         for (int q = 0; q < IMG_Q; q++) {
             const int i4 = q * THREADS + (int)threadIdx.x;
             iw[q] = img[i4 < img_words ? i4 : img_words - 1];
         }
-    } else {
+    } else if constexpr (MODE == FUSED_MODE_STEP) {
         fused_stage_tables<W, NOISE, HS, KIND>(sp, ptab, p, packed, n_layers, loc, scale);
     }
-    double* tl = reinterpret_cast<double*>(sp + (size_t)n_layers * FD::LAYER);
+    double* tl = reinterpret_cast<double*>(sp + (MODE == FUSED_MODE_NQ ? (size_t)0 : (size_t)n_layers * FD::LAYER));
     bm_d2* bmt = reinterpret_cast<bm_d2*>(tl + FUSED_TL_DOUBLES);
     unsigned* const par_bits = reinterpret_cast<unsigned*>(bmt + BM_TAB_N);
     for (int wd = threadIdx.x; wd < par_words; wd += THREADS) {
@@ -203,7 +209,7 @@
         }
         par_bits[wd] = bits;
     }
-    if (img != nullptr) {
+    if (MODE != FUSED_MODE_STEP || img != nullptr) {
         __builtin_amdgcn_sched_barrier(0);
 #pragma unroll
         for (int q = 0; q < IMG_Q; q++) {
@@ -289,7 +295,7 @@
     const unsigned n_dealt = (unsigned)(((n + 63) / 64) / deal_stride) * deal_stride;
     unsigned deal_next = blockIdx.x * (unsigned)(THREADS / 64) + (threadIdx.x >> 6);
     auto tile_fetch = [&]() -> unsigned {
-        if (deal_next < n_dealt) {
+        if (MODE == FUSED_MODE_LQ || deal_next < n_dealt) {
             const unsigned t_d = deal_next;
             deal_next += deal_stride;
             return t_d;
@@ -313,7 +319,9 @@
 #pragma unroll
         for (int j = 0; j < D; j++) v[j] = soa_load<T>(ysr, ys_lane, ys_tile + (unsigned)j * ys_row);
         oll = olp = olq = 0.0;
-        if (valid) oll = ll[i], olp = lp[i], olq = lq[i];
+        if constexpr (MODE != FUSED_MODE_LQ) {
+            if (valid) oll = ll[i], olp = lp[i], olq = lq[i];
+        }
     };
     double v[D];
     double oll = 0.0, olp = 0.0, olq = 0.0;
@@ -322,10 +330,21 @@
     bool have = (int64_t)t < n_tiles;
     if (have) {
         par = tile_parity(t);
-        tile_load(t, par, v, oll, olp, olq);
+        if constexpr (MODE != FUSED_MODE_LQ) tile_load(t, par, v, oll, olp, olq);
     }
     while (have) {
         STAMP(0);
+        bool lq_mine = false;
+        if constexpr (MODE == FUSED_MODE_LQ) {
+            const int64_t i_m = (int64_t)t * 64 + lane;
+            lq_mine = i_m < n && moved[i_m] != 0;
+            if (__ballot(lq_mine) == 0ull) {
+                t = (unsigned)__builtin_amdgcn_readfirstlane((int)tile_fetch());
+                have = (int64_t)t < n_tiles;
+                continue;
+            }
+            tile_load(t, par, v, oll, olp, olq);
+        }
         int zoff;
         asm volatile("v_mov_b32 %0, 0" : "=v"(zoff));
         const double* __restrict__ Lt = tl + zoff;
@@ -338,12 +357,13 @@
 #endif
         const unsigned long long gid = p.gid0 + (unsigned long long)i;
         double q0 = 0.0, q1 = 0.0, q0t = 0.0;
-        if (p.gam != nullptr) {
+        if (MODE != FUSED_MODE_LQ && p.gam != nullptr) {
 #pragma unroll
             for (int j = 0; j < D; j++) q0t = fma(v[j], v[j], q0t);
         }
         STAMP(1);
-        const double rs = tpcn_scale(rho, p.nu, q0t, p.gam, valid ? i : 0);
+        double rs = 0.0;
+        if constexpr (MODE != FUSED_MODE_LQ) rs = tpcn_scale(rho, p.nu, q0t, p.gam, valid ? i : 0);
         auto noise_phase = [&](auto full_c) {
             constexpr bool FULL = decltype(full_c)::value;
 #pragma unroll
@@ -378,8 +398,10 @@
                 }
             }
         };
-        if (dn == D) noise_phase(std::true_type{});
-        else noise_phase(std::false_type{});
+        if constexpr (MODE != FUSED_MODE_LQ) {
+            if (dn == D) noise_phase(std::true_type{});
+            else noise_phase(std::false_type{});
+        }
         STAMP(2);
         float xf[D];
         double qa = 0.0, qb = 0.0, mix_ll = 0.0, mix_lp = 0.0;
@@ -575,12 +597,14 @@
         double logu = bm_log_unit(accept_uniform(p.seed, gid, step));
         double kll = nll, klp = nlp;
         double kacc = ((t2 + c1) - rhs) - logu;
-        asm volatile("" : "+v"(kacc), "+v"(kll), "+v"(klp));
+        if constexpr (MODE != FUSED_MODE_LQ) asm volatile("" : "+v"(kacc), "+v"(kll), "+v"(klp));
 #ifndef FUSED_NOSB
         __builtin_amdgcn_sched_barrier(0);
 #endif
-        float lqt[2];
+        float lqt[2] = {0.0f, 0.0f};
         unsigned tn_l = 0;
+        if constexpr (MODE == FUSED_MODE_NQ) tn_l = tile_fetch();
+        if constexpr (MODE != FUSED_MODE_NQ) {
         float xaA[1][H / 2], xbA[1][H / 2], xaB[1][H / 2], xbB[1][H / 2];
         if constexpr (MVM) {
 #pragma unroll
@@ -745,16 +769,27 @@
         }
         __builtin_amdgcn_sched_barrier(0);
         __builtin_amdgcn_s_setprio(0);
+        }
         STAMP(6);
-        const double nlq = (double)(hh == 0 ? lqt[0] : lqt[1]);
+        const double nlq = MODE == FUSED_MODE_NQ ? 0.0 : (double)(hh == 0 ? lqt[0] : lqt[1]);
         const bool lq_finite = fabs(nlq) < INFINITY;
-        if (valid && !lq_finite) n_bad++;
-        const bool accepted = valid && lq_finite && fma(1.0 - p.beta, nlq, kacc) > 0.0;
+        if constexpr (MODE == FUSED_MODE_LQ) {
+            if (lq_mine) {
+                lq[i] = nlq;
+                if (!lq_finite) n_bad++;
+            }
+            t = (unsigned)__builtin_amdgcn_readfirstlane((int)tn_l);
+            have = (int64_t)t < n_tiles;
+        } else {
+        if (MODE == FUSED_MODE_STEP && valid && !lq_finite) n_bad++;
+        const bool accepted = MODE == FUSED_MODE_NQ ? (valid && kacc > 0.0)
+                                                    : (valid && lq_finite && fma(1.0 - p.beta, nlq, kacc) > 0.0);
 #if FUSED_INPLACE
         if (accepted) {
             ll[i] = kll;
             lp[i] = klp;
             lq[i] = nlq;
+            if constexpr (MODE == FUSED_MODE_NQ) moved[i] = 1;
             n_acc++;
         }
         if constexpr (MVM) {
@@ -831,6 +866,7 @@
         oll = olln, olp = olpn, olq = olqn;
 #pragma unroll
         for (int j = 0; j < D; j++) v[j] = vn[j];
+        }
     }
 #ifdef FUSED_STAMP
     if (lane == 0 && blockIdx.x == 7 && (wave == 0 || wave == 4) && ntile > 0)
@@ -841,6 +877,7 @@
     n_acc = wave_sum_ll(n_acc);
     n_bad = wave_sum_ll(n_bad);
     if (lane == 0 && n_bad != 0 && ad.nonfinite) atomicAdd(ad.nonfinite, (unsigned long long)n_bad);
+    if constexpr (MODE == FUSED_MODE_LQ) return;
     if (lane == 0) s_cnt[wave] = n_acc;
     __syncthreads();
     if (threadIdx.x == 0) {
@@ -883,6 +920,37 @@
             *ad.rho = r;
         }
     }
+}
+
+template <typename T, int W, int NOISE, bool HS, int KIND = ASMC_FLOW_COUPLING, bool MIX = false>
+__global__ __launch_bounds__(FUSED_THREADS) void k_pcn_flow_fused(
+    int64_t n, double* __restrict__ ll, double* __restrict__ lp, double* __restrict__ lq, const double* __restrict__ ptab,
+    PcnScalars p, const double* rho_ptr, uint32_t step, const float* __restrict__ packed, int n_layers,
+    const float* __restrict__ loc, const float* __restrict__ scale, float ladj0, float base_const,
+    unsigned int* __restrict__ tile_counter, long long* __restrict__ block_counts, PcnAdaptArgs ad, int par_words, int affine,
+    const fused_u4* __restrict__ img, int img_words) {
+    fused_step_body<T, W, NOISE, HS, KIND, MIX, FUSED_MODE_STEP>(n, ll, lp, lq, ptab, p, rho_ptr, step, packed, n_layers, loc, scale, ladj0, base_const,
+                                                                 tile_counter, block_counts, ad, par_words, affine, img, img_words, nullptr);
+}
+template <typename T, int NOISE, bool MIX>
+__global__ __launch_bounds__(FUSED_THREADS) void k_pcn_flow_fused_nq(
+    int64_t n, double* __restrict__ ll, double* __restrict__ lp, double* __restrict__ lq, PcnScalars p, const double* rho_ptr, uint32_t step,
+    unsigned int* __restrict__ tile_counter, long long* __restrict__ block_counts, PcnAdaptArgs ad, const fused_u4* __restrict__ img,
+    int img_words, unsigned char* __restrict__ moved) {
+    fused_step_body<T, 64, NOISE, true, ASMC_FLOW_COUPLING, MIX, FUSED_MODE_NQ>(n, ll, lp, lq, nullptr, p, rho_ptr, step, nullptr, 0, nullptr, nullptr, 0.0f,
+                                                                               0.0f, tile_counter, block_counts, ad, 0, 0, img, img_words, moved);
+}
+template <typename T, int W, int KIND>
+__global__ __launch_bounds__(FUSED_THREADS) void k_pcn_flow_fused_lq(
+    int64_t n, double* __restrict__ lq, PcnScalars p, const double* rho_ptr, int n_layers, float ladj0, float base_const,
+    unsigned long long* __restrict__ nonfinite, int affine, const fused_u4* __restrict__ img, int img_words,
+    unsigned char* __restrict__ moved) {
+    PcnAdaptArgs ad;
+    ad.done = nullptr, ad.nonfinite = nonfinite, ad.cell = nullptr, ad.prev_cell = nullptr, ad.counts_out = nullptr, ad.rho = nullptr;
+    ad.rho_hist = nullptr, ad.target = 0.0, ad.n = n, ad.t = 0, ad.adapt = 0, ad.last = 0;
+    fused_step_body<T, W, ASMC_NOISE_F32, true, KIND, false, FUSED_MODE_LQ>(n, nullptr, nullptr, lq, nullptr, p, rho_ptr, 0u, nullptr, n_layers, nullptr,
+                                                                            nullptr, ladj0, base_const, nullptr, nullptr, ad, 0, affine, img,
+                                                                            img_words, moved);
 }
 
 static PcnScalars fused_scalars(const PcnDev& pd) {
@@ -904,10 +972,19 @@
     return ps;
 }
 
+static int fused_table_word0(const asmc_coupling* f) {
+    const int H = f->kind == ASMC_FLOW_MAF ? 32 : 16, W = (int)f->hidden;
+    const int layer = (2 * (W / 32) + H / 16) * 32 + W * H + W * W + 2 * H * W;
+    static_assert(FlowDims<16, 64>::LAYER == (2 * 2 + 1) * 32 + 64 * 16 + 64 * 64 + 2 * 16 * 64 && FlowDims<32, 32>::LAYER == (2 + 2) * 32 + 3 * 32 * 32 + 32 * 32,
+                  "FlowDims::LAYER by hand");
+    return (int)((size_t)f->n_layers * layer / 4);
+}
+
 template <typename T>
 static int launch_pcn_flow_fused(asmc_ctx* ctx, int64_t n, double* ll, double* lp, double* lq, const PcnDev& pd,
                                  const asmc_coupling* f, const double* rho_ptr, uint32_t step, unsigned int* tile_counter,
-                                 long long* block_counts, int* grid_out, const PcnAdaptArgs& adapt, int img_words, hipStream_t st) {
+                                 long long* block_counts, int* grid_out, const PcnAdaptArgs& adapt, int img_words, bool no_density,
+                                 hipStream_t st) {
     const PcnScalars ps = fused_scalars(pd);
     const fused_u4* img = img_words > 0 ? reinterpret_cast<const fused_u4*>(ctx->d_fimg) : nullptr;
     const float ladj0 = (float)(-f->log_scale_sum);
@@ -915,6 +992,30 @@
     const int64_t n_tiles = (n + 63) / 64;
     const int grid = (int)(n_tiles < (int64_t)ctx->num_cu * (FUSED_THREADS / 64) ? (n_tiles + FUSED_THREADS / 64 - 1) / (FUSED_THREADS / 64) : ctx->num_cu);
     *grid_out = grid;
+#if FUSED_MVMFMA && FUSED_INPLACE
+    if (no_density) {
+        const int tab_word0 = fused_table_word0(f);
+        const size_t lds = FUSED_TL_DOUBLES * sizeof(double) + BM_TAB_N * sizeof(bm_d2);
+        const bool mix = pd.ll.C > 1 || pd.lp.C > 1;
+#define ASMC_FUSED_NQ_CASE(NZ, MX)                                                                                              \
+    if (pd.noise == NZ && mix == MX) {                                                                                          \
+        auto kern = k_pcn_flow_fused_nq<T, NZ, MX>;                                                                             \
+        ASMC_LAUNCH(ctx, st, "k_pcn_flow_fused", kern, dim3(grid), dim3(FUSED_THREADS), lds, st, n, ll, lp, lq, ps, rho_ptr,     \
+                    step, tile_counter, block_counts, adapt, img + tab_word0, img_words - tab_word0, ctx->d_flags + scratch_flags_moved_off(n)); \
+        ASMC_LAUNCH_CHECK();                                                                                                    \
+        return ASMC_OK;                                                                                                         \
+    }
+        ASMC_FUSED_NQ_CASE(ASMC_NOISE_F64, false)
+#ifndef FUSED_ONLY_HEADLINE
+        ASMC_FUSED_NQ_CASE(ASMC_NOISE_F32, false)
+        ASMC_FUSED_NQ_CASE(ASMC_NOISE_F64, true)
+        ASMC_FUSED_NQ_CASE(ASMC_NOISE_F32, true)
+#endif
+#undef ASMC_FUSED_NQ_CASE
+        asmc_set_error("fused flow step without the density: unsupported noise mode %d", (int)pd.noise);
+        return ASMC_ERR_UNSUPPORTED;
+    }
+#endif
     const bool hs = asmc_flow_math_split();
     const bool mix = pd.ll.C > 1 || pd.lp.C > 1;
 #define ASMC_FUSED_CASE_K(WW, NZ, HSV, KD) ASMC_FUSED_CASE_KM(WW, NZ, HSV, KD, false)
@@ -1032,8 +1133,77 @@
 
 int asmc_pcn_flow_fused_launch(asmc_ctx* ctx, int64_t n, int x_dtype, double* ll, double* lp, double* lq, const PcnDev& pd,
                                const asmc_coupling* f, const double* rho_ptr, uint32_t step, unsigned int* tile_counter,
-                               long long* block_counts, int* grid_out, const PcnAdaptArgs& adapt, int img_words, hipStream_t st) {
+                               long long* block_counts, int* grid_out, const PcnAdaptArgs& adapt, int img_words, bool no_density,
+                               hipStream_t st) {
     if (x_dtype == ASMC_F64)
-        return launch_pcn_flow_fused<double>(ctx, n, ll, lp, lq, pd, f, rho_ptr, step, tile_counter, block_counts, grid_out, adapt, img_words, st);
-    return launch_pcn_flow_fused<float>(ctx, n, ll, lp, lq, pd, f, rho_ptr, step, tile_counter, block_counts, grid_out, adapt, img_words, st);
-}
+        return launch_pcn_flow_fused<double>(ctx, n, ll, lp, lq, pd, f, rho_ptr, step, tile_counter, block_counts, grid_out, adapt, img_words,
+                                             no_density, st);
+    return launch_pcn_flow_fused<float>(ctx, n, ll, lp, lq, pd, f, rho_ptr, step, tile_counter, block_counts, grid_out, adapt, img_words,
+                                        no_density, st);
+}
+
+bool asmc_pcn_flow_fused_beta1_ok(const asmc_coupling* f, int img_words) {
+#if FUSED_MVMFMA && FUSED_INPLACE
+    const char* mode = getenv("ASMC_FLOW_BETA1");
+    if (mode && !strcmp(mode, "full")) return false;
+    if (img_words <= 0 || !asmc_flow_math_split()) return false;
+#ifdef FUSED_ONLY_HEADLINE
+    return f->kind == ASMC_FLOW_COUPLING && f->hidden == 64;
+#else
+    if (f->kind == ASMC_FLOW_MAF) return f->hidden == 32 || f->hidden == 64;
+    return f->kind == ASMC_FLOW_COUPLING && (f->hidden == 32 || f->hidden == 64 || f->hidden == 128);
+#endif
+#else
+    (void)f, (void)img_words;
+    return false;
+#endif
+}
+
+#if FUSED_MVMFMA && FUSED_INPLACE
+template <typename T>
+static int launch_fused_lq_refresh(asmc_ctx* ctx, int64_t n, double* lq, const PcnDev& pd, const asmc_coupling* f, const double* rho_ptr,
+                                   unsigned long long* nonfinite, hipStream_t st) {
+    const PcnScalars ps = fused_scalars(pd);
+    const float ladj0 = (float)(-f->log_scale_sum);
+    const float base_const = (float)(-0.5 * f->dims * 1.8378770664093453);
+    const int64_t n_tiles = (n + 63) / 64;
+    const int grid = (int)(n_tiles < (int64_t)ctx->num_cu * (FUSED_THREADS / 64) ? (n_tiles + FUSED_THREADS / 64 - 1) / (FUSED_THREADS / 64) : ctx->num_cu);
+    const int words = fused_table_word0(f) + (int)(FUSED_TL_DOUBLES * sizeof(double) / 16);
+    const size_t lds = (size_t)words * 16;
+#define ASMC_FUSED_LQ_CASE(WW, KD)                                                                                               \
+    if (f->hidden == WW && f->kind == KD) {                                                                                      \
+        auto kern = k_pcn_flow_fused_lq<T, WW, KD>;                                                                              \
+        static size_t attr_lds_dev[ASMC_MAX_DEVICES] = {0}; size_t& attr_lds = attr_lds_dev[asmc_dev_slot(ctx)];                 \
+        if (lds > 64 * 1024 && lds > attr_lds) {                                                                                 \
+            ASMC_HIP(hipFuncSetAttribute(reinterpret_cast<const void*>(kern), hipFuncAttributeMaxDynamicSharedMemorySize, (int)lds)); \
+            attr_lds = lds;                                                                                                      \
+        }                                                                                                                        \
+        ASMC_LAUNCH(ctx, st, "k_fused_lq_refresh", kern, dim3(grid), dim3(FUSED_THREADS), lds, st, n, lq, ps, rho_ptr, (int)f->n_layers, ladj0, \
+                    base_const, nonfinite, KD == ASMC_FLOW_MAF ? (int)f->affine : 0, reinterpret_cast<const fused_u4*>(ctx->d_fimg), words, \
+                    ctx->d_flags + scratch_flags_moved_off(n));                                                                  \
+        ASMC_LAUNCH_CHECK();                                                                                                     \
+        return ASMC_OK;                                                                                                          \
+    }
+    ASMC_FUSED_LQ_CASE(64, ASMC_FLOW_COUPLING)
+#ifndef FUSED_ONLY_HEADLINE
+    ASMC_FUSED_LQ_CASE(32, ASMC_FLOW_COUPLING)
+    ASMC_FUSED_LQ_CASE(128, ASMC_FLOW_COUPLING)
+    ASMC_FUSED_LQ_CASE(64, ASMC_FLOW_MAF)
+    ASMC_FUSED_LQ_CASE(32, ASMC_FLOW_MAF)
+#endif
+#undef ASMC_FUSED_LQ_CASE
+    asmc_set_error("fused log q refresh: unsupported flow (kind %d, hidden width %d)", (int)f->kind, (int)f->hidden);
+    return ASMC_ERR_UNSUPPORTED;
+}
+#endif
+
+int asmc_pcn_flow_fused_refresh(asmc_ctx* ctx, int64_t n, int x_dtype, double* lq, const PcnDev& pd, const asmc_coupling* f,
+                                const double* rho_ptr, unsigned long long* nonfinite, hipStream_t st) {
+#if FUSED_MVMFMA && FUSED_INPLACE
+    if (x_dtype == ASMC_F64) return launch_fused_lq_refresh<double>(ctx, n, lq, pd, f, rho_ptr, nonfinite, st);
+    return launch_fused_lq_refresh<float>(ctx, n, lq, pd, f, rho_ptr, nonfinite, st);
+#else
+    asmc_set_error("fused log q refresh: not in this build");
+    return ASMC_ERR_UNSUPPORTED;
+#endif
+}
diff --git a/aspire_amd/csrc/asmc_scratch.h b/aspire_amd/csrc/asmc_scratch.h
--- a/aspire_amd/csrc/asmc_scratch.h
+++ b/aspire_amd/csrc/asmc_scratch.h
@@ -48,6 +48,14 @@
 static inline long long* scratch_count_total(const asmc_ctx* ctx) { return ctx->d_tiles_i + ctx->n_tiles_max * 8; }
 constexpr bool scratch_tiles_fit(int64_t t) { return 4 * t <= (int64_t)scratch_tiles_len(t) && 8 * t + 1 <= (int64_t)scratch_tiles_i_len(t); }
 static_assert(scratch_tiles_fit(1) && scratch_tiles_fit(1 << 20), "four / eight entries per tile and the total lie inside the tile arrays");
+
+constexpr size_t SCRATCH_FLAGS_SLACK = 64;
+constexpr size_t scratch_flags_len(int64_t n_max) { return (size_t)n_max + (size_t)n_max / 64 + SCRATCH_FLAGS_SLACK; }
+constexpr size_t scratch_flags_fill(int64_t entries) { return ((size_t)entries + 15) / 16 * 16; }
+constexpr size_t scratch_flags_moved_off(int64_t n) { return scratch_flags_fill((n + 63) / 64); }
+constexpr bool scratch_flags_fit(int64_t n) { return scratch_flags_moved_off(n) + scratch_flags_fill(n) <= scratch_flags_len(n); }
+static_assert(scratch_flags_fit(1) && scratch_flags_fit(63) && scratch_flags_fit(193) && scratch_flags_fit(1 << 20) && scratch_flags_fit((1 << 20) + 1),
+              "parities and moved marks, each rounded to 16 bytes, stay inside the allocation");
 
 struct ScratchRegion {
     int buf, off, len, held;
diff --git a/aspire_amd/samplers/smc.py b/aspire_amd/samplers/smc.py
--- a/aspire_amd/samplers/smc.py
+++ b/aspire_amd/samplers/smc.py
@@ -797,8 +797,11 @@
                 done += chunk
                 n_bad = e.pcn_flow_nonfinite() if hasattr(e, "pcn_flow_nonfinite") else 0
                 if n_bad > 0:
-                    logger.warning(f"{n_bad} proposals had a non-finite flow density and were rejected (a badly scaled flow "
-                                   "overflows the fp16 operand pairs of the flow kernel; ASMC_FLOW_MATH=f32 uses fp32 MFMAs)")
+                    what = ("particles moved at beta = 1 carry a non-finite flow density (the accept test has no log q term there; "
+                            "the check of the carried log q raises on them)" if beta == 1.0
+                            else "proposals had a non-finite flow density and were rejected")
+                    logger.warning(f"{n_bad} {what} (a badly scaled flow overflows the fp16 operand pairs of the flow kernel; "
+                                   "ASMC_FLOW_MATH=f32 uses fp32 MFMAs)")
         else:
             for t in range(n_steps):
                 n_acc, _, _ = e.pcn_mutate_flow(x, ll, lp, lq, beta, mu, L, Linv, t_ll, t_lp, dev_flow, seed, gid0,
```

Result: faster. 3.835 billion, median of 6 (+7.2%).
